# Robinatp/YOLO_Tensorflow

Measured on AMD Instinct MI355X. Metric: images_per_sec, higher is better.
Workload: dtype bf16; 1 GPU; YOLOv3 416x416 batch=32 per GPU, bf16: conv stack + head decode + threshold + TF-NMS; global_batch=32, input=uint8 NHWC resident in HBM, weights=seeded synthetic darknet stream (seed 0), parallelism=dp1

## Files before the change

### include/yolo_hip.h

```cpp
#ifndef YOLO_HIP_H
#define YOLO_HIP_H

#include <stddef.h>
#include <stdint.h>

#ifdef __cplusplus
extern "C" {
#endif

typedef struct yolo_ctx yolo_ctx;

enum yolo_status {
    YOLO_OK = 0,
    YOLO_ERR_INVALID = -1,
    YOLO_ERR_HIP = -2,
    YOLO_ERR_STATE = -3,
    YOLO_ERR_NOMEM = -4,
    YOLO_ERR_IO = -5,
    YOLO_ERR_UNSUPPORTED = -6
};

enum yolo_dtype { YOLO_BF16 = 0, YOLO_FP32 = 1, YOLO_FP8 = 2,
                  YOLO_FP16 = 3,
                  YOLO_FP16X2 = 4 };
// ... 107 lines not shown

int yolo_synchronize(yolo_ctx *ctx);

int yolo_layer_output(yolo_ctx *ctx, int index, int n, float *out, size_t out_floats, int *dims_out);
int yolo_time_forward(yolo_ctx *ctx, int n, int iters, float *total_ms, float *conv_ms);
int yolo_calibrate(int device, void *stream, int f16, double seconds, float *tflops, float *clock_ghz);
int yolo_calibrate_copy(int device, void *stream, double seconds, float *gbs);
int yolo_time_layers(yolo_ctx *ctx, int n, int iters, float *ms_out);
int yolo_autotune(yolo_ctx *ctx, int n, int iters);
int yolo_get_tile_configs(const yolo_ctx *ctx, int32_t *cfgs);
int yolo_set_tile_configs(yolo_ctx *ctx, const int32_t *cfgs);

int yolo_op_conv2d(const float *x, int n, int h, int w, int cin, const float *w_hwio, const float *bias,
                   int k, int stride, int cout, int act, const float *residual, float *out,
                   int dtype, int tile_cfg, int device);
int yolo_op_conv_num_cfgs(void);
int yolo_op_upsample2x(const float *x, int n, int h, int w, int c, int semantics, float *out, int device);
int yolo_op_reorg(const float *x, int n, int h, int w, int c, int stride, int semantics, float *out, int device);
int yolo_op_maxpool(const float *x, int n, int h, int w, int c, int size, int stride, float *out, int device);
int yolo_op_resize_u8(const uint8_t *img, int h, int w, int s, float post_scale, float *out, int device);
int yolo_op_resize_cv2(const uint8_t *img, int h, int w, int oh, int ow, int swap_rb, float divisor, float *out, int device);
int yolo_op_detections_boxes(const float *det, int n, int rows, int attrs, float *out, int device);
int yolo_op_decode(const float *raw, int n, int g, int na, int classes, const float *anchors_wh,
                   int img_size, int decode, int region, float *out, int device);
int yolo_op_letterbox(const float *image_chw, int iw, int ih, int w, int h, int embed, float *out_chw, int device);
int yolo_op_nms_detections(const float *boxes_xywh, float *prob, float *objectness, int n, int classes, float thresh,
                           int by_objectness, int device);
int yolo_op_postprocess(const float *det, int n, int rows, int attrs, float score_thr, float iou_thr,
                        int max_out, int nms_mode, int select_mode, yolo_box *boxes_out,
                        int32_t *counts_out, int device);
int yolo_op_postprocess_rows(const float *det, int n, int rows, int attrs, float score_thr, float iou_thr,
                             int max_out, int nms_mode, int select_mode, yolo_box *boxes_out,
                             int32_t *counts_out, int32_t *rows_out, int device);

int yolo_num_classes(const yolo_ctx *ctx);
int yolo_classify(yolo_ctx *ctx, const void *images, int n, int fmt, int loc, float scale, int top_k,
                  int32_t *classes_out, float *probs_out, int out_loc);
int yolo_classify_images_u8(yolo_ctx *ctx, const uint8_t *pixels, size_t bytes, const yolo_image_desc *descs, int n, int fit, int loc,
                            int top_k, int32_t *classes_out, float *probs_out, int out_loc);
int yolo_op_avgpool(const float *x, int n, int h, int w, int c, int dtype, float *out, int device);
int yolo_op_softmax(const float *x, int n, int len, int groups, float temperature, int top_k, float *probs_out,
                    int32_t *classes_out, float *topk_probs_out, int device);

enum yolo_hierarchy_mode { YOLO_HIER_CONDITIONAL = 0, YOLO_HIER_ABSOLUTE = 1, YOLO_HIER_LEAVES = 2 };
int yolo_set_hier_thresh(yolo_ctx *ctx, float hier_thresh);
int yolo_set_hierarchy_mode(yolo_ctx *ctx, int mode);
int yolo_darknet_boxes_map(yolo_ctx *ctx, int image, int w, int h, float thresh, int relative, const int32_t *map200, float *records, int cap, int *count);
int yolo_tree_geometry(const yolo_ctx *ctx, int32_t *nodes, int32_t *groups, int32_t *parent, int32_t *child, int32_t *group_offset,
                       int32_t *group_size, int32_t *leaf);
int yolo_tree_read(const char *path, int32_t *nodes, int32_t *groups, int32_t *parent, int32_t *child, int32_t *group_offset, int32_t *group_size,
                   int32_t *leaf, char *err, size_t err_len);
int yolo_plan_check(const char *cfg_text, int dtype, char *err, size_t err_len);
int yolo_plan_table(const char *cfg_text, int dtype, int max_batch, int keep_layers, char *out, size_t out_len, char *err, size_t err_len);
int yolo_op_tree_softmax(const float *x, int n, int len, const char *tree_path, float temperature, int mode, float *out, int device);
int yolo_op_tree_top(const float *x_logits, int n, const char *tree_path, float hier_thresh, int32_t *labels_out, int device);

#ifdef __cplusplus
}
#endif
#endif
```

### yolo_tensorflow_amd/csrc/conv_cfgs.h

```cpp
#pragma once
#include "kernels.h"
#include <type_traits>

struct ConvCfg {
    int id, wp, wc, tp, tc, ns, bk, nl;
    bool halo;
    bool free;
    int bh, bw;
    bool head_tail;
};
#define X(id, wp, wc, tp, tc, ns, bk, nl) {id, wp, wc, tp, tc, ns, bk, nl, false, false, 0, 0, false},
#define HX(id, wp, wc, tp, tc, ns, bk, nl, free, bh, bw, head_tail) {id, wp, wc, tp, tc, ns, bk, nl, true, free, bh, bw, head_tail},
constexpr ConvCfg kCfgs[] = {
    X(0, 2, 2, 4, 4, 2, 64, 0)  X(1, 2, 2, 4, 4, 3, 64, 0)  X(2, 2, 2, 2, 4, 2, 64, 0)  X(3, 2, 2, 2, 4, 3, 64, 0)
    X(4, 4, 1, 4, 2, 2, 64, 0)  X(5, 4, 1, 4, 2, 3, 64, 0)  X(6, 2, 2, 4, 2, 2, 64, 0)  X(7, 2, 2, 4, 2, 3, 64, 0)
    X(8, 4, 1, 4, 4, 2, 64, 0)  X(9, 4, 1, 4, 4, 3, 64, 0)  X(10, 4, 2, 4, 4, 2, 64, 0) X(11, 4, 2, 4, 4, 3, 64, 0)
    X(12, 2, 4, 4, 4, 2, 64, 0) X(13, 2, 4, 4, 4, 3, 64, 0) X(14, 2, 2, 2, 2, 2, 64, 0) X(15, 2, 2, 2, 2, 4, 64, 0)
    X(16, 1, 4, 11, 2, 2, 64, 0) X(17, 1, 4, 11, 4, 2, 64, 0) X(18, 1, 4, 11, 1, 2, 64, 0) X(19, 1, 4, 10, 2, 2, 64, 0)
    X(20, 1, 4, 12, 2, 2, 64, 0) X(21, 1, 4, 9, 2, 2, 64, 0) X(22, 1, 4, 13, 2, 2, 64, 0) X(23, 1, 4, 6, 2, 2, 64, 0)
    X(24, 1, 4, 7, 2, 2, 64, 0)
    X(25, 1, 4, 11, 2, 2, 32, 0) X(26, 2, 2, 4, 2, 2, 32, 0)  X(27, 4, 1, 4, 2, 2, 32, 0)  X(28, 4, 1, 4, 4, 2, 32, 0)
    X(29, 2, 2, 2, 2, 2, 32, 0)  X(30, 2, 2, 2, 4, 2, 32, 0)
    X(31, 1, 8, 11, 2, 2, 64, 4) X(32, 1, 8, 11, 2, 2, 64, 0)
    X(33, 1, 4, 11, 2, 3, 64, 0) X(34, 1, 4, 6, 2, 3, 64, 0)
    X(35, 2, 4, 3, 4, 2, 64, 0)
    HX(36, 1, 8, 11, 2, 2, 64, 0, false, 13, 13, false) HX(37, 1, 8, 11, 2, 2, 64, 4, false, 13, 13, false)
    HX(38, 1, 4, 11, 2, 2, 64, 4, false, 13, 13, false) HX(39, 1, 4, 11, 2, 2, 64, 0, false, 13, 13, false)
    HX(40, 1, 8, 11, 2, 2, 64, 0, true, 13, 13, true)   HX(41, 1, 8, 11, 1, 2, 64, 0, true, 13, 13, false)
    HX(42, 1, 4, 11, 2, 2, 64, 0, true, 13, 13, false)  HX(43, 1, 8, 11, 1, 3, 64, 0, true, 13, 13, false)
    X(44, 1, 8, 6, 2, 2, 64, 0) X(45, 1, 8, 6, 2, 3, 64, 0) X(46, 2, 4, 3, 4, 2, 64, 0) X(47, 2, 4, 2, 4, 2, 64, 0)
    X(48, 2, 4, 3, 2, 2, 64, 0) X(49, 2, 4, 4, 2, 3, 64, 0) X(50, 1, 8, 4, 2, 3, 64, 0) X(51, 2, 4, 2, 2, 3, 64, 0)
    X(52, 2, 4, 3, 2, 3, 64, 0) X(53, 2, 4, 3, 2, 4, 64, 0)
    HX(54, 1, 8, 12, 2, 2, 64, 0, true, 10, 19, true) HX(55, 1, 8, 12, 1, 3, 64, 0, true, 10, 19, false) HX(56, 1, 8, 6, 1, 3, 64, 0, true, 5, 19, false)
    HX(57, 1, 4, 11, 4, 2, 64, 0, true, 13, 13, false) HX(58, 1, 4, 11, 2, 2, 64, 0, true, 13, 13, false)
};
#undef X
#undef HX
constexpr int kNumCfgs = (int)(sizeof(kCfgs) / sizeof(kCfgs[0]));
constexpr bool conv_cfgs_indexed() { for (int i = 0; i < kNumCfgs; ++i) if (kCfgs[i].id != i) return false; return true; }
static_assert(conv_cfgs_indexed(), "a tile configuration's id is its index in kCfgs");

template <int... I> struct CfgList { static constexpr bool has(int cfg) { return ((cfg == I) || ...); } };
template <int... I, class F> hipError_t cfg_dispatch(CfgList<I...>, int cfg, F &&f)
{
    hipError_t e = hipErrorInvalidValue;
    (void)((cfg == I && ((e = f(std::integral_constant<int, I>{})), true)) || ...);
    return e;
}
using Cfgs16 = CfgList<0, 1, 2, 3, 4, 5, 6, 7, 8, 9, 10, 11, 12, 13, 14, 15, 16, 17, 18, 19, 20, 21, 22, 23, 24, 25, 26, 27, 28, 29, 30, 31, 32, 33, 34, 35,
                       44, 45, 46, 47, 48, 49, 50, 51, 52, 53>;
using CfgsHalo16 = CfgList<36, 37, 38, 39, 40, 41, 42, 43, 54, 55, 56>;
using CfgsFp8 = CfgList<0, 2, 4, 6, 8, 12, 14, 16, 17, 19, 20, 23, 31, 32, 33, 34, 45, 48, 49, 51>;
using CfgsHaloFp8 = CfgList<36, 37, 38, 39, 40, 41, 42, 43>;
using CfgsSplit = CfgList<0, 2, 3, 4, 6, 7, 8, 14, 15, 16, 23, 25, 26, 27, 28, 33, 34, 45, 49, 52>;
using CfgsHaloSplit = CfgList<40, 41, 43>;
using CfgsPairK = CfgList<0, 2, 3, 4, 6, 7, 8, 14, 15, 16, 23, 33, 34, 45, 49, 52>;
using CfgsHaloPairK = CfgList<40, 41, 43, 57, 58>;
using CfgsPairKPlain = CfgList<0, 2, 4, 6, 8, 14, 16, 33>;

template <int... I> constexpr bool cfgs_are(CfgList<I...>, bool halo) { return ((I >= 0 && I < kNumCfgs && kCfgs[I].halo == halo) && ...); }
static_assert(cfgs_are(Cfgs16{}, false) && cfgs_are(CfgsFp8{}, false) && cfgs_are(CfgsSplit{}, false) && cfgs_are(CfgsPairK{}, false) && cfgs_are(CfgsPairKPlain{}, false), "tiled lists hold tiled ids");
static_assert(cfgs_are(CfgsHalo16{}, true) && cfgs_are(CfgsHaloFp8{}, true) && cfgs_are(CfgsHaloSplit{}, true) && cfgs_are(CfgsHaloPairK{}, true), "halo lists hold halo ids");

inline bool conv_cfg_instantiated(const ConvArgs &a, int cfg)
{
    if (a.in_dt == DT_FP8) return CfgsFp8::has(cfg) || CfgsHaloFp8::has(cfg);
    if (a.pairk) return a.split ? CfgsPairK::has(cfg) || CfgsHaloPairK::has(cfg) : CfgsPairKPlain::has(cfg);
    if (a.split) return CfgsSplit::has(cfg) || CfgsHaloSplit::has(cfg);
    return Cfgs16::has(cfg) || CfgsHalo16::has(cfg);
}

constexpr bool conv_tail_shape(int wp, int wc, int bc, int nl, int eb) { return wp == 1 && wc == 8 && (eb == 2 ? nl == 0 && (bc == 256 || bc == 128) : bc == 256); }
```

### yolo_tensorflow_amd/csrc/conv_igemm.hip

```cpp
#include "kernels.h"
#include <cstdio>
#include <mutex>
#include <set>
#include <utility>

hipError_t conv_opt_in_lds(const void *kernel, size_t lds_bytes)
{
    static std::mutex mu;
    static std::set<std::pair<int, const void *>> done;
    int dev = 0;
    hipError_t e = hipGetDevice(&dev); if (e != hipSuccess) return e;
    std::lock_guard<std::mutex> g(mu);
    if (done.count({dev, kernel})) return hipSuccess;
    e = hipFuncSetAttribute(kernel, hipFuncAttributeMaxDynamicSharedMemorySize, (int)lds_bytes);
    if (e == hipSuccess) done.insert({dev, kernel});
    return e;
}

#include "conv_igemm_kernel.h"


template <int EB>
static hipError_t launch_conv_diag_t(const ConvArgs &a, hipStream_t s)
{
// ... 90 lines not shown

bool conv_c8_direct_ok(const ConvArgs &a)
{
    return (a.in_dt == DT_BF16 || (a.in_dt == DT_F16 && a.out_dt == DT_F16)) && a.ksize == 3 && a.stride == 1 && a.pad == 1 && a.Cin_pad == 8 && a.out_dt != DT_F32 && !a.res && a.Kpad >= 96 &&
           (a.Cout == 16 || a.Cout == 32 || a.Cout == 64);
}

hipError_t launch_conv_c8_direct(const ConvArgs &a, hipStream_t s)
{
    const long M = (long)a.N * a.Ho * a.Wo;
    long waves = (M + 63) / 64;
    long blocks = (waves + 3) / 4; if (blocks > 256 * 8) blocks = 256 * 8;
    dim3 grid((unsigned)blocks), block(256);
    if (a.in_dt == DT_F16) {
        if (a.Cout == 16) hipLaunchKernelGGL((conv_c8_3x3_direct<1, true>), grid, block, 0, s, a);
        else if (a.Cout == 32) hipLaunchKernelGGL((conv_c8_3x3_direct<2, true>), grid, block, 0, s, a);
        else hipLaunchKernelGGL((conv_c8_3x3_direct<4, true>), grid, block, 0, s, a);
    }
    else if (a.Cout == 16) hipLaunchKernelGGL((conv_c8_3x3_direct<1>), grid, block, 0, s, a);
    else if (a.Cout == 32) hipLaunchKernelGGL((conv_c8_3x3_direct<2>), grid, block, 0, s, a);
    else hipLaunchKernelGGL((conv_c8_3x3_direct<4>), grid, block, 0, s, a);
    return hipGetLastError();
}

int conv_num_cfgs() { return kNumCfgs; }
bool conv_cfg_is_halo(int cfg) { return cfg >= 0 && cfg < kNumCfgs && kCfgs[cfg].halo; }
bool conv_cfg_tail_ok(int cfg, int cout, bool fp8, bool head)
{
    if (cfg < 0 || cfg >= kNumCfgs) return false;
    const ConvCfg &c = kCfgs[cfg];
    const int bc = c.wc * c.tc * 16;
    if (head) return !fp8 && c.head_tail && cout == 256;
    return conv_tail_shape(c.wp, c.wc, bc, c.nl, fp8 ? 1 : 2) && bc == cout;
}
const char *conv_cfg_name(int cfg)
{
    struct Names {
        char s[kNumCfgs][32];
        Names()
        {
            for (const ConvCfg &c : kCfgs) {
                const int bp = c.wp * c.tp * 16, bc = c.wc * c.tc * 16;
                if (c.halo && !CfgsHalo16::has(c.id)) snprintf(s[c.id], sizeof s[c.id], "f%dc%d_w%d_pair", bp, bc, c.wp * c.wc);
                else if (c.halo && (c.bh != HALO_B || c.bw != HALO_B)) snprintf(s[c.id], sizeof s[c.id], "f%dx%dc%d_s%d", c.bh, c.bw, bc, c.ns);
                else snprintf(s[c.id], sizeof s[c.id], "%s%dc%d_s%d_k%d%s%d", c.halo ? (c.free ? "f" : "h") : "p", bp, bc, c.ns, c.bk, c.nl ? "_L" : "_w", c.nl ? c.nl : c.wp * c.wc);
            }
        }
    };
    static const Names names;
    if (cfg < 0 || cfg >= kNumCfgs) return cfg == CONV_CFG_DIRECT ? "direct_c8" : "?";
    return names.s[cfg];
}

template <int WP, int WC, int TP, int TC, int NS, int BK, int NL, bool UNI, int EB, bool H16 = false, bool SPLIT = false>
static hipError_t launch_u(const ConvArgs &a, hipStream_t s)
{
    constexpr int BP = WP * TP * 16, BC = WC * TC * 16;
    const long M = (long)a.N * a.Ho * a.Wo;
    const long tiles = ((M + BP - 1) / BP) * ((a.Cout + BC - 1) / BC);
    constexpr size_t lds = conv_lds_bytes<WP, WC, TP, TC, NS, BK, NL>();
    dim3 grid((unsigned)((tiles + 7) / 8 * 8)), block(64 * (WP * WC + NL));
    if (lds > 65536) {
        hipError_t e = conv_opt_in_lds((const void *)conv_igemm<WP, WC, TP, TC, NS, BK, UNI, NL, false, EB, false, false, H16, SPLIT>, lds);
        if (e != hipSuccess) return e;
    }
    hipLaunchKernelGGL((conv_igemm<WP, WC, TP, TC, NS, BK, UNI, NL, false, EB, false, false, H16, SPLIT>), grid, block, lds, s, conv_tile_magic(a, BC, 0));
    return hipGetLastError();
}

template <int WP, int WC, int TP, int TC, int NS, int BK, int NL, int EB, bool H16 = false, bool SPLIT = false>
static hipError_t launch_t(const ConvArgs &a, hipStream_t s)
{
    if (((double)a.N * a.H * a.W * a.in_stride + 2.0 * (a.W + 1) * a.in_stride) * EB >= 2147483648.0) return hipErrorInvalidValue;
    constexpr int BKE = BK * 2 / EB;
    if (a.Kpad % BKE) return hipErrorInvalidValue;
    return (a.Cin_pad % BKE) == 0 ? launch_u<WP, WC, TP, TC, NS, BK, NL, true, EB, H16, SPLIT>(a, s) : launch_u<WP, WC, TP, TC, NS, BK, NL, false, EB, H16, SPLIT>(a, s);
}

template <int ID, int EB, bool H16 = false, bool SPLIT = false>
static hipError_t launch_id(const ConvArgs &a, hipStream_t s)
{
    constexpr ConvCfg c = kCfgs[ID];
    return launch_t<c.wp, c.wc, c.tp, c.tc, c.ns, c.bk, c.nl, EB, H16, SPLIT>(a, s);
}

hipError_t launch_conv_bf16(const ConvArgs &a, int cfg, hipStream_t s)
{
    if (a.in_dt != DT_BF16 && a.in_dt != DT_F16) return hipErrorInvalidValue;
    if (a.in_dt == DT_F16 && a.out_dt != DT_F16 && a.out_dt != DT_F32) return hipErrorInvalidValue;
    if (cfg == CONV_CFG_DIRECT && a.split) return launch_conv_c8_direct_pair(a, s);
    if (a.pairk) return launch_conv_pair(a, cfg, s);
    if (a.split) {
        if (a.in_dt != DT_F16 || (a.out_dt != DT_F16 && a.out_dt != DT_F32) || a.w2 || (a.res && a.out_dt == DT_F32)) return hipErrorInvalidValue;
        if (CfgsHaloSplit::has(cfg)) return launch_conv_halo13(a, cfg, s);
        return cfg_dispatch(CfgsSplit{}, cfg, [&](auto id) { return launch_id<decltype(id)::value, 2, true, true>(a, s); });
    }
    if (cfg == CONV_CFG_DIRECT) return conv_c8_direct_ok(a) ? launch_conv_c8_direct(a, s) : hipErrorInvalidValue;
    if (conv_cfg_is_halo(cfg)) return launch_conv_halo13(a, cfg, s);
    if (a.in_dt == DT_F16) return cfg_dispatch(Cfgs16{}, cfg, [&](auto id) { return launch_id<decltype(id)::value, 2, true>(a, s); });
    return cfg_dispatch(Cfgs16{}, cfg, [&](auto id) { return launch_id<decltype(id)::value, 2>(a, s); });
}

hipError_t launch_conv_fp8(const ConvArgs &a, int cfg, hipStream_t s)
{
    if (a.in_dt != DT_FP8) return hipErrorInvalidValue;
    if (CfgsHaloFp8::has(cfg)) return launch_conv_halo13(a, cfg, s);
    return cfg_dispatch(CfgsFp8{}, cfg, [&](auto id) { return launch_id<decltype(id)::value, 1>(a, s); });
}
```

### yolo_tensorflow_amd/csrc/conv_igemm_kernel.h

```cpp
#pragma once
#include "kernels.h"
#include "conv_cfgs.h"
#include "device_common.h"
#include "halo_perm_tables.h"
#include <type_traits>
#include <utility>

__device__ __forceinline__ uint32_t f32_to_bf16_rn(float f)
{
    __bf16 b = (__bf16)f;
    return (uint32_t)__builtin_bit_cast(uint16_t, b);
}
__device__ __forceinline__ float bf16_bits_to_f32(uint32_t b) { return __builtin_bit_cast(float, b << 16); }
__device__ __forceinline__ void pair_join2(uint32_t H, uint32_t L, float &a, float &b)
{
    asm("v_fma_mix_f32 %0, %1, 1.0, %2 op_sel_hi:[1,0,1]" : "=v"(a) : "v"(H), "v"(L));
    asm("v_fma_mix_f32 %0, %1, 1.0, %2 op_sel:[1,0,1] op_sel_hi:[1,0,1]" : "=v"(b) : "v"(H), "v"(L));
}
__device__ __forceinline__ void pair_split2(float a, float b, uint32_t &H, uint32_t &L)
{
    H = __builtin_bit_cast(uint32_t, __builtin_convertvector(f32x2_t{a, b}, f16x2_t));
    uint32_t l;
    asm("v_fma_mixlo_f16 %0, %1, -1.0, %2 op_sel_hi:[1,0,0]" : "=v"(l) : "v"(H), "v"(a));
    asm("v_fma_mixhi_f16 %0, %1, -1.0, %2 op_sel:[1,0,0] op_sel_hi:[1,0,0]" : "+v"(l) : "v"(H), "v"(b));
    L = l;
}
template <bool HI> __device__ __forceinline__ uint32_t f32x2_to_fp8(float a, float b, uint32_t old)
{
    a = __builtin_amdgcn_fmed3f(a, -FP8_MAX, FP8_MAX); b = __builtin_amdgcn_fmed3f(b, -FP8_MAX, FP8_MAX);
    return (uint32_t)__builtin_amdgcn_cvt_pk_fp8_f32(a, b, (int)old, HI);
}

__device__ __forceinline__ int fast_div(int n, uint32_t mul, uint32_t shift)
{
    return shift == 255 ? n : (int)(__umulhi((uint32_t)n, mul) >> shift);
}

constexpr int PAIR_PD = 4, PAIR_SLEEP = 48;
template <int MAXN> __device__ __forceinline__ void wait_vmcnt_rt(int n)
{
    static_assert(MAXN <= 16, "ladder length");
    switch (n) {
#define W_(k) case k: if (k <= MAXN) { wait_vmcnt<k>(); } break;
        W_(1) W_(2) W_(3) W_(4) W_(5) W_(6) W_(7) W_(8) W_(9) W_(10) W_(11) W_(12) W_(13) W_(14) W_(15) W_(16)
#undef W_
    default: wait_vmcnt<0>(); break;
    }
}

#define OOB_OFFSET 0x80000000u

template <int... I, class F> __device__ __forceinline__ void static_for_impl(std::integer_sequence<int, I...>, F &&f) { (f(std::integral_constant<int, I>{}), ...); }
template <int N, class F> __device__ __forceinline__ void static_for(F &&f) { static_for_impl(std::make_integer_sequence<int, N>{}, f); }

struct HaloPermPk { unsigned w[16][8]; };
template <int N> constexpr HaloPermPk make_halo_perm_pk(const unsigned short (&tab)[N])
{
    HaloPermPk t{};
    for (int l = 0; l < 16; ++l)
        for (int j = 0; j < N / 16; ++j) {
            const unsigned v = tab[j * 16 + l];
            t.w[l][j / 4] |= (v & 0xffu) << (8 * (j % 4));
            t.w[l][4 + j / 4] |= (v >> 8) << (8 * (j % 4));
        }
    return t;
}
__device__ const HaloPermPk kHaloPermPk = make_halo_perm_pk(kHaloPerm13);
__device__ const HaloPermPk kHaloPermPk10x19 = make_halo_perm_pk(kHaloPerm10x19);
__device__ const HaloPermPk kHaloPermPk5x19 = make_halo_perm_pk(kHaloPerm5x19);
constexpr int HALO_B = 13;
constexpr int HALO_APIX = 160;
constexpr int halo_apieces(int bh, int bw) { return ((bh + 2) * (bw + 2) * (HALO_APIX / 16) + 63) / 64; }
constexpr int HALO_APIECES = halo_apieces(HALO_B, HALO_B);
constexpr int HALO_ACT_BYTES = HALO_APIECES * 1024;
constexpr unsigned halo_div_mul(int bw) { return (65536u + bw - 1) / bw; }
constexpr bool halo_div_ok(int bw) { for (unsigned r = 0; r < 256; ++r) if (((r * halo_div_mul(bw)) >> 16) != r / bw) return false; return true; }

template <int WP, int WC, int TP, int TC, int NS, int BK, bool UNI, int NL = 0, bool DIAG = false, int EB = 2, bool HALO = false, bool FREE = false, bool H16 = false, bool SPLIT = false, int BH = HALO_B, int BW = HALO_B, bool HEADT = false, bool PAIRK = false>
__global__ __launch_bounds__(64 * (WP * WC + NL)) void conv_igemm(const ConvArgs a)
{
#if defined(__HIP_DEVICE_COMPILE__)
    constexpr int NC = WP * WC;
    constexpr int NW = NL > 0 ? NL : NC;
    constexpr int NTOT = NC + NL;
    constexpr int BP = WP * TP * 16;
    constexpr int BC = WC * TC * 16;
    static_assert(BK == 64 || BK == 32, "K-step");
    static_assert(BC <= 256, "filters and bias are padded to multiples of 256 output channels (cout_pad): a wider tile would read past them");
    static_assert(EB == 2 || (EB == 1 && BK == 64), "fp8 operands need the 128-B-row form");
    static_assert(!H16 || EB == 2, "fp16 is a 16-bit storage type");
    static_assert(!SPLIT || (H16 && !DIAG), "split pairs are fp16 pairs");
    static_assert(!PAIRK || (H16 && EB == 2 && BK == 64 && UNI && !DIAG && NL == 0), "pair K loop: fp16, 128-byte rows = one 32-channel group hi | lo, uniform taps");
    constexpr int RB = BK * 2;
    constexpr int EPC = 16 / EB;
    constexpr int BKE = RB / EB;
    constexpr int CPRW = RB / 16;
    constexpr int RG = 64 / CPRW;
    constexpr int GP = (BP + RG - 1) / RG, GC = (BC + RG - 1) / RG;
    constexpr int LA = (GP + NW - 1) / NW, LB = (GC + NW - 1) / NW;
    constexpr int L = LA + LB;
    constexpr int BPL = LA * NW * RG, BCL = LB * NW * RG;
    constexpr int STAGE_BYTES = (BPL + BCL) * RB;
    static_assert(!HALO || (WP == 1 && TP == (BH * BW + 15) / 16 && TP <= 16 && BK == 64 && UNI && (NS == 2 || (FREE && NS <= 4))), "halo form: one BH x BW block per workgroup; more than two filter stages in the free-running form only");
    static_assert((BH == 13 && BW == 13) || (BH == 10 && BW == 19) || (BH == 5 && BW == 19), "block shapes with a generated permutation table");
    static_assert(halo_div_ok(BW) && BH * BW <= 256, "row / BW by multiply-high");
    constexpr int HBH = BH, HBW = BW, HPW = BW + 2, HPH = BH + 2, APIX = HALO_APIX, APIECES = halo_apieces(BH, BW), ACT_BYTES = APIECES * 1024;
    constexpr int LAH = HALO ? (APIECES + NW - 1) / NW : 1;
    constexpr int FSTAGE = BCL * RB;
    static_assert(!HALO || LAH <= 9, "a halo tile is fetched during the nine taps of the previous chunk");
    static_assert(!FREE || (HALO && NL == 0 && LB * RG == TC * 16), "free-running form: every wave fetches its own filter rows");

    if constexpr (H16) fp16_saturating_mode();
    extern __shared__ __attribute__((aligned(16))) char smem[];

    unsigned long long t_top = 0;
    if (DIAG) asm volatile("s_memtime %0\n\ts_waitcnt lgkmcnt(0)" : "=s"(t_top)::"memory");
    const int tid = threadIdx.x;
    const int lane = tid & 63;
    u32x4_t perm_rd = {0, 0, 0, 0}, perm_wr = {0, 0, 0, 0};
    if constexpr (HALO) {
        const u32x4_t *pk = (const u32x4_t *)(BH == 10 ? kHaloPermPk10x19.w[lane & 15] : BH == 5 ? kHaloPermPk5x19.w[lane & 15] : kHaloPermPk.w[lane & 15]);
        perm_rd = pk[0]; perm_wr = pk[1];
    }
    asm volatile("" ::"s"(a.in), "s"(a.wt), "s"(a.in_stride), "s"(a.N), "s"(a.H), "s"(a.W), "s"(a.Cout), "s"(a.Kpad), "s"(a.Ho), "s"(a.Wo),
                 "s"(a.tc_mul), "s"(a.tc_shift), "s"(a.bpi_mul), "s"(a.bpi_shift), "s"(a.bpr_mul), "s"(a.bpr_shift));
    const int wave_id = __builtin_amdgcn_readfirstlane(tid >> 6);
    const bool is_loader = NL == 0 || wave_id >= NC;
    const bool is_consumer = wave_id < NC;
    const int wid = NL > 0 ? (wave_id >= NC ? wave_id - NC : 0) : wave_id;
    const int wpi = wave_id % WP, wci = (wave_id / WP) % WC;

    const int M = a.N * a.Ho * a.Wo;
    const int tilesC = (a.Cout + BC - 1) / BC;
    const int hbr = HALO ? (a.H + HBH - 1) / HBH : 0, hbc = HALO ? (a.W + HBW - 1) / HBW : 0;
    const int tilesP = HALO ? a.N * hbr * hbc : (M + BP - 1) / BP;
    const int per_xcd = gridDim.x >> 3;
    const int tile = (blockIdx.x & 7) * per_xcd + (blockIdx.x >> 3);
    if (tile >= tilesP * tilesC) return;
    const int pt = fast_div(tile, a.tc_mul, a.tc_shift);
    const int ct = tile - pt * tilesC;
    int bn = 0, by = 0, bx = 0;
    if constexpr (HALO) {
        const int bpr = hbc, bpi = hbc * hbr;
        bn = fast_div(pt, a.bpi_mul, a.bpi_shift); const int r = pt - bn * bpi; by = fast_div(r, a.bpr_mul, a.bpr_shift); bx = r - by * bpr;
    }
// ... 760 lines not shown
                        *(uint2 *)(st2 + (j * 16 + l15) * RS2 + ((t2g * T2W + t) * 16 + lq * 4) * 2) = uint2{pack16x2<H16>(v[0], v[1]), pack16x2<H16>(v[2], v[3])};
                    };
                    const int j0 = head_tail ? 0 : (TP * t2p) / T2P, j1 = head_tail ? TP : (TP * (t2p + 1)) / T2P;
                    {
                        int j = j0;
#pragma unroll 1
                        for (; j + 1 < j1; j += 2) {
                            f32x4 ca[T2W], cb[T2W];
#pragma unroll
                            for (int t = 0; t < T2W; ++t) ca[t] = cb[t] = f32x4{0.f, 0.f, 0.f, 0.f};
#pragma unroll
                            for (int kk = 0; kk < K2S; ++kk) {
                                const bf16x8 xa = *(const bf16x8 *)(smem + (j * 16 + l15) * RS + (kk * 4 + lq) * 16);
                                const bf16x8 xb = *(const bf16x8 *)(smem + ((j + 1) * 16 + l15) * RS + (kk * 4 + lq) * 16);
#pragma unroll
                                for (int t = 0; t < T2W; ++t) {
                                    ca[t] = mma16<H16>(fw2[t][kk], xa, ca[t]);
                                    cb[t] = mma16<H16>(fw2[t][kk], xb, cb[t]);
                                }
                            }
#pragma unroll
                            for (int t = 0; t < T2W; ++t) { finish(ca[t], j, t); finish(cb[t], j + 1, t); }
                        }
                        if (j < j1) {
                            f32x4 cc_[T2W];
#pragma unroll
                            for (int t = 0; t < T2W; ++t) cc_[t] = f32x4{0.f, 0.f, 0.f, 0.f};
#pragma unroll
                            for (int kk = 0; kk < K2S; ++kk) {
                                const bf16x8 x = *(const bf16x8 *)(smem + (j * 16 + l15) * RS + (kk * 4 + lq) * 16);
#pragma unroll
                                for (int t = 0; t < T2W; ++t) cc_[t] = mma16<H16>(fw2[t][kk], x, cc_[t]);
                            }
#pragma unroll
                            for (int t = 0; t < T2W; ++t) finish(cc_[t], j, t);
                        }
                    }
                }
                if (DIAG) te5 = stamp();
                asm volatile("s_waitcnt lgkmcnt(0)" ::: "memory");
                block_barrier();
                if (DIAG) te6 = stamp();
                constexpr int CPR2 = C2 / 8;
                const __amdgpu_buffer_rsrc_t rs_out2 = tile_rsrc((char *)a.out2 + m0 * a.out2_stride * 2);
                if (!head_tail)
#pragma unroll
                for (int it = 0; it < (BP * CPR2 + NT - 1) / NT; ++it) {
                    int row, cc;
                    const unsigned off = piece_off(tid + it * NT, CPR2, 0, (unsigned)a.out2_stride * 2u, row, cc);
                    __builtin_amdgcn_raw_buffer_store_b128(*(const u32x4_t *)(st2 + row * RS2 + cc * 16), rs_out2, off, 0, OUT_STORE_AUX);
                }
            }
        }
    } else if (is_consumer && !HALO) {
#pragma unroll
        for (int i = 0; i < TC; ++i) {
            const int ch = ct * BC + (wci * TC + i) * 16 + lq * 4;
            if (ch >= a.Cout) continue;
            const float4 bv = *(const float4 *)(a.bias + ch);
            float4 sv = float4{1.f, 1.f, 1.f, 1.f};
            if (EB == 1 && a.oscale) sv = *(const float4 *)(a.oscale + ch);
            int oq = -1, oan = 0;
            if (a.obj_out) {
#pragma unroll
                for (int q = 0; q < 4; ++q) {
                    const int an = fast_div(ch + q, a.obj_mul, a.obj_shift);
                    if (ch + q - an * a.obj_attrs == 4 && ch + q < a.Cout) { oq = q; oan = an; }
                }
            }
#pragma unroll
            for (int j = 0; j < TP; ++j) {
                const int m = pt * BP + (wpi * TP + j) * 16 + l15;
                if (m >= M) continue;
                float v[4];
                if (EB == 1) { v[0] = acc[i][j][0] * sv.x + bv.x; v[1] = acc[i][j][1] * sv.y + bv.y; v[2] = acc[i][j][2] * sv.z + bv.z; v[3] = acc[i][j][3] * sv.w + bv.w; }
                else { v[0] = acc[i][j][0] + bv.x; v[1] = acc[i][j][1] + bv.y; v[2] = acc[i][j][2] + bv.z; v[3] = acc[i][j][3] + bv.w; }
                if (a.act == ACT_LEAKY) {
#pragma unroll
                    for (int q = 0; q < 4; ++q) v[q] = fmaxf(v[q], 0.1f * v[q]);
                }
                float *o = (float *)a.out + (size_t)m * a.out_stride + ch;
                if (oq >= 0) a.obj_out[(size_t)m * a.obj_na + oan] = oq == 0 ? v[0] : oq == 1 ? v[1] : oq == 2 ? v[2] : v[3];
                if (ch + 3 < a.Cout) *(float4 *)o = float4{v[0], v[1], v[2], v[3]};
                else
                    for (int q = 0; q < 4; ++q) if (ch + q < a.Cout) o[q] = v[q];
            }
        }
    }
    if (DIAG && a.dbg && lane == 0) {
        asm volatile("s_waitcnt vmcnt(0)" ::: "memory");
        const unsigned long long t_end = stamp_loop();
        unsigned long long *d = a.dbg + ((size_t)tile * NTOT + wave_id) * 16;
        const unsigned long long rt1 = __builtin_amdgcn_s_memrealtime();
        d[0] = t_wait; d[1] = t_issue; d[2] = t_mma; d[3] = t_loop_end - t_all0; d[4] = t_end - t_loop_end;
        d[6] = t_all0 - t_top; d[7] = t_first - t_all0; d[8] = te1 - t_loop_end; d[9] = te2 - te1; d[10] = te3 - te2; d[11] = t_end - (te6 ? te6 : te3);
        d[12] = te4 ? te4 - te3 : 0; d[13] = te4 ? te5 - te4 : 0; d[14] = te4 ? te6 - te5 : 0;
        d[15] = (t_loop_end - t_all0) * 100ull / (rt_loop - rt0 ? rt_loop - rt0 : 1);
        d[5] = ((unsigned long long)KT << 40) | ((t_end - t_all0) * 100ull / (rt1 - rt0 ? rt1 - rt0 : 1));
    }
#endif
}

template <int WP, int WC, int TP, int TC, int NS, int BK, int NL = 0, bool HALO = false, int BH = HALO_B, int BW = HALO_B>
constexpr size_t conv_lds_bytes()
{
    constexpr int NW = NL > 0 ? NL : WP * WC, BP = WP * TP * 16, BC = WC * TC * 16;
// ... 8 lines not shown
```

### yolo_tensorflow_amd/csrc/kernels.h

```cpp
#pragma once
#ifndef OUT_STORE_AUX
#define OUT_STORE_AUX 16
#endif
#ifndef HALO_LOAD_AUX
#define HALO_LOAD_AUX 0
#endif
#ifndef RES_LOAD_AUX
#define RES_LOAD_AUX 0
#endif
#include <hip/hip_runtime.h>
#include <stdint.h>
typedef unsigned out_u32x4 __attribute__((ext_vector_type(4)));
__device__ __forceinline__ void out_store16_at(const void *base, unsigned byte_off, unsigned x, unsigned y, unsigned z, unsigned w)
{
#if defined(__HIP_DEVICE_COMPILE__)
    __amdgpu_buffer_rsrc_t r = __builtin_amdgcn_make_buffer_rsrc((void *)base, 0, 0x80000000u, 0x00020000);
    __builtin_amdgcn_raw_buffer_store_b128(out_u32x4{x, y, z, w}, r, byte_off, 0, OUT_STORE_AUX);
#endif
}

typedef uint16_t bf16_t;
struct fp8_t { uint8_t b; };
struct f16_t { uint16_t b; };
enum { DT_BF16 = 0, DT_F32 = 1, DT_FP8 = 2, DT_F16 = 3 };
inline size_t dt_size(int dt) { return dt == DT_F32 ? 4 : dt == DT_FP8 ? 1 : 2; }
#define FP8_MAX 448.0f

struct TView {
    void *ptr = nullptr;
    int n = 0, h = 0, w = 0, c = 0;
    int stride = 0;
    int dt = DT_BF16;
};

enum { ACT_LINEAR = 0, ACT_LEAKY = 1 };

struct ConvArgs {
    const void *in; int in_stride;
    const void *wt;
    const float *bias;
    void *out; int out_stride; int out_dt;
    const void *res; int res_stride;
    int in_dt;
    int split;
    int pairk;
    const float *oscale;
    float out_inv_scale, res_scale;
    float mid_scale, mid_inv_scale;
    const void *w2; const float *b2; void *out2; int out2_stride, K2pad, act2;
    const void *w2f;
    const float *oscale2; float out2_inv_scale;
    int N, H, W, Cin_pad;
    int Ho, Wo, Cout;
    int ksize, stride, pad;
    int Kpad;
    int kchunk;
    int act;
    const void *zeros;
    uint32_t howo_mul, howo_shift, wo_mul, wo_shift;
    float *obj_out; int obj_attrs, obj_na; uint32_t obj_mul, obj_shift;
    unsigned long long *dbg;
    int dbg_light;
    int C2out;
    int tail_f32;
    uint32_t tc_mul, tc_shift, bpi_mul, bpi_shift, bpr_mul, bpr_shift;
};
inline int conv_kchunk(int cin_pad, int wdt) { const int row = wdt == DT_FP8 ? 128 : 64; return (wdt != DT_F32 && cin_pad % row == 0) ? row : cin_pad; }
inline void conv_magic(uint32_t d, uint32_t &mul, uint32_t &shift)
{
    if (d <= 1) { mul = 0; shift = 255; return; }
    uint32_t l = 0; while ((1u << l) < d) ++l;
    const unsigned k = 31 + l;
    mul = (uint32_t)(((unsigned long long)1 << k) / d + 1);
    shift = k - 32;
}
inline void conv_finalize(ConvArgs &a)
{
    conv_magic((uint32_t)(a.Ho * a.Wo), a.howo_mul, a.howo_shift);
    conv_magic((uint32_t)a.Wo, a.wo_mul, a.wo_shift);
}
inline ConvArgs conv_tile_magic(const ConvArgs &a0, int BC, int bh, int bw = 0)
{
    ConvArgs a = a0;
    if (bw == 0) bw = bh;
    conv_magic((uint32_t)((a.Cout + BC - 1) / BC), a.tc_mul, a.tc_shift);
    if (bh > 0) { const int br = (a.H + bh - 1) / bh, bc = (a.W + bw - 1) / bw; conv_magic((uint32_t)(br * bc), a.bpi_mul, a.bpi_shift); conv_magic((uint32_t)bc, a.bpr_mul, a.bpr_shift); }
    return a;
}

hipError_t conv_opt_in_lds(const void *kernel, size_t lds_bytes);
#define CONV_CFG_DIRECT 1000
bool conv_c8_direct_ok(const ConvArgs &a);
int conv_num_cfgs();
const char *conv_cfg_name(int cfg);
int conv_default_cfg(const ConvArgs &a);
bool conv_cfg_runs(const ConvArgs &a, int cfg);
int conv_resolve_cfg(const ConvArgs &a, int planned);
hipError_t launch_conv_bf16(const ConvArgs &a, int cfg, hipStream_t s);
bool conv_halo13_ok(const ConvArgs &a);
bool conv_halo_cfg_ok(const ConvArgs &a, int cfg);
bool conv_cfg_is_halo(int cfg);
hipError_t launch_conv_halo13(const ConvArgs &a, int cfg, hipStream_t s);
hipError_t launch_conv_halo13_diag(const ConvArgs &a, hipStream_t s, int variant = 0);
bool conv_cfg_tail_ok(int cfg, int cout, bool fp8, bool head = false);
hipError_t launch_conv_pair(const ConvArgs &a, int cfg, hipStream_t s);
struct StemPairArgs {
    const void *in;
    const uint8_t *in_u8; float in_scale, in_mul, in_add;
    const void *w0; const float *b0; int Kpad0, C0, act0;
    const void *w1; const float *b1; int Kpad1, act1;
    void *out; int out_stride;
    int N, H, W, Ho, Wo;
};
bool conv_stem_pair_ok(const StemPairArgs &a);
hipError_t launch_conv_stem_pair(const StemPairArgs &a, hipStream_t s);
bool conv_c8_direct_pair_ok(const ConvArgs &a);
hipError_t launch_conv_c8_direct_pair(const ConvArgs &a, hipStream_t s);
hipError_t launch_conv_fp8(const ConvArgs &a, int cfg, hipStream_t s);
hipError_t launch_conv_diag(const ConvArgs &a, hipStream_t s);
struct StemArgs {
    const void *in; int in_stride;
    const uint8_t *in_u8; float in_scale, in_mul, in_add;
    const void *w0; const float *b0; int Kpad0, C0, act0;
    const void *w1; const float *b1; int Kpad1, C1, act1;
    void *out; int out_stride;
    int dt;
    const void *w2; const float *b2; int Kpad2, C2, act2;
    void *out2; int out2_stride;
    int N, H, W, Ho, Wo;
    const void *zeros;
};
bool conv_stem_ok(const StemArgs &a);
hipError_t launch_conv_stem(const StemArgs &a, hipStream_t s);
// ... 54 lines not shown
hipError_t launch_upsample2x(const TView &in, const TView &out, int bilinear, hipStream_t s);
hipError_t launch_maxpool(const TView &in, const TView &out, int size, int stride, int pad, hipStream_t s);
hipError_t launch_reorg(const TView &in, const TView &out, int stride, int darknet, hipStream_t s);
hipError_t launch_add(const TView &a, const TView &b, const TView &out, hipStream_t s, float sa = 1.f, float sb = 1.f, float so = 1.f);
hipError_t launch_copy(const TView &in, const TView &out, hipStream_t s);
hipError_t launch_local(const TView &in, const TView &out, const void *w, const float *bias, int k, int stride, int pad, int act, hipStream_t s);
hipError_t launch_to_f32(const TView &in, float *out, hipStream_t s, float scale = 1.f);
hipError_t launch_from_f32(const float *in, const TView &out, hipStream_t s, float scale = 1.f);
enum { PAIR_ILV = 0, PAIR_B3 = 1 };
hipError_t launch_split_from_f32(const float *in, int in_stride, void *out, int out_stride, int Cp, size_t npix, hipStream_t s, int layout = PAIR_ILV);
hipError_t launch_split_to_f32(const void *in, int in_stride, int Cp, float *out, int out_stride, size_t npix, hipStream_t s, int layout = PAIR_ILV);
hipError_t launch_upsample2x_pair(const TView &in, const TView &out, int bilinear, hipStream_t s);
hipError_t launch_add_split(const void *a, int a_stride, const void *b, int b_stride, void *out, int out_stride, int Cp, size_t npix, hipStream_t s);

hipError_t launch_avgpool(const TView &in, bool in_pair, const TView &out, hipStream_t s);
#define CLS_SOFTMAX_MAX 8192
#define CLS_TOPK_MAX 32
struct SoftmaxArgs {
    const float *x; int x_stride;
    int n, groups, len; float temperature;
    float *probs; int p_stride;
    int top_k; int *cls; float *topk_probs;
};
hipError_t launch_softmax_topk(const SoftmaxArgs &a, hipStream_t s);
bool avgpool_softmax_ok(const TView &in, const SoftmaxArgs &a);
hipError_t launch_avgpool_softmax(const TView &in, float *pooled, int pooled_stride, const SoftmaxArgs &a, hipStream_t s);

struct TreeDev { int n, groups, levels; const int *parent, *child, *goff, *gsize, *leaf, *order, *lvl; };
struct TreeRows { const float *x; size_t rows; int na, cell_stride, an_stride, off; };
enum { TREE_CONDITIONAL = 0, TREE_ABSOLUTE = 1, TREE_LEAVES = 2 };
hipError_t launch_tree_softmax(const TreeDev &t, const TreeRows &x, float temperature, int mode, float *out, int out_stride,
                               int top_k, int *cls, float *topk_probs, hipStream_t s);
hipError_t launch_tree_top(const TreeDev &t, const TreeRows &x, float hier_thresh, int *labels, hipStream_t s);
struct DecodeArgs;
hipError_t launch_decode_region_tree(const DecodeArgs &a, const TreeDev &t, hipStream_t s);
hipError_t launch_tree_score_rows(const float *det, size_t nrows, int attrs, const TreeDev &t, float hier_thresh, float *scores, int *labels, hipStream_t s);
hipError_t launch_decode_region_tree_lean(const DecodeArgs &a, const TreeDev &t, float hier_thresh, float *scores, int *labels, hipStream_t s);
hipError_t launch_darknet_tree_probs(const float *det, int attrs, const TreeDev &t, float thresh, float hier_thresh, const int *map200,
                                     float *rec, const int *src, const int *count, int cap, hipStream_t s);
hipError_t launch_head_darknet_layout_tree(const float *raw, int raw_stride, int cells, int na, int classes, const TreeDev &t, float *out, hipStream_t s);

struct DecodeArgs {
    const float *raw; int raw_stride;
    int n, g, na, classes;
    float anchors[2 * 16];
    int img_size;
    int mode;
    int region;
    float *det; int rows_total; int row_off;
    float *box4;
    float reject_below;
};
#ifdef __HIPCC__
__device__ __forceinline__ float region_sigmoid(float x) { return 1.0f / (1.0f + expf(-x)); }
__device__ __forceinline__ float region_box_attr(int k, const float *p, int cell, int g, const float *anchor_wh)
{
    const float G = (float)g;
    if (k == 0) return ((float)(cell % g) + region_sigmoid(p[0])) / G;
    if (k == 1) return ((float)(cell / g) + region_sigmoid(p[1])) / G;
    if (k == 2) return (anchor_wh[0] * expf(p[2])) / G;
    if (k == 3) return (anchor_wh[1] * expf(p[3])) / G;
    return region_sigmoid(p[4]);
}
__device__ __forceinline__ float darknet_layout_box_attr(int k, const float *p)
{
    return (k == 2 || k == 3) ? p[k] : (float)(1. / (1. + exp(-(double)p[k])));
}
#endif
struct LeanHead { const float *raw; const float *obj; int raw_stride, g, na, row_off; long box_begin; float anchors[2 * 16]; };
struct LeanArgs {
    int nheads; LeanHead h[4];
    long total;
    int n, classes, img_size, mode, rows_total;
    float *box4; float reject_below;
    uint4 *list; unsigned *list_count; unsigned list_cap;
};
hipError_t launch_decode_lean(const LeanArgs &a, float *scores, int *labels, hipStream_t s);
hipError_t launch_decode(const DecodeArgs &a, float *scores, int *labels, hipStream_t s);
hipError_t launch_decode_v1(const float *raw, int raw_stride, int n, int side, int num, int classes, int sqr, float *det, int rows_total,
                            int row_off, float *scores, int *labels, hipStream_t s);

struct PostArgs {
    const float *det; int n, rows, attrs;
    float score_thr, iou_thr; int max_out, nms_mode, select_mode;
    const float *box4;
    int scores_ready;
    int corners_in;
    int img_h, img_w;
    float *scores; int *labels; int *cand; unsigned long long *keys; int rows_pow2;
    float4 *sbox; int *slabel; float *sscore;
    void *boxes_out; int *counts_out;
    int *rows_out; int *srow;
    unsigned *zero_word;
    const ImgDesc *geom; int geom_fit, geom_pixels, geom_relative, net_size;
    int geom_net_pixels;
};
hipError_t launch_postprocess(const PostArgs &a, hipStream_t s);
void launch_score_rows(const float *det, size_t nrows, int attrs, float *scores, int *labels, hipStream_t s, int objectness_mode = 0);
hipError_t launch_letterbox_chw(const float *img, int iw, int ih, int S, void *out, int out_dt, int out_stride, hipStream_t s);
hipError_t launch_nms_dets(const float4 *boxes, float *prob, float *objectness, int n, int classes, float thresh, int by_obj, hipStream_t s);
struct DnBoxesArgs {
    const float *det; int attrs;
    int nheads, kind[8], grid[8], na[8], off[8];
    float thresh; int w, h, netw, neth, relative;
    const float *raw; int side, classes, sqr;
    float *rec;
// ... 8 lines not shown
```

### yolo_tensorflow_amd/csrc/post_ops.hip

```cpp
#include "kernels.h"
#include "wave_ops.h"
#include <math.h>

struct BoxOut { float x0, y0, x1, y1, score; int cls; };

__device__ __forceinline__ float sigmoidf_(float x) { return 1.0f / (1.0f + expf(-x)); }
__device__ __forceinline__ float sigmoid_fast(float x)
{
    const float e = __builtin_amdgcn_exp2f(-x * 1.44269504088896340736f);
    return __builtin_amdgcn_rcpf(1.0f + e);
}

__device__ __forceinline__ float yolo_box_attr(int k, float x, int cx, int cy, const float *anchor, float G, float S, int mode)
{
    const float t = k < 2 ? sigmoidf_(x) + (float)(k == 0 ? cx : cy) : expf(x) * anchor[k - 2];
    return mode == 0 ? t / G : t * S;
}

__global__ __launch_bounds__(256) void k_decode_yolo(const DecodeArgs a, float *scores, int *labels)
{
    const int attrs = 5 + a.classes;
    const int lane = threadIdx.x & 63;
    const long wave = ((long)blockIdx.x * blockDim.x + threadIdx.x) >> 6;
    const long nwaves = ((long)gridDim.x * blockDim.x) >> 6;
    const long total = (long)a.n * a.g * a.g * a.na;
    const int stride = a.img_size / a.g;
    const float G = (float)a.g, S = (float)stride;
    const int gg = a.g * a.g;
    constexpr int U = 4;
    const bool two = attrs > 64;
    for (long b0 = wave * U; b0 < total; b0 += nwaves * U) {
        float v0[U], v1[U];
        const float *src[U]; float *dst[U]; size_t rowi[U]; int an_[U], cell_[U];
        const unsigned ub = (unsigned)__builtin_amdgcn_readfirstlane((int)b0);
        unsigned t0 = ub / (unsigned)a.na; int an = (int)(ub - t0 * a.na);
        int b = (int)(t0 / (unsigned)gg); int cell = (int)(t0 - (unsigned)b * gg);
#pragma unroll
        for (int u = 0; u < U; ++u) {
            if (u > 0 && b0 + u < total) { if (++an == a.na) { an = 0; if (++cell == gg) { cell = 0; ++b; } } }
            an_[u] = an; cell_[u] = cell;
            src[u] = a.raw + ((size_t)b * gg + cell) * a.raw_stride + an * attrs;
            rowi[u] = (size_t)b * a.rows_total + a.row_off + (size_t)cell * a.na + an;
            dst[u] = a.det + rowi[u] * attrs;
            v0[u] = lane < attrs ? src[u][lane] : 0.f;
            v1[u] = (two && lane + 64 < attrs) ? src[u][lane + 64] : 0.f;
        }
#pragma unroll
        for (int u = 0; u < U; ++u) {
            if (b0 + u >= total) break;
            const int an = an_[u], cell = cell_[u];
            const float r0 = lane < 4 ? yolo_box_attr(lane, v0[u], cell % a.g, cell / a.g, a.anchors + 2 * an, G, S, a.mode) : sigmoid_fast(v0[u]);
            const float r1 = sigmoid_fast(v1[u]);
            if (lane < attrs) dst[u][lane] = r0;
            if (two && lane + 64 < attrs) dst[u][lane + 64] = r1;
            const float obj = __shfl(r0, 4);
            float best = -INFINITY; int bi = 0x7fffffff;
            if (lane >= 5 && lane < attrs) { best = obj * r0; bi = lane - 5; }
            if (two && lane + 64 < attrs) first_max(best, bi, obj * r1, lane + 59);
            wave_argmax(best, bi);
            if (lane == 0 && scores) { scores[rowi[u]] = best; labels[rowi[u]] = bi; }
        }
    }
}

// ... 907 lines not shown
```

### yolo_tensorflow_amd/csrc/yolo_api.cpp

```cpp
#include "yolo_ctx.h"

extern "C" {

yolo_ctx *yolo_create(const yolo_config *cfg, char *err, size_t err_len)
{
    auto bail = [&](yolo_ctx *c, const std::string &m) -> yolo_ctx * { if (err && err_len) snprintf(err, err_len, "%s", m.c_str()); if (c) yolo_destroy(c); return nullptr; };
    if (!cfg || cfg->struct_size != sizeof(yolo_config)) return bail(nullptr, "yolo_create: bad yolo_config (struct_size)");
    if (cfg->max_batch < 1) return bail(nullptr, "yolo_create: max_batch < 1");
    if (cfg->dtype != YOLO_BF16 && cfg->dtype != YOLO_FP32 && cfg->dtype != YOLO_FP8 && cfg->dtype != YOLO_FP16 && cfg->dtype != YOLO_FP16X2) return bail(nullptr, "yolo_create: dtype");
    yolo_ctx *c = new yolo_ctx();
    c->device = cfg->device; c->max_batch = cfg->max_batch; c->dtype = cfg->dtype; c->semantics = cfg->semantics;
    c->decode = cfg->decode; c->keep_layers = cfg->keep_layers;
    int ndev = 0;
    if (hipGetDeviceCount(&ndev) != hipSuccess || ndev < 1) return bail(c, "yolo_create: no HIP device (this library has no CPU fallback)");
    if (hipSetDevice(c->device) != hipSuccess) return bail(c, "yolo_create: hipSetDevice failed");
    if (cfg->stream) c->stream = (hipStream_t)cfg->stream;
    else { if (hipStreamCreate(&c->stream) != hipSuccess) return bail(c, "yolo_create: hipStreamCreate failed"); c->own_stream = true; }
    std::vector<Section> secs; std::string perr;
    c->cfg_text = cfg->cfg_text ? cfg->cfg_text : "";
    if (!parse_cfg(cfg->cfg_text, secs, perr)) return bail(c, perr);
    if (build_plan(c, secs) != YOLO_OK) return bail(c, c->err);
    if (allocate(c) != YOLO_OK) return bail(c, c->err);
    resolve_scales(c);
    return c;
}

void yolo_destroy(yolo_ctx *c)
{
    if (!c) return;
    hipSetDevice(c->device);
    if (c->stream) hipStreamSynchronize(c->stream);
    for (void *p : c->phys) if (p) hipFree(p);
    for (auto &L : c->layers) { if (L.d_w) hipFree(L.d_w); if (L.d_b) hipFree(L.d_b); if (L.d_sc) hipFree(L.d_sc); if (L.d_wf) hipFree(L.d_wf); if (L.d_obj) hipFree(L.d_obj); }
    void *ptrs[] = {c->input.ptr, c->d_zeros, c->d_stage, c->d_det, c->d_scores, c->d_labels, c->d_cand, c->d_keys, c->d_sbox, c->d_slabel, c->d_sscore, c->d_boxes, c->d_counts,
                    c->d_dn_rec, c->d_dn_src, c->d_dn_count, c->d_dn_last, c->d_box4, c->s2d.ptr, c->d_srow, c->d_rows, c->d_lean_list, c->d_lean_cnt, c->d_f32a, c->d_f32b, c->d_descs, c->d_pix, c->d_cls_idx, c->d_cls_prob};
    for (void *p : ptrs) if (p) hipFree(p);
    for (auto &t : c->trees) free_tree(t);
    if (c->d_map200) hipFree(c->d_map200);
    if (c->gexec) hipGraphExecDestroy(c->gexec);
    if (c->gexec_img) hipGraphExecDestroy(c->gexec_img);
    if (c->own_stream && c->stream) hipStreamDestroy(c->stream);
    delete c;
}

const char *yolo_last_error(const yolo_ctx *c) { return c ? c->err.c_str() : g_op_err.c_str(); }

size_t yolo_weights_count(const yolo_ctx *c) { return c ? c->weights_count : 0; }

int yolo_input_size(const yolo_ctx *c, int *h, int *w, int *ch) { if (!c) return YOLO_ERR_INVALID; if (h) *h = c->in_h; if (w) *w = c->in_w; if (ch) *ch = c->in_c; return YOLO_OK; }
int yolo_num_rows(const yolo_ctx *c) { return c ? c->rows : YOLO_ERR_INVALID; }
int yolo_num_attrs(const yolo_ctx *c) { return c ? c->attrs : YOLO_ERR_INVALID; }
int yolo_num_classes(const yolo_ctx *c) { return !c ? YOLO_ERR_INVALID : c->cls_layer >= 0 ? c->layers[c->cls_layer].C : c->attrs - 5; }
int yolo_num_layers(const yolo_ctx *c) { return c ? (int)c->layers.size() : YOLO_ERR_INVALID; }
// ... 63 lines not shown
        if (a.nheads == 8) return fail(c, YOLO_ERR_UNSUPPORTED, "more than 8 heads");
        if (L.type == L_DETECT) {
            if (a.nheads) return fail(c, YOLO_ERR_UNSUPPORTED, "a [detection] head next to other heads");
            a.raw = (const float *)c->layers[li - 1].out.ptr + (size_t)image * c->layers[li - 1].out.stride; a.side = L.side; a.classes = L.classes; a.sqr = L.sqr;
            a.kind[0] = 2; a.grid[0] = L.side; a.na[0] = L.na; a.off[0] = L.row_off; a.nheads = 1;
            continue;
        }
        if (a.raw) return fail(c, YOLO_ERR_UNSUPPORTED, "a [detection] head next to other heads");
        a.kind[a.nheads] = L.type == L_REGION; a.grid[a.nheads] = L.H; a.na[a.nheads] = L.na; a.off[a.nheads] = L.row_off; ++a.nheads;
    }
    a.thresh = thresh; a.w = w; a.h = h; a.netw = c->in_w; a.neth = c->in_h; a.relative = relative;
    a.cap = cap < c->rows ? cap : c->rows;
    a.rec = a.cap > 0 ? c->d_dn_rec : nullptr; a.src = c->d_dn_src; a.count = c->d_dn_count;
    HIPCK(c, launch_darknet_boxes(a, c->stream));
    if (c->tree_head >= 0 && a.rec) {
        if (map200) {
            if (!c->d_map200) HIPCK(c, hipMalloc((void **)&c->d_map200, 200 * 4));
            HIPCK(c, hipMemcpyAsync(c->d_map200, map200, 200 * 4, hipMemcpyHostToDevice, c->stream));
        }
        HIPCK(c, launch_darknet_tree_probs(a.det, c->attrs, c->trees[c->layers[c->tree_head].tree].dev, thresh, c->hier_thresh, map200 ? c->d_map200 : nullptr,
                                           a.rec, a.src, a.count, a.cap, c->stream));
    }
    int n = 0;
    HIPCK(c, hipMemcpyAsync(&n, c->d_dn_count, 4, hipMemcpyDeviceToHost, c->stream)); HIPCK(c, hipStreamSynchronize(c->stream));
    *count = n;
    const int got = n < a.cap ? n : a.cap;
    if (got > 0) { HIPCK(c, hipMemcpyAsync(records, c->d_dn_rec, (size_t)got * c->attrs * 4, hipMemcpyDeviceToHost, c->stream)); HIPCK(c, hipStreamSynchronize(c->stream)); }
    return YOLO_OK;
}

size_t yolo_last_layer_size(const yolo_ctx *c)
{
    if (!c) return 0;
    if (c->cls_layer >= 0) return (size_t)c->layers[c->cls_layer].C;
    for (int i = (int)c->layers.size() - 1; i >= 0; --i) {
        const Layer &L = c->layers[i];
        if (L.type == L_DETECT) return (size_t)L.side * L.side * (L.classes + 5 * L.na);
        if (L.type == L_YOLO || L.type == L_REGION) return (size_t)L.H * L.W * L.na * (5 + L.classes);
    }
    return 0;
}

int yolo_last_layer_output_batch(yolo_ctx *c, int n, float *out, size_t out_floats)
{
    if (!c || !out) return YOLO_ERR_INVALID;
    if (c->last_n < 1) return fail(c, YOLO_ERR_STATE, "yolo_last_layer_output before a forward pass");
    if (n < 1 || n > c->last_n) return fail(c, YOLO_ERR_INVALID, "yolo_last_layer_output of %d images but the last forward ran %d", n, c->last_n);
    if (c->cls_layer >= 0) {
        const Layer &S = c->layers[c->cls_layer];
        if (out_floats < (size_t)n * S.C) return fail(c, YOLO_ERR_INVALID, "output buffer too small (%zu < %zu floats)", out_floats, (size_t)n * S.C);
        HIPCK(c, hipSetDevice(c->device));
        return copy_out(c, out, S.out.ptr, (size_t)n * S.C * 4, YOLO_HOST);
    }
    const int li = output_layer(c);
    if (li < 1 || (c->layers[li].type != L_YOLO && c->layers[li].type != L_REGION && c->layers[li].type != L_DETECT))
        return fail(c, YOLO_ERR_UNSUPPORTED, "the last layer is not a detection head");
    const Layer &L = c->layers[li]; const Layer &P = c->layers[li - 1];
    const size_t per = yolo_last_layer_size(c), need = per * (size_t)n;
    if (out_floats < need) return fail(c, YOLO_ERR_INVALID, "output buffer too small (%zu < %zu floats)", out_floats, need);
    HIPCK(c, hipSetDevice(c->device));
    if (L.type == L_DETECT) {
        HIPCK(c, hipMemcpy2DAsync(out, per * 4, P.out.ptr, (size_t)P.out.stride * 4, per * 4, (size_t)n, hipMemcpyDeviceToHost, c->stream)); HIPCK(c, hipStreamSynchronize(c->stream));
        return YOLO_OK;
    }
    if (!c->d_dn_last || c->dn_last_cap < need) {
        if (c->d_dn_last) { HIPCK(c, hipStreamSynchronize(c->stream)); HIPCK(c, hipFree(c->d_dn_last)); c->d_dn_last = nullptr; c->dn_last_cap = 0; }
        HIPCK(c, hipMalloc((void **)&c->d_dn_last, need * 4)); c->dn_last_cap = need;
    }
    const size_t cells = (size_t)L.H * L.W;
    for (int b = 0; b < n; ++b)
        if (L.tree >= 0) HIPCK(c, launch_head_darknet_layout_tree((const float *)P.out.ptr + (size_t)b * cells * P.out.stride, P.out.stride, (int)cells, L.na, L.classes, c->trees[L.tree].dev, c->d_dn_last + (size_t)b * per, c->stream));
        else HIPCK(c, launch_head_darknet_layout((const float *)P.out.ptr + (size_t)b * cells * P.out.stride, P.out.stride, (int)cells, L.na, L.classes, L.type == L_REGION, c->d_dn_last + (size_t)b * per, c->stream));
    HIPCK(c, hipMemcpyAsync(out, c->d_dn_last, need * 4, hipMemcpyDeviceToHost, c->stream)); HIPCK(c, hipStreamSynchronize(c->stream));
    return YOLO_OK;
}

int yolo_last_layer_output(yolo_ctx *c, float *out, size_t out_floats) { return yolo_last_layer_output_batch(c, 1, out, out_floats); }

int yolo_head_raw(yolo_ctx *c, int head, int n, float *out, size_t out_floats)
{
    if (!c || !out || head < 0) return YOLO_ERR_INVALID;
    if (int r = need_detector(c, "yolo_head_raw")) return r;
    if (c->last_n < 1 || n < 1 || n > c->last_n) return fail(c, YOLO_ERR_STATE, "yolo_head_raw of %d images but the last forward ran %d", n, c->last_n);
    int k = 0;
    for (size_t li = 1; li < c->layers.size(); ++li) {
        const Layer &L = c->layers[li];
        if (L.type != L_YOLO && L.type != L_REGION && L.type != L_DETECT) continue;
        if (k++ != head) continue;
        const Layer &P = c->layers[li - 1];
        const size_t px = (size_t)n * P.H * P.W, need = px * P.C;
        if (out_floats < need) return fail(c, YOLO_ERR_INVALID, "output buffer too small (%zu < %zu floats)", out_floats, need);
        if (P.out.dt != DT_F32 || !P.out.ptr) return fail(c, YOLO_ERR_STATE, "internal: head conv output is not fp32");
        HIPCK(c, hipSetDevice(c->device));
        HIPCK(c, hipMemcpy2DAsync(out, (size_t)P.C * 4, P.out.ptr, (size_t)P.out.stride * 4, (size_t)P.C * 4, px, hipMemcpyDeviceToHost, c->stream));
        HIPCK(c, hipStreamSynchronize(c->stream));
        return YOLO_OK;
    }
    return fail(c, YOLO_ERR_INVALID, "no detection head %d", head);
}

int yolo_synchronize(yolo_ctx *c) { if (!c) return YOLO_ERR_INVALID; HIPCK(c, hipStreamSynchronize(c->stream)); return YOLO_OK; }

int yolo_layer_output(yolo_ctx *c, int index, int n, float *out, size_t out_floats, int *dims_out)
{
    if (!c) return YOLO_ERR_INVALID;
    if (index < 0 || index >= (int)c->layers.size() || n < 1 || n > c->last_n) return fail(c, YOLO_ERR_INVALID, "bad layer index / n");
    const Layer &L = c->layers[index];
    if (!c->keep_layers) {
        bool kept = L.type == L_CONV && L.storage >= 0 && L.residual_from < -1 && !never_stored(L, index);
        if (kept) for (const Storage &o : c->storages) if (&o != &c->storages[L.storage] && o.phys == c->storages[L.storage].phys && o.def > c->storages[L.storage].def) kept = false;
        if (!kept) return fail(c, YOLO_ERR_STATE, "yolo_layer_output needs keep_layers=1 (without it: only a conv layer's own tensor whose buffer no later layer reuses)");
    }
    if (dims_out) { dims_out[0] = L.H; dims_out[1] = L.W; dims_out[2] = L.C; }
    size_t need = (size_t)n * L.H * L.W * L.C;
    if (!out) return YOLO_OK;
    if (out_floats < need) return fail(c, YOLO_ERR_INVALID, "output buffer too small");
    HIPCK(c, hipSetDevice(c->device));
    float *tmp = nullptr; HIPCK(c, hipMalloc((void **)&tmp, need * 4));
    TView v = L.out; v.n = n;
    float vs = 1.f;
    if (v.dt == DT_FP8) {
        vs = c->eff_scale[index];
        if (vs != vs) { hipFree(tmp); return fail(c, YOLO_ERR_UNSUPPORTED, "layer %d concatenates tensors with different fp8 scales; read its sources", index); }
    }
    hipError_t e = hipSuccess;
    float *wide = nullptr;
    if (L.pair && v.dt == DT_F16) {
        const int cp = roundup(L.C, 32);
        e = hipMalloc((void **)&wide, (size_t)n * L.H * L.W * cp * 4);
        if (e == hipSuccess) e = launch_split_to_f32(v.ptr, v.stride, cp, wide, cp, (size_t)n * L.H * L.W, c->stream);
        v.ptr = wide; v.stride = cp; v.dt = DT_F32;
    }
    if (e == hipSuccess) e = launch_to_f32(v, tmp, c->stream, vs);
    if (e == hipSuccess) e = hipMemcpyAsync(out, tmp, need * 4, hipMemcpyDeviceToHost, c->stream);
    if (e == hipSuccess) e = hipStreamSynchronize(c->stream);
    hipFree(tmp); if (wide) hipFree(wide);
    if (e != hipSuccess) return fail(c, YOLO_ERR_HIP, "layer_output: %s", hipGetErrorString(e));
    return YOLO_OK;
}

}
```

### yolo_tensorflow_amd/csrc/yolo_ctx.h

```cpp
#pragma once
#include "../../include/yolo_hip.h"
#include "kernels.h"

#include <algorithm>
#include <cmath>
#include <cstdarg>
#include <cstdio>
#include <cstdlib>
#include <cstring>
#include <map>
#include <string>
#include <vector>

namespace yolo_impl {

enum LType { L_CONV, L_SHORTCUT, L_ROUTE, L_UPSAMPLE, L_MAXPOOL, L_REORG, L_YOLO, L_REGION, L_DETECT, L_LOCAL, L_AVGPOOL, L_SOFTMAX };
enum ConvKernel { K_TILED, K_HALO, K_S2 };
enum FuseKind { F_NONE, F_STEM, F_PSTEM, F_RESBLOCK, F_C3S2 };

struct Section { std::string type; std::map<std::string, std::string> kv; };

struct Layer {
    LType type;
    int H = 0, W = 0, C = 0;
    std::vector<int> in;
    int filters = 0, size = 0, stride = 1, pad = 0, bn = 0, act = ACT_LINEAR;
    int cin = 0, cin_pad = 0, kpad = 0, cout_pad = 0;
    void *d_w = nullptr; float *d_b = nullptr; float *d_sc = nullptr;
    void *d_wf = nullptr;
    int in_dt = DT_BF16;
    int store_dt = DT_BF16;
    bool pair = false;
    int tile_cfg = -1;
    int residual_from = -2;
    bool head = false;
    float *d_obj = nullptr;
    int kernel = K_TILED;
    int fused = F_NONE, launcher = -1;
    int fuse_n = 0; bool fuse_ok = false;
    bool fc = false; int fc_h = 0, fc_w = 0, fc_c = 0;
    bool s2d7 = false;
    int side = 0, sqr = 0;
    int tail_layer = -1, fused_into = -1; bool tail_on = false;
    bool noop = false;
    std::vector<int> copy_inputs;
    std::vector<int> copy_offsets;
    int psize = 0, pstride = 0, ppad = 0;
    int na = 0, classes = 0, row_off = 0;
    std::vector<float> anchors;
    int groups = 1; float temperature = 1.f; bool pool_fused = false; bool cost = false;
    int tree = -1;
    int storage = -1; int ch_off = 0;
    TView out;
};

struct Tree {
    std::string path, text;
    int n = 0, groups = 0, levels = 0;
    std::vector<int> parent, child, goff, gsize, leaf, order, lvl;
    int *d_all = nullptr; TreeDev dev{};
};

struct Storage { int def = 1 << 30, last = -1; size_t bytes = 0; int phys = -1; int stride = 0; int dt = DT_BF16; bool persistent = false; };


}
using namespace yolo_impl;

struct yolo_ctx {
    std::string err, cfg_text;
    int device = 0;
    hipStream_t stream = nullptr; bool own_stream = false;
    int max_batch = 1, dtype = YOLO_BF16, semantics = YOLO_SEM_TF, decode = YOLO_DECODE_RATIO, keep_layers = 0;
    int in_h = 0, in_w = 0, in_c = 0;
    std::vector<Layer> layers;
    std::vector<Storage> storages;
    std::vector<void *> phys; std::vector<size_t> phys_bytes;
    TView input;
    void *d_zeros = nullptr;
    void *d_stage = nullptr; size_t stage_bytes = 0;
    TView s2d;
    const uint8_t *stem_u8 = nullptr; float stem_scale = 1.f; int stem_u8_n = 0;
    float in_mul = 1.f, in_add = 0.f;
    float *d_det = nullptr; int rows = 0, attrs = 0;
    int cls_layer = -1, cls_topk = 0, cls_mode = 0; int *d_cls_idx = nullptr; float *d_cls_prob = nullptr;
    bool lean_cnt_dirty = false;
    void *d_lean_list = nullptr; unsigned *d_lean_cnt = nullptr;
    float *d_box4 = nullptr; bool lean = false, det_valid = false, lean_ok = false; float lean_thr = 0.f; int lean_heads = 0;
    float *d_scores = nullptr; int *d_labels = nullptr; int *d_cand = nullptr; unsigned long long *d_keys = nullptr;
    float4 *d_sbox = nullptr; int *d_slabel = nullptr; float *d_sscore = nullptr; int rows_pow2 = 0;
    void *d_boxes = nullptr; int *d_counts = nullptr; int boxes_cap = 0;
    int *d_srow = nullptr, *d_rows = nullptr;
    float *d_dn_rec = nullptr; int *d_dn_src = nullptr; int *d_dn_count = nullptr; float *d_dn_last = nullptr; size_t dn_last_cap = 0;
    struct GKey { const void *img; int n, fmt; float scale, st, it; int mo, nm, sm; void *bo, *co; } gkey{};
    hipGraphExec_t gexec = nullptr; int gstate = 0;
    ImgDesc *d_descs = nullptr; void *d_pix = nullptr; size_t pix_cap = 0;
    int geom_fit = -1, geom_n = 0;
    struct GKeyImages { const void *pix; size_t bytes; int n, fit, units; float st, it; int mo, nm, sm; void *bo, *co; } gkey_img;
    hipGraphExec_t gexec_img = nullptr; int gstate_img = 0;
    std::vector<Tree> trees; int tree_head = -1; float hier_thresh = 0.5f, lean_hier = 0.f; int hierarchy_mode = 0; bool tree_full = false;
    int *d_map200 = nullptr;
    bool weights_loaded = false;
    int scores_mode = -1;
    size_t weights_count = 0;
    double conv_flops = 0;
    int last_n = 0;
    std::vector<float> user_scale, eff_scale;
    bool split() const { return dtype == YOLO_FP16X2; }
    bool in_pair = false;
    bool pair_of(int idx) const { return idx < 0 ? in_pair : layers[idx].pair; }
    float *d_f32a = nullptr, *d_f32b = nullptr; size_t f32_cap = 0;
    int act_dt() const { return dtype == YOLO_FP32 ? DT_F32 : dtype == YOLO_FP8 ? DT_FP8 : (dtype == YOLO_FP16 || dtype == YOLO_FP16X2) ? DT_F16 : DT_BF16; }
    bool half_like() const { return dtype == YOLO_BF16 || dtype == YOLO_FP16; }
    int gran() const { return dtype == YOLO_FP8 ? 16 : 8; }
    size_t esize() const { return dt_size(act_dt()); }
};

namespace yolo_impl {

int fail(yolo_ctx *c, int code, const char *fmt, ...);
#define HIPCK(c, expr)                                                                       \
    do { hipError_t e_ = (expr);                                                             \
        if (e_ != hipSuccess) return fail(c, YOLO_ERR_HIP, "%s: %s", #expr, hipGetErrorString(e_)); } while (0)

inline int roundup(int x, int m) { return (x + m - 1) / m * m; }
inline int pair_width(int C) { return 2 * roundup(C, 32); }
inline int gran_of(int dt) { return dt == DT_FP8 ? 16 : 8; }
inline void drop_graph(yolo_ctx *c)
{
    if (c->gexec) { hipGraphExecDestroy(c->gexec); c->gexec = nullptr; } if (c->gstate > 0) c->gstate = 0;
    if (c->gexec_img) { hipGraphExecDestroy(c->gexec_img); c->gexec_img = nullptr; } if (c->gstate_img > 0) c->gstate_img = 0;
}

inline bool fused_may_fall_back(const Layer &L) { return L.fused == F_RESBLOCK || L.fused == F_C3S2; }
inline bool never_stored(const Layer &L, int i) { return L.fused != F_NONE && i < L.launcher; }
inline bool input_never_loaded(const Layer &L, int i) { return L.fused != F_NONE && L.fused != F_PSTEM && i >= L.launcher; }
inline bool fixed_kernel(const Layer &L) { return L.kernel != K_TILED || L.fused != F_NONE; }
inline bool window_check_skipped(const Layer &L, int i) { return L.fused != F_NONE && (!fused_may_fall_back(L) || (L.fused == F_RESBLOCK && i < L.launcher)); }
inline bool rides_as_tail(const yolo_ctx *c, const Layer &L) { return L.fused_into >= 0 && c->layers[L.fused_into].tail_on; }
inline bool issues_launch(const yolo_ctx *c, int i) { const Layer &L = c->layers[i]; return (L.fused == F_NONE || L.launcher == i) && !rides_as_tail(c, L); }

uint16_t f2bf(float f);
uint16_t f2h(float f);
uint8_t f2e4m3(float f);
void pack_conv(const Layer &L, const float *bn_or_bias, const float *w_oihw, int wdt, const float *in_scale,
               std::vector<uint8_t> &wbuf, std::vector<float> &bias, std::vector<float> &osc, int semantics = YOLO_SEM_TF, int split = 0);
float h2f(uint16_t h);
void resolve_scales(yolo_ctx *c);
void channel_scales(const yolo_ctx *c, int idx, std::vector<float> &out);
int tail_fragments(yolo_ctx *c);
int parse_tree(const std::string &text, Tree &t, std::string &err);
int load_tree(const std::string &path, Tree &t, std::string &err);
std::vector<int> pack_tree(const Tree &t, size_t at[7]);
TreeDev tree_dev(const Tree &t, const int *base, const size_t at[7]);
int upload_tree(yolo_ctx *c, Tree &t);
void free_tree(Tree &t);
int score_tree_rows(yolo_ctx *c, int n);
extern thread_local const std::vector<std::pair<std::string, std::string>> *g_tree_texts;
bool parse_cfg(const char *text, std::vector<Section> &out, std::string &err);
int build_plan(yolo_ctx *c, const std::vector<Section> &secs);
int allocate(yolo_ctx *c);
TView view_of(const yolo_ctx *c, int idx);
ConvArgs conv_args(const yolo_ctx *c, const Layer &L, int n);
int run_layer(yolo_ctx *c, int i, int n);
int stage_in(yolo_ctx *c, const void *images, int n, int fmt, int loc, float scale);
int run_network(yolo_ctx *c, int n, bool lean = false);
int copy_out(yolo_ctx *c, void *dst, const void *src, size_t bytes, int loc);
int output_layer(const yolo_ctx *c);
int need_detector(yolo_ctx *c, const char *what);
int post_args_ok(yolo_ctx *c, int max_out, int nms_mode, int select_mode);
struct PostGeom { int fit, pixels; };
int post(yolo_ctx *c, const float *det, int n, int rows, int attrs, float score_thr, float iou_thr, int max_out,
         int nms_mode, int select_mode, int img_h, int img_w, int scores_ready, yolo_box *boxes_out, int32_t *counts_out, int out_loc, int32_t *rows_out = nullptr,
         const PostGeom *geom = nullptr);
extern thread_local std::string g_op_err;
TView make_view(void *p, int n, int h, int w, int c, int stride, int dt);

}
```

### yolo_tensorflow_amd/csrc/yolo_pack.cpp

```cpp
#include "yolo_ctx.h"

namespace yolo_impl {

uint16_t f2bf(float f)
{
    uint32_t u; memcpy(&u, &f, 4);
    if ((u & 0x7fffffffu) > 0x7f800000u) return (uint16_t)((u >> 16) | 0x40);
    u += 0x7fffu + ((u >> 16) & 1u);
    return (uint16_t)(u >> 16);
}

uint16_t f2h(float f)
{
    uint32_t u; memcpy(&u, &f, 4);
    const uint16_t sign = (uint16_t)((u >> 16) & 0x8000u);
    if (f != f) return (uint16_t)(sign | 0x7e00u);
    float a = fabsf(f);
    if (a >= 65504.f) return (uint16_t)(sign | 0x7bffu);
    if (a < ldexpf(1.f, -24) * 0.5f) return sign;
    int e; frexpf(a, &e); e -= 1;
    if (e < -14) e = -14;
    const float quantum = ldexpf(1.f, e - 10);
    const float q = nearbyintf(a / quantum);
    const float v = q * quantum;
// ... 83 lines not shown
    }
}

void resolve_scales(yolo_ctx *c)
{
    const int NL = (int)c->layers.size();
    if ((int)c->user_scale.size() != NL) c->user_scale.assign(NL, 1.f);
    c->eff_scale.assign(NL, 1.f);
    for (int i = 0; i < NL; ++i) {
        const Layer &L = c->layers[i];
        switch (L.type) {
        case L_CONV: c->eff_scale[i] = L.store_dt != DT_FP8 ? 1.f : (L.residual_from >= -1 && i + 1 < NL) ? c->user_scale[i + 1] : c->user_scale[i]; break;
        case L_SHORTCUT: c->eff_scale[i] = L.store_dt != DT_FP8 ? 1.f : c->user_scale[i]; break;
        case L_ROUTE: c->eff_scale[i] = L.in.size() == 1 ? c->eff_scale[L.in[0]] : NAN; break;
        case L_UPSAMPLE: case L_MAXPOOL: case L_REORG: c->eff_scale[i] = c->eff_scale[L.in[0]]; break;
        default: break;
        }
    }
}
void channel_scales(const yolo_ctx *c, int idx, std::vector<float> &out)
{
    const Layer &L = c->layers[idx];
    if (L.type == L_ROUTE && L.in.size() > 1) { for (int j : L.in) channel_scales(c, j, out); return; }
    if (L.type == L_REORG) {
        std::vector<float> src; channel_scales(c, L.in[0], src);
        for (int k = 0; k < L.C; ++k) out.push_back(src[0]);
        return;
    }
    if (L.type == L_ROUTE || L.type == L_UPSAMPLE || L.type == L_MAXPOOL) { channel_scales(c, L.in[0], out); return; }
    for (int k = 0; k < L.C; ++k) out.push_back(c->eff_scale[idx]);
}

int tail_fragments(yolo_ctx *c)
{
    std::vector<uint16_t> src, dst;
    for (auto &T : c->layers) {
        if (T.type != L_CONV || T.fused_into < 0) continue;
        if (T.in_dt != DT_BF16 && T.in_dt != DT_F16) continue;
        const int C2 = T.head ? T.cout_pad : roundup(T.filters, 16), K = T.kpad;
        if (C2 > T.cout_pad || K % 32 || (T.head && T.cout_pad < 256)) continue;
        src.resize((size_t)T.cout_pad * K); dst.assign((size_t)C2 * K, 0);
        HIPCK(c, hipMemcpy(src.data(), T.d_w, src.size() * 2, hipMemcpyDeviceToHost));
        const int K2S = K / 32;
        for (int ct2 = 0; ct2 < C2 / 16; ++ct2)
            for (int kk = 0; kk < K2S; ++kk)
                for (int lane = 0; lane < 64; ++lane)
                    memcpy(&dst[(((size_t)ct2 * K2S + kk) * 64 + lane) * 8], &src[(size_t)(ct2 * 16 + (lane & 15)) * K + (kk * 4 + (lane >> 4)) * 8], 16);
        if (!T.d_wf) HIPCK(c, hipMalloc(&T.d_wf, dst.size() * 2));
        HIPCK(c, hipMemcpy(T.d_wf, dst.data(), dst.size() * 2, hipMemcpyHostToDevice));
    }
    return YOLO_OK;
}

}

extern "C" {

int yolo_set_act_scales(yolo_ctx *c, const float *scales, int n)
{
    if (!c) return YOLO_ERR_INVALID;
    if (c->dtype != YOLO_FP8) return fail(c, YOLO_ERR_STATE, "activation scales only exist in the fp8 configuration");
    if (!scales || n != (int)c->layers.size()) return fail(c, YOLO_ERR_INVALID, "need one scale per layer (%zu)", c->layers.size());
    for (int i = 0; i < n; ++i) if (!(scales[i] > 0.f) || !std::isfinite(scales[i])) return fail(c, YOLO_ERR_INVALID, "layer %d: scale must be finite and > 0", i);
    c->user_scale.assign(scales, scales + n);
    resolve_scales(c);
    c->weights_loaded = false;
    drop_graph(c);
    return YOLO_OK;
}

int yolo_set_weights(yolo_ctx *c, const float *flat, size_t n)
{
    if (!c) return YOLO_ERR_INVALID;
    if (!flat) return fail(c, YOLO_ERR_INVALID, "weights == NULL");
    if (n != c->weights_count) return fail(c, YOLO_ERR_IO, "weights stream has %zu floats, topology needs %zu", n, c->weights_count);
    HIPCK(c, hipSetDevice(c->device));
    const float *p = flat;
    std::vector<uint8_t> wbuf; std::vector<float> bias, osc;
    resolve_scales(c);
    for (auto &L : c->layers) {
        if (L.type == L_LOCAL) {
            const int loc = L.H * L.W, F = L.filters, k = L.size, C = L.cin;
            const float *bfile = p; p += (size_t)F * loc;
            const float *wfile = p; p += (size_t)loc * F * C * k * k;
            std::vector<float> b((size_t)loc * F);
            for (int f = 0; f < F; ++f) for (int l = 0; l < loc; ++l) b[(size_t)l * F + f] = bfile[(size_t)f * loc + l];
            const size_t es = dt_size(L.in_dt);
            std::vector<uint8_t> wb((size_t)loc * F * k * k * C * es);
            for (size_t lf = 0; lf < (size_t)loc * F; ++lf)
                for (int ch = 0; ch < C; ++ch)
                    for (int t = 0; t < k * k; ++t) {
                        const float v = wfile[(lf * C + ch) * k * k + t];
                        const size_t idx = (lf * k * k + t) * C + ch;
                        if (L.in_dt == DT_F32) memcpy(&wb[idx * 4], &v, 4);
                        else { uint16_t h = L.in_dt == DT_F16 ? f2h(v) : f2bf(v); memcpy(&wb[idx * 2], &h, 2); }
                    }
            HIPCK(c, hipMemcpy(L.d_w, wb.data(), wb.size(), hipMemcpyHostToDevice));
            HIPCK(c, hipMemcpy(L.d_b, b.data(), b.size() * 4, hipMemcpyHostToDevice));
            continue;
        }
        if (L.type != L_CONV) continue;
        const float *params = p; p += (size_t)L.filters * (L.bn ? 4 : 1);
        const float *w = p; p += (size_t)L.filters * L.cin * L.size * L.size;
        std::vector<float> in_sc;
        if (L.in_dt == DT_FP8) {
            channel_scales(c, L.in[0], in_sc);
            if ((int)in_sc.size() != L.cin) return fail(c, YOLO_ERR_STATE, "internal: scale vector of %zu for %d channels", in_sc.size(), L.cin);
        }
        std::vector<float> wperm;
        const Layer *PL = &L; Layer tmp;
        if (L.fc && L.fc_h * L.fc_w > 1) {
            const int hw = L.fc_h * L.fc_w, C = L.fc_c;
            wperm.resize((size_t)L.filters * L.cin);
            for (int o = 0; o < L.filters; ++o)
                for (int ch = 0; ch < C; ++ch)
                    for (int q = 0; q < hw; ++q) wperm[(size_t)o * L.cin + (size_t)q * C + ch] = w[(size_t)o * L.cin + (size_t)ch * hw + q];
            w = wperm.data();
        } else if (L.s2d7) {
            tmp = L; tmp.size = 4; tmp.cin = 32; PL = &tmp;
            wperm.assign((size_t)L.filters * 32 * 16, 0.f);
            for (int o = 0; o < L.filters; ++o)
                for (int ch = 0; ch < 3; ++ch)
                    for (int a4 = 0; a4 < 4; ++a4) for (int dy = 0; dy < 2; ++dy) { const int kh = 2 * a4 + dy - 1; if (kh < 0 || kh > 6) continue;
                        for (int b4 = 0; b4 < 4; ++b4) for (int dx = 0; dx < 2; ++dx) { const int kw = 2 * b4 + dx - 1; if (kw < 0 || kw > 6) continue;
                            wperm[(((size_t)o * 32 + (dy * 2 + dx) * 8 + ch) * 4 + a4) * 4 + b4] = w[(((size_t)o * 3 + ch) * 7 + kh) * 7 + kw]; } }
            w = wperm.data();
        }
        pack_conv(*PL, params, w, L.in_dt, in_sc.empty() ? nullptr : in_sc.data(), wbuf, bias, osc, c->semantics, !c->pair_of(L.in[0]) ? 0 : L.in[0] < 0 ? 1 : 2);
        HIPCK(c, hipMemcpy(L.d_w, wbuf.data(), wbuf.size(), hipMemcpyHostToDevice));
        HIPCK(c, hipMemcpy(L.d_b, bias.data(), bias.size() * 4, hipMemcpyHostToDevice));
        if (L.d_sc) HIPCK(c, hipMemcpy(L.d_sc, osc.data(), osc.size() * 4, hipMemcpyHostToDevice));
    }
    if (int rc = tail_fragments(c)) return rc;
    c->weights_loaded = true;
    return YOLO_OK;
}

int yolo_load_darknet_weights(yolo_ctx *c, const char *path, int header_ints)
{
    if (!c) return YOLO_ERR_INVALID;
    FILE *f = path ? fopen(path, "rb") : nullptr;
    if (!f) return fail(c, YOLO_ERR_IO, "cannot open weights file '%s'", path ? path : "(null)");
    int32_t ver[3];
    if (fread(ver, 4, 3, f) != 3) { fclose(f); return fail(c, YOLO_ERR_IO, "truncated header in '%s'", path); }
    if (header_ints == 0) header_ints = (ver[0] * 10 + ver[1]) >= 2 ? 5 : 4;
    if (header_ints != 4 && header_ints != 5) { fclose(f); return fail(c, YOLO_ERR_INVALID, "header_ints must be 0, 4 or 5"); }
    fseek(f, 0, SEEK_END); long end = ftell(f); fseek(f, header_ints * 4, SEEK_SET);
    size_t n = (size_t)(end - header_ints * 4) / 4;
    if (n != c->weights_count) { fclose(f); return fail(c, YOLO_ERR_IO, "'%s' holds %zu floats after a %d-int header, topology needs %zu", path, n, header_ints, c->weights_count); }
    std::vector<float> flat(n);
    size_t got = fread(flat.data(), 4, n, f); fclose(f);
    if (got != n) return fail(c, YOLO_ERR_IO, "short read on '%s'", path);
    return yolo_set_weights(c, flat.data(), n);
}

namespace {
struct ArtHeader { char magic[8]; uint32_t version, dtype, semantics, decode, n_layers, num_cfgs, cfg_len, reserved; };
const char kArtMagic[8] = {'Y', 'O', 'L', 'O', 'H', 'I', 'P', '1'};
const uint32_t kArtHasTrees = 1;
const uint32_t kArtVersion = 3;
uint64_t fnv1a(uint64_t h, const void *p, size_t n) { const uint8_t *b = (const uint8_t *)p; for (size_t i = 0; i < n; ++i) { h ^= b[i]; h *= 1099511628211ull; } return h; }
struct ArtWriter {
    FILE *f; uint64_t h = 1469598103934665603ull; bool ok = true;
    void put(const void *p, size_t n) { if (ok && n && fwrite(p, 1, n, f) != n) ok = false; h = fnv1a(h, p, n); }
};
struct ArtReader {
    FILE *f; uint64_t h = 1469598103934665603ull; bool ok = true;
    void get(void *p, size_t n) { if (ok && n && fread(p, 1, n, f) != n) ok = false; if (ok) h = fnv1a(h, p, n); }
};
}

int yolo_export(yolo_ctx *c, const char *path)
{
    if (!c) return YOLO_ERR_INVALID;
    if (!c->weights_loaded) return fail(c, YOLO_ERR_STATE, "yolo_export before weights were loaded");
    HIPCK(c, hipSetDevice(c->device)); HIPCK(c, hipStreamSynchronize(c->stream));
    FILE *f = path ? fopen(path, "wb") : nullptr;
    if (!f) return fail(c, YOLO_ERR_IO, "cannot create '%s'", path ? path : "(null)");
    ArtWriter w{f};
    const uint32_t NL = (uint32_t)c->layers.size();
    ArtHeader hd; memset(&hd, 0, sizeof hd); memcpy(hd.magic, kArtMagic, 8);
    hd.version = kArtVersion; hd.dtype = c->dtype; hd.semantics = c->semantics; hd.decode = c->decode; hd.n_layers = NL;
    hd.num_cfgs = (uint32_t)conv_num_cfgs(); hd.cfg_len = (uint32_t)c->cfg_text.size();
    hd.reserved = c->trees.empty() ? 0 : kArtHasTrees;
    w.put(&hd, sizeof hd); w.put(c->cfg_text.data(), c->cfg_text.size());
    std::vector<float> sc(c->user_scale); sc.resize(NL, 1.f); w.put(sc.data(), NL * 4);
    std::vector<int32_t> plan(NL); yolo_get_tile_configs(c, plan.data()); w.put(plan.data(), NL * 4);
    for (auto &t : c->trees) { const uint32_t len[2] = {(uint32_t)t.path.size(), (uint32_t)t.text.size()}; w.put(len, sizeof len); w.put(t.path.data(), t.path.size()); w.put(t.text.data(), t.text.size()); }
// ... 21 lines not shown
{
    auto bail = [&](yolo_ctx *c, const std::string &m) -> yolo_ctx * { if (err && err_len) snprintf(err, err_len, "%s", m.c_str()); if (c) yolo_destroy(c); return nullptr; };
    FILE *f = path ? fopen(path, "rb") : nullptr;
    if (!f) return bail(nullptr, std::string("cannot open '") + (path ? path : "(null)") + "'");
    ArtReader r{f};
    ArtHeader hd; r.get(&hd, sizeof hd);
    if (!r.ok || memcmp(hd.magic, kArtMagic, 8) != 0 || hd.version != kArtVersion || hd.cfg_len > (1u << 24) || hd.n_layers > 4096) { fclose(f); return bail(nullptr, "not a YOLOHIP1 artifact (or an unsupported version)"); }
    std::string cfg_text(hd.cfg_len, '\0'); r.get(&cfg_text[0], hd.cfg_len);
    std::vector<float> sc(hd.n_layers); r.get(sc.data(), (size_t)hd.n_layers * 4);
    std::vector<int32_t> plan(hd.n_layers); r.get(plan.data(), (size_t)hd.n_layers * 4);
    std::vector<std::pair<std::string, std::string>> trees;
    {
        std::vector<Section> secs; std::string perr;
        if (parse_cfg(cfg_text.c_str(), secs, perr))
            for (size_t i = 1; i < secs.size() && r.ok; ++i) {
                if ((secs[i].type != "region" && secs[i].type != "softmax") || !secs[i].kv.count("tree")) continue;
                if (!(hd.reserved & kArtHasTrees)) { fclose(f); return bail(nullptr, "the artifact's cfg names a softmax tree but the artifact carries none (exported before trees were served): export it again"); }
                uint32_t len[2] = {0, 0}; r.get(len, sizeof len);
                if (!r.ok || len[0] > (1u << 16) || len[1] > (1u << 26)) { r.ok = false; break; }
                std::string path(len[0], '\0'), text(len[1], '\0'); r.get(&path[0], len[0]); r.get(&text[0], len[1]);
                trees.emplace_back(path, text);
            }
    }
    if (!r.ok) { fclose(f); return bail(nullptr, "truncated artifact"); }
    yolo_config cfg; memset(&cfg, 0, sizeof cfg);
    cfg.struct_size = sizeof cfg; cfg.cfg_text = cfg_text.c_str(); cfg.max_batch = max_batch; cfg.dtype = (int)hd.dtype; cfg.semantics = (int)hd.semantics;
    cfg.decode = (int)hd.decode; cfg.device = device; cfg.keep_layers = keep_layers; cfg.stream = stream;
    g_tree_texts = &trees;
    yolo_ctx *c = yolo_create(&cfg, err, err_len);
    g_tree_texts = nullptr;
    if (!c) { fclose(f); return nullptr; }
    if (c->layers.size() != hd.n_layers) { fclose(f); return bail(c, "artifact layer count does not match its own cfg"); }
    if (c->dtype == YOLO_FP8 && yolo_set_act_scales(c, sc.data(), (int)hd.n_layers) != YOLO_OK) { fclose(f); return bail(c, c->err); }
    std::vector<uint8_t> buf;
    for (auto &L : c->layers) {
        if (L.type != L_CONV && L.type != L_LOCAL) continue;
        uint64_t sz[3]; r.get(sz, sizeof sz);
        uint64_t want[3] = {(uint64_t)L.cout_pad * L.kpad * dt_size(L.in_dt), (uint64_t)L.cout_pad, L.d_sc ? (uint64_t)L.cout_pad : 0};
        if (L.type == L_LOCAL) { want[0] = (uint64_t)L.H * L.W * L.filters * L.size * L.size * L.cin * dt_size(L.in_dt); want[1] = (uint64_t)L.H * L.W * L.filters; want[2] = 0; }
        if (!r.ok || sz[0] != want[0] || sz[1] != want[1] || sz[2] != want[2]) { fclose(f); return bail(c, "artifact parameters do not fit the topology (truncated file or different packing)"); }
        void *dst[3] = {L.d_w, L.d_b, L.d_sc}; const size_t bytes[3] = {(size_t)sz[0], (size_t)sz[1] * 4, (size_t)sz[2] * 4};
        for (int k = 0; k < 3; ++k) {
            if (!bytes[k]) continue;
            buf.resize(bytes[k]); r.get(buf.data(), bytes[k]);
            if (!r.ok) { fclose(f); return bail(c, "truncated artifact"); }
            if (hipMemcpy(dst[k], buf.data(), bytes[k], hipMemcpyHostToDevice) != hipSuccess) { fclose(f); return bail(c, "artifact upload failed"); }
        }
    }
    uint64_t sum = 0; const bool got = fread(&sum, 1, 8, f) == 8; fclose(f);
    if (!got || sum != r.h) return bail(c, "artifact checksum mismatch");
    if (tail_fragments(c) != YOLO_OK) return bail(c, c->err);
    c->weights_loaded = true;
    if (hd.num_cfgs == (uint32_t)conv_num_cfgs() && !keep_layers) { if (yolo_set_tile_configs(c, plan.data()) != YOLO_OK) { std::vector<int32_t> none(hd.n_layers, -1); yolo_set_tile_configs(c, none.data()); } }
    return c;
}

}
```

### yolo_tensorflow_amd/csrc/yolo_plan.cpp

```cpp
#include "yolo_ctx.h"

namespace yolo_impl {

bool parse_cfg(const char *text, std::vector<Section> &out, std::string &err)
{
    std::string s(text ? text : "");
    size_t pos = 0;
    while (pos <= s.size()) {
        size_t e = s.find('\n', pos); if (e == std::string::npos) e = s.size();
        std::string line = s.substr(pos, e - pos); pos = e + 1;
        size_t a = line.find_first_not_of(" \t\r"); if (a == std::string::npos) continue;
        size_t b = line.find_last_not_of(" \t\r"); line = line.substr(a, b - a + 1);
        if (line[0] == '#' || line[0] == ';') continue;
        if (line[0] == '[') {
            size_t r = line.find(']'); if (r == std::string::npos) { err = "cfg: unterminated section " + line; return false; }
            Section sec; sec.type = line.substr(1, r - 1); out.push_back(sec);
        } else {
            size_t eq = line.find('='); if (eq == std::string::npos || out.empty()) { err = "cfg: bad line '" + line + "'"; return false; }
            std::string k = line.substr(0, eq), v = line.substr(eq + 1);
            auto trim = [](std::string &t) { size_t x = t.find_first_not_of(" \t"); size_t y = t.find_last_not_of(" \t"); t = x == std::string::npos ? "" : t.substr(x, y - x + 1); };
            trim(k); trim(v); out.back().kv[k] = v;
        }
    }
    if (out.empty() || (out[0].type != "net" && out[0].type != "network")) { err = "cfg: first section must be [net]"; return false; }
    return true;
}
int opt_i(const Section &s, const char *k, int d) { auto it = s.kv.find(k); return it == s.kv.end() ? d : atoi(it->second.c_str()); }
std::string opt_s(const Section &s, const char *k, const char *d) { auto it = s.kv.find(k); return it == s.kv.end() ? std::string(d) : it->second; }
std::vector<float> opt_list(const Section &s, const char *k)
{
    std::vector<float> v; auto it = s.kv.find(k); if (it == s.kv.end()) return v;
    const char *p = it->second.c_str();
    while (*p) { char *e; double d = strtod(p, &e); if (e == p) break; v.push_back((float)d); p = e; while (*p == ',' || *p == ' ') ++p; }
    return v;
}

#define TREE_DESCENT_DEFAULT 0

static int plan_tree(yolo_ctx *c, int i, const char *section, const std::string &path, int want, const char *of)
{
    Tree t; std::string err;
    if (int r = load_tree(path, t, err)) return fail(c, r, "layer %d: [%s] %s", i, section, err.c_str());
    if (t.n != want) return fail(c, YOLO_ERR_INVALID, "layer %d: [%s] tree '%s' has %d nodes but the layer has %d %s", i, section, path.c_str(), t.n, want, of);
    c->trees.push_back(std::move(t)); c->layers[i].tree = (int)c->trees.size() - 1;
    return YOLO_OK;
}

TView view_of(const yolo_ctx *c, int idx) { return idx < 0 ? c->input : c->layers[idx].out; }

int build_plan(yolo_ctx *c, const std::vector<Section> &secs)
{
    const Section &net = secs[0];
    c->in_h = opt_i(net, "height", 0); c->in_w = opt_i(net, "width", 0); c->in_c = opt_i(net, "channels", 3);
// ... 358 lines not shown
    c->input.dt = c->dtype == YOLO_FP32 ? DT_F32 : (c->dtype == YOLO_FP16 || c->split()) ? DT_F16 : DT_BF16;
    const int in_stride = c->in_pair ? 24 : 8;
    size_t in_bytes = (size_t)c->max_batch * c->in_h * c->in_w * in_stride * dt_size(c->input.dt);
    HIPCK(c, hipMalloc(&c->input.ptr, in_bytes)); HIPCK(c, hipMemsetAsync(c->input.ptr, 0, in_bytes, c->stream));
    c->input.n = c->max_batch; c->input.h = c->in_h; c->input.w = c->in_w; c->input.c = 8; c->input.stride = in_stride;
    if (c->split()) {
        size_t cap = (size_t)c->max_batch * c->in_h * c->in_w * 8;
        for (auto &L : c->layers) if (L.type == L_UPSAMPLE || L.type == L_MAXPOOL || L.type == L_REORG) {
            const TView in = view_of(c, L.in[0]);
            cap = std::max(cap, (size_t)c->max_batch * in.h * in.w * roundup(in.c, 32));
            cap = std::max(cap, (size_t)c->max_batch * L.H * L.W * roundup(L.C, 32));
        }
        c->f32_cap = cap;
        HIPCK(c, hipMalloc((void **)&c->d_f32a, cap * 4)); HIPCK(c, hipMalloc((void **)&c->d_f32b, cap * 4));
    }
    HIPCK(c, hipMalloc(&c->d_zeros, 4096)); HIPCK(c, hipMemsetAsync(c->d_zeros, 0, 4096, c->stream));
    for (size_t i = 0; i < c->layers.size(); ++i) {
        const Layer &L = c->layers[i];
        if (L.s2d7 && c->split()) return fail(c, YOLO_ERR_UNSUPPORTED, "layer %zu: a 7x7 / stride 2 first conv is not served in the split-fp16 configuration", i);
        if (L.s2d7) {
            c->s2d = c->input; c->s2d.h = c->in_h / 2; c->s2d.w = c->in_w / 2; c->s2d.c = 32; c->s2d.stride = 32;
            HIPCK(c, hipMalloc(&c->s2d.ptr, (size_t)c->max_batch * c->s2d.h * c->s2d.w * 32 * dt_size(c->s2d.dt)));
        }
        if (L.fc) {
            const TView in = view_of(c, L.in[0]);
            if (in.stride != in.c || in.c != L.fc_c) return fail(c, YOLO_ERR_UNSUPPORTED, "layer %zu: [connected] needs a dense producer (channels a multiple of 8, not part of a concat)", i);
        }
    }
    c->stage_bytes = (size_t)c->max_batch * c->in_h * c->in_w * 3 * 4;
    HIPCK(c, hipMalloc(&c->d_stage, c->stage_bytes));
    HIPCK(c, hipMalloc((void **)&c->d_descs, (size_t)c->max_batch * sizeof(ImgDesc)));
    size_t nr = (size_t)c->max_batch * c->rows;
    if (c->cls_layer >= 0) {
        nr = 1;
        HIPCK(c, hipMalloc((void **)&c->d_cls_idx, (size_t)c->max_batch * CLS_TOPK_MAX * 4)); HIPCK(c, hipMalloc((void **)&c->d_cls_prob, (size_t)c->max_batch * CLS_TOPK_MAX * 4));
    }
    HIPCK(c, hipMalloc((void **)&c->d_det, nr * (c->attrs ? c->attrs : 1) * 4));
    HIPCK(c, hipMalloc((void **)&c->d_box4, nr * 16));
    HIPCK(c, hipMalloc(&c->d_lean_list, nr * 16)); HIPCK(c, hipMalloc((void **)&c->d_lean_cnt, 4)); HIPCK(c, hipMemsetAsync(c->d_lean_cnt, 0, 4, c->stream));
    for (auto &t : c->trees) if (int r = upload_tree(c, t)) return r;
    c->lean_ok = true;
    for (auto &L : c->layers) {
        if (L.type == L_REGION || L.type == L_DETECT) c->lean_ok = false;
        if (L.type == L_YOLO && L.na * (5 + L.classes) > 256) c->lean_ok = false;
    }
    c->tree_full = getenv("YOLO_TREE_FULL") ? true : getenv("YOLO_TREE_DESCENT") ? false : !TREE_DESCENT_DEFAULT;
    if (c->tree_head >= 0) c->lean_ok = !c->tree_full;
    c->lean_heads = 0;
    if (c->lean_ok) {
        int classes = -1; bool same = true;
        for (auto &L : c->layers) if (L.type == L_YOLO) { ++c->lean_heads; same = same && (classes < 0 || classes == L.classes) && L.na <= 16 && 5 + L.classes <= 128; classes = L.classes; }
        if (!same || (size_t)c->max_batch * c->rows * 340 >= 0xffffffffull) c->lean_heads = 0;
    }
    c->rows_pow2 = 1; while (c->rows_pow2 < c->rows) c->rows_pow2 <<= 1;
    HIPCK(c, hipMalloc((void **)&c->d_scores, nr * 4)); HIPCK(c, hipMalloc((void **)&c->d_labels, nr * 4));
    HIPCK(c, hipMalloc((void **)&c->d_cand, nr * 4)); HIPCK(c, hipMalloc((void **)&c->d_keys, (size_t)c->max_batch * c->rows_pow2 * 8));
    HIPCK(c, hipMalloc((void **)&c->d_sbox, nr * 16)); HIPCK(c, hipMalloc((void **)&c->d_slabel, nr * 4)); HIPCK(c, hipMalloc((void **)&c->d_sscore, nr * 4));
    HIPCK(c, hipMalloc((void **)&c->d_counts, (size_t)c->max_batch * 4));
    for (auto &L : c->layers) if (L.type == L_CONV) {
        size_t wb = (size_t)L.cout_pad * L.kpad * dt_size(L.in_dt);
        HIPCK(c, hipMalloc(&L.d_w, wb)); HIPCK(c, hipMemsetAsync(L.d_w, 0, wb, c->stream));
        HIPCK(c, hipMalloc((void **)&L.d_b, (size_t)L.cout_pad * 4)); HIPCK(c, hipMemsetAsync(L.d_b, 0, (size_t)L.cout_pad * 4, c->stream));
        if (L.in_dt == DT_FP8) { HIPCK(c, hipMalloc((void **)&L.d_sc, (size_t)L.cout_pad * 4)); HIPCK(c, hipMemsetAsync(L.d_sc, 0, (size_t)L.cout_pad * 4, c->stream)); }
    }
    for (auto &L : c->layers) if (L.type == L_LOCAL) {
        const size_t wn = (size_t)L.H * L.W * L.filters * L.size * L.size * L.cin;
        HIPCK(c, hipMalloc(&L.d_w, wn * dt_size(L.in_dt))); HIPCK(c, hipMalloc((void **)&L.d_b, (size_t)L.H * L.W * L.filters * 4));
    }
    if (c->dtype != YOLO_FP32)
        for (size_t i = 1; i < c->layers.size(); ++i) {
            const Layer &Y = c->layers[i]; Layer &P = c->layers[i - 1];
            if (Y.type == L_YOLO && P.type == L_CONV && P.head && !P.fc) HIPCK(c, hipMalloc((void **)&P.d_obj, (size_t)c->max_batch * P.H * P.W * Y.na * 4));
        }
    HIPCK(c, hipStreamSynchronize(c->stream));
    if (c->dtype != YOLO_FP32)
        for (size_t i = 0; i < c->layers.size(); ++i) {
            const Layer &L = c->layers[i];
            if (L.type != L_CONV || L.fc || L.s2d7 || window_check_skipped(L, (int)i)) continue;
            const TView in = view_of(c, L.in[0]);
            const double per_image = (double)in.h * in.w * in.stride * dt_size(L.in_dt), slack = 2.0 * (in.w + 1) * in.stride * dt_size(L.in_dt);
            if (per_image * c->max_batch + slack >= 2147483648.0)
                return fail(c, YOLO_ERR_UNSUPPORTED, "max_batch %d: layer %zu reads %.0f bytes per image%s, and a conv's whole-batch input must stay below 2 GiB (32-bit buffer offsets): at most %d images per context",
                            c->max_batch, i, per_image, c->split() ? " (split fp16 pairs: 2 x the channels)" : "", (int)((2147483648.0 - slack - 1) / per_image));
        }
    return YOLO_OK;
}

}
```

### yolo_tensorflow_amd/csrc/yolo_run.cpp

```cpp
#include "yolo_ctx.h"

namespace yolo_impl {

int fail(yolo_ctx *c, int code, const char *fmt, ...)
{
    char buf[512];
    va_list ap; va_start(ap, fmt); vsnprintf(buf, sizeof buf, fmt, ap); va_end(ap);
    if (c) c->err = buf;
    return code;
}

ConvArgs conv_args(const yolo_ctx *c, const Layer &L, int n)
{
    ConvArgs a; memset(&a, 0, sizeof a);
    TView in = view_of(c, L.in[0]);
    a.in = in.ptr; a.in_stride = in.stride; a.wt = L.d_w; a.bias = L.d_b;
    a.out = L.out.ptr; a.out_stride = L.out.stride; a.out_dt = L.out.dt; a.in_dt = L.in_dt; a.oscale = L.d_sc;
    if (L.pair || (c->split() && L.out.dt == DT_F32)) a.split = 1;
    a.pairk = L.in[0] >= 0 && c->pair_of(L.in[0]) ? 1 : 0;
    a.out_inv_scale = 1.f; a.res_scale = 1.f; a.mid_scale = 1.f; a.mid_inv_scale = 1.f;
    const int li = (int)(&L - c->layers.data());
    if (L.residual_from >= -1) { TView r = view_of(c, L.residual_from); a.res = r.ptr; a.res_stride = r.stride; }
    if (L.tail_on && L.tail_layer >= 0 && c->layers[L.tail_layer].in_dt == L.in_dt && (L.in_dt == DT_FP8 || c->layers[L.tail_layer].d_wf)) {
        const Layer &T = c->layers[L.tail_layer];
// ... 70 lines not shown
    b.N = n; b.H = B.H; b.W = B.W; b.C = B.filters; b.Cmid = A.filters; b.dt = B.in_dt;
    return b;
}
static C3S2Args c3s2_args(const yolo_ctx *c, int l, int n)
{
    const Layer &A = c->layers[l - 2], &B = c->layers[l]; const TView x = view_of(c, A.in[0]), r = view_of(c, A.residual_from); C3S2Args t; memset(&t, 0, sizeof t);
    t.in = x.ptr; t.in_stride = x.stride; t.w3 = A.d_w; t.b3 = A.d_b; t.Kpad3 = A.kpad; t.act3 = A.act; t.res = r.ptr; t.res_stride = r.stride;
    t.w5 = B.d_w; t.b5 = B.d_b; t.Kpad5 = B.kpad; t.act5 = B.act; t.out = B.out.ptr; t.out_stride = B.out.stride;
    t.N = n; t.H = A.H; t.W = A.W; t.dt = B.in_dt;
    return t;
}
static HaloArgs halo_args(const ConvArgs &a, const Layer &L, int n)
{
    HaloArgs h; memset(&h, 0, sizeof h);
    h.in = a.in; h.in_stride = a.in_stride; h.w = a.wt; h.b = a.bias; h.Kpad = a.Kpad; h.Cin = L.cin; h.Cout = L.filters; h.act = L.act;
    h.res = a.res; h.res_stride = a.res_stride; h.out = a.out; h.out_stride = a.out_stride; h.N = n; h.H = a.H; h.W = a.W; h.dt = L.in_dt;
    return h;
}

static bool fused_launch_applies(yolo_ctx *c, const Layer &L, int n)
{
    if (!fused_may_fall_back(L)) return L.fused != F_NONE;
    Layer &G = c->layers[L.launcher]; const int l = L.launcher;
    if (G.fuse_n != n) { G.fuse_ok = L.fused == F_RESBLOCK ? conv_resblock_ok(block_args(c, l, n)) : conv_c3s2_ok(c3s2_args(c, l, n)); G.fuse_n = n; }
    return G.fuse_ok;
}

static int run_conv(yolo_ctx *c, int i, int n)
{
    Layer &L = c->layers[i];
    hipStream_t s = c->stream;
    auto nview = [&](TView v) { v.n = n; return v; };
    if (fused_launch_applies(c, L, n)) {
        if (i == L.launcher) switch (L.fused) {
        case F_STEM: { StemArgs t = stem_args(c, i, n); HIPCK(c, launch_conv_stem(t, s)); break; }
        case F_PSTEM: { StemPairArgs t = stem_pair_args(c, i, n); if (c->input.stride != 24 || !conv_stem_pair_ok(t)) return fail(c, YOLO_ERR_STATE, "layer %d: the fused split-fp16 stem does not apply to this plan", i);
            HIPCK(c, launch_conv_stem_pair(t, s)); break; }
        case F_RESBLOCK: { BlockArgs b = block_args(c, i, n); HIPCK(c, launch_conv_resblock(b, s)); break; }
        case F_C3S2: { C3S2Args t = c3s2_args(c, i, n); HIPCK(c, launch_conv_c3s2(t, s)); break; }
        }
        return YOLO_OK;
    }
    if (rides_as_tail(c, L)) return YOLO_OK;
    ConvArgs a = conv_args(c, L, n);
    if (L.tail_on && !a.w2) return fail(c, YOLO_ERR_STATE, "layer %d: the plan folds the 1x1 conv %d into this layer, but its filters are not available in the producer's operand type", i, L.tail_layer);
    if (L.s2d7) HIPCK(c, launch_reorg(nview(c->input), nview(c->s2d), 2, 0, s));
    if (L.kernel != K_TILED) {
        HaloArgs h = halo_args(a, L, n);
        if (L.kernel == K_HALO && conv_halo_ok(h)) { HIPCK(c, launch_conv_halo(h, s)); return YOLO_OK; }
        if (L.kernel == K_S2 && conv_s2_ok(h)) { HIPCK(c, launch_conv_s2(h, s)); return YOLO_OK; }
    }
    if (c->dtype == YOLO_FP32) { HIPCK(c, launch_conv_f32(a, s)); return YOLO_OK; }
    const int cfg = conv_resolve_cfg(a, L.tile_cfg);
    if (a.w2 && !a.split && !a.pairk && !conv_cfg_tail_ok(cfg, a.Cout, a.in_dt == DT_FP8, a.tail_f32 != 0)) return fail(c, YOLO_ERR_STATE, "layer %d: tile config %d cannot run the fused 1x1 tail", i, cfg);
    HIPCK(c, a.in_dt == DT_FP8 ? launch_conv_fp8(a, cfg, s) : launch_conv_bf16(a, cfg, s));
    return YOLO_OK;
}

static int run_decode(yolo_ctx *c, int i, int n)
{
    const Layer &L = c->layers[i];
    hipStream_t s = c->stream;
    if (L.tree < 0 && c->lean && c->lean_thr > 0.f && c->lean_heads >= 1 && c->lean_heads <= 4) {
        bool later_head = false;
        for (size_t k = i + 1; k < c->layers.size(); ++k) later_head |= c->layers[k].type == L_YOLO;
        if (later_head) return YOLO_OK;
        LeanArgs la; memset(&la, 0, sizeof la);
        long begin = 0;
        for (size_t k = 0; k < c->layers.size(); ++k) {
            const Layer &Y = c->layers[k];
            if (Y.type != L_YOLO) continue;
            const Layer &P = c->layers[k - 1];
            LeanHead &h = la.h[la.nheads++];
            h.raw = (const float *)P.out.ptr; h.obj = P.d_obj; h.raw_stride = P.out.stride; h.g = Y.H; h.na = Y.na; h.row_off = Y.row_off; h.box_begin = begin;
            const int stride = c->in_h / Y.H;
            for (int q = 0; q < 2 * Y.na; ++q) h.anchors[q] = (float)(1.0 * (double)Y.anchors[q] / (double)stride);
            begin += (long)n * Y.H * Y.W * Y.na;
        }
        la.total = begin; la.n = n; la.classes = L.classes; la.img_size = c->in_h; la.mode = c->decode; la.rows_total = c->rows;
        la.box4 = c->d_box4; la.reject_below = c->lean_thr; la.list = (uint4 *)c->d_lean_list; la.list_count = c->d_lean_cnt; la.list_cap = (unsigned)((size_t)c->max_batch * c->rows);
        if (c->lean_cnt_dirty) HIPCK(c, hipMemsetAsync(c->d_lean_cnt, 0, 4, s));
        c->lean_cnt_dirty = true;
        HIPCK(c, launch_decode_lean(la, c->d_scores, c->d_labels, s));
        return YOLO_OK;
    }
    const Layer &P = c->layers[i - 1];
    DecodeArgs d; memset(&d, 0, sizeof d);
    d.raw = (const float *)P.out.ptr; d.raw_stride = P.out.stride; d.n = n; d.g = L.H; d.na = L.na; d.classes = L.classes;
    d.img_size = c->in_h; d.mode = c->decode; d.region = L.type == L_REGION;
    const int stride = c->in_h / L.H;
    for (int k = 0; k < 2 * L.na; ++k) d.anchors[k] = L.type == L_YOLO ? (float)(1.0 * (double)L.anchors[k] / (double)stride) : L.anchors[k];
    d.det = c->lean ? nullptr : c->d_det; d.box4 = c->lean ? c->d_box4 : nullptr; d.rows_total = c->rows; d.row_off = L.row_off;
    d.reject_below = c->lean ? c->lean_thr : -INFINITY;
    if (L.tree < 0) HIPCK(c, launch_decode(d, c->d_scores, c->d_labels, s));
    else if (c->lean) { HIPCK(c, launch_decode_region_tree_lean(d, c->trees[L.tree].dev, c->hier_thresh, c->d_scores, c->d_labels, s)); c->lean_hier = c->hier_thresh; }
    else HIPCK(c, launch_decode_region_tree(d, c->trees[L.tree].dev, s));
    return YOLO_OK;
}

int run_layer(yolo_ctx *c, int i, int n)
{
    Layer &L = c->layers[i];
    hipStream_t s = c->stream;
    auto nview = [&](TView v) { v.n = n; return v; };
    switch (L.type) {
    case L_CONV: return run_conv(c, i, n);
    case L_SHORTCUT:
        if (!L.noop && L.pair) {
            HIPCK(c, launch_add_split(view_of(c, L.in[0]).ptr, view_of(c, L.in[0]).stride, view_of(c, L.in[1]).ptr, view_of(c, L.in[1]).stride, L.out.ptr, L.out.stride, roundup(L.C, 32), (size_t)n * L.H * L.W, s));
        } else if (!L.noop) {
            float sa = 1.f, sb = 1.f, so = 1.f;
            if (c->dtype == YOLO_FP8) { sa = c->eff_scale[L.in[0]]; sb = c->eff_scale[L.in[1]]; so = 1.f / c->eff_scale[i]; }
            HIPCK(c, launch_add(nview(view_of(c, L.in[0])), nview(view_of(c, L.in[1])), nview(L.out), s, sa, sb, so));
        }
        break;
    case L_ROUTE:
// ... 31 lines not shown
            const TreeRows rows{(const float *)in.ptr, (size_t)n, 1, in.stride, 0, 0};
            HIPCK(c, launch_tree_softmax(c->trees[L.tree].dev, rows, L.temperature, i == c->cls_layer ? c->cls_mode : TREE_CONDITIONAL, a.probs, a.p_stride,
                                         a.top_k, a.cls, a.topk_probs, s));
            break;
        }
        if (P.type == L_AVGPOOL && P.pool_fused) {
            const TView in = nview(view_of(c, P.in[0]));
            if (!avgpool_softmax_ok(in, a)) return fail(c, YOLO_ERR_STATE, "layer %d: the fused [avgpool] + [softmax] launch does not apply to this plan", i);
            HIPCK(c, launch_avgpool_softmax(in, (float *)P.out.ptr, P.out.stride, a, s));
        } else {
            const TView in = view_of(c, L.in[0]);
            if (in.dt != DT_F32) return fail(c, YOLO_ERR_STATE, "layer %d: [softmax] input is not fp32", i);
            a.x = (const float *)in.ptr; a.x_stride = in.stride;
            HIPCK(c, launch_softmax_topk(a, s));
        }
        break; }
    case L_DETECT: {
        const Layer &P = c->layers[i - 1];
        HIPCK(c, launch_decode_v1((const float *)P.out.ptr, P.out.stride, n, L.side, L.na, L.classes, L.sqr, c->d_det, c->rows, L.row_off,
                                  c->d_scores, c->d_labels, s));
        break; }
    case L_YOLO: case L_REGION: return run_decode(c, i, n);
    }
    return YOLO_OK;
}

int stage_in(yolo_ctx *c, const void *images, int n, int fmt, int loc, float scale)
{
    if (n < 1 || n > c->max_batch) return fail(c, YOLO_ERR_INVALID, "batch %d outside 1..%d", n, c->max_batch);
    if (!images) return fail(c, YOLO_ERR_INVALID, "images == NULL");
    size_t npix = (size_t)n * c->in_h * c->in_w;
    const void *src = images;
    if (loc == YOLO_HOST) {
        HIPCK(c, hipMemcpyAsync(c->d_stage, images, npix * 3 * (fmt == YOLO_IMG_U8 ? 1 : 4), hipMemcpyHostToDevice, c->stream));
        src = c->d_stage;
    }
    c->stem_u8 = nullptr;
    if (fmt == YOLO_IMG_U8 && c->layers.size() > 1 && never_stored(c->layers[0], 0) && (double)npix * 3 < 2147483648.0 && ((size_t)src & 3) == 0) {
        c->stem_u8 = (const uint8_t *)src; c->stem_scale = scale; c->stem_u8_n = n;
        return YOLO_OK;
    }
    if (c->in_pair) {
        HIPCK(c, launch_preprocess(src, fmt, n, c->in_h * c->in_w, scale, c->d_f32a, DT_F32, 8, c->stream, c->in_mul, c->in_add));
        HIPCK(c, launch_split_from_f32(c->d_f32a, 8, c->input.ptr, 24, 8, npix, c->stream, PAIR_B3));
        return YOLO_OK;
    }
    HIPCK(c, launch_preprocess(src, fmt, n, c->in_h * c->in_w, scale, c->input.ptr, c->input.dt, 8, c->stream, c->in_mul, c->in_add));
    return YOLO_OK;
}

static int run_layers(yolo_ctx *c, int n, bool skip_conv = false, std::vector<hipEvent_t> *ev = nullptr)
{
    const int NL = (int)c->layers.size();
    for (int i = 0; i < NL; ++i) {
        if (!(skip_conv && c->layers[i].type == L_CONV)) { int r = run_layer(c, i, n); if (r) return r; }
        if (ev) HIPCK(c, hipEventRecord((*ev)[i + 1], c->stream));
    }
    return YOLO_OK;
}

int run_network(yolo_ctx *c, int n, bool lean)
{
    c->lean = lean && c->lean_ok;
    { int r = run_layers(c, n); if (r) { c->lean = false; return r; } }
    c->last_n = n; c->scores_mode = 0; c->det_valid = !c->lean;
    return YOLO_OK;
}

int output_layer(const yolo_ctx *c)
{
    int o = (int)c->layers.size() - 1;
    while (o >= 0 && c->layers[o].cost) --o;
    return o;
}

int need_detector(yolo_ctx *c, const char *what)
{
    if (c->cls_layer >= 0) return fail(c, YOLO_ERR_INVALID, "%s: the network is a classifier (its output layer is a [softmax], it has no detection head); use yolo_classify*", what);
    return YOLO_OK;
}

int post_args_ok(yolo_ctx *c, int max_out, int nms_mode, int select_mode)
{
    if (int r = need_detector(c, "threshold + NMS")) return r;
    if (max_out < 1) return fail(c, YOLO_ERR_INVALID, "max_out < 1");
    if (nms_mode < 0 || nms_mode > 4 || select_mode < 0 || select_mode > 1) return fail(c, YOLO_ERR_INVALID, "bad nms/select mode");
    return YOLO_OK;
}

int copy_out(yolo_ctx *c, void *dst, const void *src, size_t bytes, int loc)
{
    if (loc == YOLO_HOST) { HIPCK(c, hipMemcpyAsync(dst, src, bytes, hipMemcpyDeviceToHost, c->stream)); HIPCK(c, hipStreamSynchronize(c->stream)); }
    else HIPCK(c, hipMemcpyAsync(dst, src, bytes, hipMemcpyDeviceToDevice, c->stream));
    return YOLO_OK;
}

int post(yolo_ctx *c, const float *det, int n, int rows, int attrs, float score_thr, float iou_thr, int max_out,
         int nms_mode, int select_mode, int img_h, int img_w, int scores_ready, yolo_box *boxes_out, int32_t *counts_out, int out_loc, int32_t *rows_out,
         const PostGeom *geom)
{
    if (int r = post_args_ok(c, max_out, nms_mode, select_mode)) return r;
    size_t need = (size_t)n * max_out;
    if ((int)need > c->boxes_cap) {
        drop_graph(c);
        HIPCK(c, hipStreamSynchronize(c->stream));
        if (c->d_boxes) HIPCK(c, hipFree(c->d_boxes));
// ... 115 lines not shown
    c->scores_mode = want;
    return post(c, c->d_det, n, c->rows, c->attrs, score_thr, iou_thr, max_out, nms_mode, select_mode,
                nms_mode == YOLO_NMS_PER_CLASS ? c->in_h : 0, nms_mode == YOLO_NMS_PER_CLASS ? c->in_w : 0, ready, boxes_out, counts_out, out_loc, rows_out, geom);
}

int yolo_postprocess_rows(yolo_ctx *c, int n, float score_thr, float iou_thr, int max_out, int nms_mode, int select_mode,
                          yolo_box *boxes_out, int32_t *counts_out, int32_t *rows_out, int out_loc)
{
    if (!c) return YOLO_ERR_INVALID;
    return postprocess_impl(c, n, score_thr, iou_thr, max_out, nms_mode, select_mode, boxes_out, counts_out, rows_out, out_loc, nullptr);
}

int yolo_postprocess(yolo_ctx *c, int n, float score_thr, float iou_thr, int max_out, int nms_mode, int select_mode,
                     yolo_box *boxes_out, int32_t *counts_out, int out_loc)
{
    return yolo_postprocess_rows(c, n, score_thr, iou_thr, max_out, nms_mode, select_mode, boxes_out, counts_out, nullptr, out_loc);
}

int yolo_detect(yolo_ctx *c, const void *images, int n, int fmt, int loc, float scale, float score_thr, float iou_thr,
                int max_out, int nms_mode, int select_mode, yolo_box *boxes_out, int32_t *counts_out, int out_loc)
{
    if (!c) return YOLO_ERR_INVALID;
    if (int r = post_args_ok(c, max_out, nms_mode, select_mode)) return r;
    int r = forward_impl(c, images, n, fmt, loc, scale, nullptr, YOLO_DEVICE, nms_mode != YOLO_NMS_NUMPY_V3, score_thr); if (r) return r;
    return yolo_postprocess(c, n, score_thr, iou_thr, max_out, nms_mode, select_mode, boxes_out, counts_out, out_loc);
}

int yolo_detect_graph(yolo_ctx *c, const void *images, int n, int fmt, float scale, float score_thr, float iou_thr, int max_out,
                      int nms_mode, int select_mode, yolo_box *boxes_out, int32_t *counts_out)
{
    if (!c) return YOLO_ERR_INVALID;
    if (!images || !boxes_out || !counts_out) return fail(c, YOLO_ERR_INVALID, "yolo_detect_graph needs device pointers for images, boxes_out and counts_out");
    yolo_ctx::GKey k{images, n, fmt, scale, score_thr, iou_thr, max_out, nms_mode, select_mode, (void *)boxes_out, (void *)counts_out};
    if (memcmp(&k, &c->gkey, sizeof k) != 0) {
        if (c->gexec) { hipGraphExecDestroy(c->gexec); c->gexec = nullptr; }
        c->gkey = k; if (c->gstate >= 0) c->gstate = 0;
    }
    if (int r = post_args_ok(c, max_out, nms_mode, select_mode)) return r;
    auto eager = [&]() -> int {
        int r = forward_impl(c, images, n, fmt, YOLO_DEVICE, scale, nullptr, YOLO_DEVICE, nms_mode != YOLO_NMS_NUMPY_V3, score_thr); if (r) return r;
        return yolo_postprocess(c, n, score_thr, iou_thr, max_out, nms_mode, select_mode, boxes_out, counts_out, YOLO_DEVICE);
    };
    if (c->gstate <= 0) { int r = eager(); if (r == YOLO_OK && c->gstate == 0) c->gstate = 1; return r; }
    HIPCK(c, hipSetDevice(c->device));
    if (c->gstate == 1) {
        hipGraph_t g = nullptr;
        if (hipStreamBeginCapture(c->stream, hipStreamCaptureModeThreadLocal) != hipSuccess) { (void)hipGetLastError(); c->gstate = -1; return eager(); }
        int r = eager();
        hipError_t e = hipStreamEndCapture(c->stream, &g);
        if (r != YOLO_OK || e != hipSuccess || !g) { (void)hipGetLastError(); if (g) hipGraphDestroy(g); c->gstate = -1; return r ? r : eager(); }
        e = hipGraphInstantiate(&c->gexec, g, nullptr, nullptr, 0);
        hipGraphDestroy(g);
        if (e != hipSuccess) { (void)hipGetLastError(); c->gexec = nullptr; c->gstate = -1; return eager(); }
        c->gstate = 2;
    }
    if (c->lean_cnt_dirty) { HIPCK(c, hipMemsetAsync(c->d_lean_cnt, 0, 4, c->stream)); c->lean_cnt_dirty = false; }
    HIPCK(c, hipGraphLaunch(c->gexec, c->stream));
    c->lean = nms_mode != YOLO_NMS_NUMPY_V3 && c->lean_ok; c->det_valid = !c->lean; c->lean_thr = score_thr;
    c->last_n = n; c->scores_mode = nms_mode == YOLO_NMS_NUMPY_V3 ? 1 : 0;
    return YOLO_OK;
}

static_assert(sizeof(ImgDesc) == sizeof(yolo_image_desc) && sizeof(yolo_image_desc) == 16, "yolo_image_desc is the device table's row");

static int images_check(yolo_ctx *c, const void *pixels, size_t bytes, const yolo_image_desc *descs, int n, int fit)
{
    if (!c->weights_loaded) return fail(c, YOLO_ERR_STATE, "forward of images before weights were loaded");
    if (n < 1 || n > c->max_batch) return fail(c, YOLO_ERR_INVALID, "batch %d outside 1..%d", n, c->max_batch);
    if (!pixels || !descs) return fail(c, YOLO_ERR_INVALID, "pixels / descs == NULL");
    if (fit < YOLO_FIT_STRETCH || fit > YOLO_FIT_CV2_BGR) return fail(c, YOLO_ERR_INVALID, "bad fit %d", fit);
    if (bytes < 3 || bytes > 0xffffffffull) return fail(c, YOLO_ERR_INVALID, "packed buffer of %zu bytes (3 .. 2^32 - 1)", bytes);
    for (int i = 0; i < n; ++i) {
        const yolo_image_desc &d = descs[i];
        if (d.h < 1 || d.w < 1) return fail(c, YOLO_ERR_INVALID, "image %d: %d x %d", i, (int)d.h, (int)d.w);
        const uint64_t need = (uint64_t)d.h * (uint64_t)d.w * 3u;
        if (d.offset > bytes || need > bytes - d.offset)
            return fail(c, YOLO_ERR_INVALID, "image %d: %d x %d x 3 bytes at offset %llu end past the %zu-byte buffer", i, (int)d.h, (int)d.w, (unsigned long long)d.offset, bytes);
        if (fit == YOLO_FIT_LETTERBOX) {
            int nw, nh; letterbox_dims(c->in_w, c->in_h, d.w, d.h, &nw, &nh);
            if (nw < 1 || nh < 1) return fail(c, YOLO_ERR_INVALID, "image %d: %d x %d letterboxes to less than one pixel", i, (int)d.h, (int)d.w);
        }
    }
    return YOLO_OK;
}

static int detect_images_check(yolo_ctx *c, int fit, int max_out, int nms_mode, int select_mode, int units)
{
    if (int r = post_args_ok(c, max_out, nms_mode, select_mode)) return r;
    if (units != YOLO_UNITS_NETWORK && units != YOLO_UNITS_SOURCE_PIXELS) return fail(c, YOLO_ERR_INVALID, "bad units %d", units);
    if (fit == YOLO_FIT_LETTERBOX)
        for (auto &L : c->layers) if (L.type == L_DETECT) return fail(c, YOLO_ERR_UNSUPPORTED, "letterbox box mapping of a [detection] head (darknet v1 does not letterbox)");
    return YOLO_OK;
}

static int images_step(yolo_ctx *c, const uint8_t *pixels, size_t bytes, const yolo_image_desc *descs, int n, int fit, bool upload, bool lean, float score_thr)
{
    c->lean_thr = score_thr;
    if (upload) HIPCK(c, hipMemcpyAsync(c->d_descs, descs, (size_t)n * sizeof(ImgDesc), hipMemcpyHostToDevice, c->stream));
    c->stem_u8 = nullptr;
    if (c->in_pair) {
        HIPCK(c, launch_fit_images(pixels, bytes, c->d_descs, n, fit, c->in_h, c->d_f32a, DT_F32, 8, c->in_mul, c->in_add, c->stream));
        HIPCK(c, launch_split_from_f32(c->d_f32a, 8, c->input.ptr, 24, 8, (size_t)n * c->in_h * c->in_w, c->stream, PAIR_B3));
    } else HIPCK(c, launch_fit_images(pixels, bytes, c->d_descs, n, fit, c->in_h, c->input.ptr, c->input.dt, 8, c->in_mul, c->in_add, c->stream));
    if (int r = run_network(c, n, lean)) return r;
    c->geom_fit = fit; c->geom_n = n;
    return YOLO_OK;
}

static int forward_images_impl(yolo_ctx *c, const uint8_t *pixels, size_t bytes, const yolo_image_desc *descs, int n, int fit, int loc,
                               float *det_out, int out_loc, bool lean, float score_thr)
{
// ... 16 lines not shown
}

int yolo_forward_images_u8(yolo_ctx *c, const uint8_t *pixels, size_t bytes, const yolo_image_desc *descs, int n, int fit, int loc,
                           float *det_out, int out_loc)
{
    if (!c) return YOLO_ERR_INVALID;
    return forward_images_impl(c, pixels, bytes, descs, n, fit, loc, det_out, out_loc, false, 0.f);
}

int yolo_detect_images_u8(yolo_ctx *c, const uint8_t *pixels, size_t bytes, const yolo_image_desc *descs, int n, int fit, int loc,
                          float score_thr, float iou_thr, int max_out, int nms_mode, int select_mode, int units,
                          yolo_box *boxes_out, int32_t *counts_out, int out_loc)
{
    if (!c) return YOLO_ERR_INVALID;
    if (int r = detect_images_check(c, fit, max_out, nms_mode, select_mode, units)) return r;
    if (int r = forward_images_impl(c, pixels, bytes, descs, n, fit, loc, nullptr, YOLO_DEVICE, nms_mode != YOLO_NMS_NUMPY_V3, score_thr)) return r;
    const PostGeom g{fit, units == YOLO_UNITS_SOURCE_PIXELS};
    return postprocess_impl(c, n, score_thr, iou_thr, max_out, nms_mode, select_mode, boxes_out, counts_out, nullptr, out_loc, &g);
}

int yolo_detect_images_graph(yolo_ctx *c, const uint8_t *pixels, size_t bytes, const yolo_image_desc *descs, int n, int fit,
                             float score_thr, float iou_thr, int max_out, int nms_mode, int select_mode, int units,
                             yolo_box *boxes_out, int32_t *counts_out)
{
    if (!c) return YOLO_ERR_INVALID;
    if (!pixels || !boxes_out || !counts_out) return fail(c, YOLO_ERR_INVALID, "yolo_detect_images_graph needs device pointers for pixels, boxes_out and counts_out");
    if (int r = detect_images_check(c, fit, max_out, nms_mode, select_mode, units)) return r;
    if (int r = images_check(c, pixels, bytes, descs, n, fit)) return r;
    yolo_ctx::GKeyImages k; memset(&k, 0, sizeof k);
    k.pix = pixels; k.bytes = bytes; k.n = n; k.fit = fit; k.units = units; k.st = score_thr; k.it = iou_thr; k.mo = max_out; k.nm = nms_mode; k.sm = select_mode;
    k.bo = (void *)boxes_out; k.co = (void *)counts_out;
    if (memcmp(&k, &c->gkey_img, sizeof k) != 0) {
        if (c->gexec_img) { hipGraphExecDestroy(c->gexec_img); c->gexec_img = nullptr; }
        c->gkey_img = k; if (c->gstate_img >= 0) c->gstate_img = 0;
    }
    HIPCK(c, hipSetDevice(c->device));
    HIPCK(c, hipMemcpyAsync(c->d_descs, descs, (size_t)n * sizeof(ImgDesc), hipMemcpyHostToDevice, c->stream));
    const PostGeom g{fit, units == YOLO_UNITS_SOURCE_PIXELS};
    const bool lean = nms_mode != YOLO_NMS_NUMPY_V3;
    auto eager = [&]() -> int {
        if (int r = images_step(c, pixels, bytes, descs, n, fit, false, lean, score_thr)) return r;
        return postprocess_impl(c, n, score_thr, iou_thr, max_out, nms_mode, select_mode, boxes_out, counts_out, nullptr, YOLO_DEVICE, &g);
    };
    if (c->gstate_img <= 0) { int r = eager(); if (r == YOLO_OK && c->gstate_img == 0) c->gstate_img = 1; return r; }
    if (c->gstate_img == 1) {
        hipGraph_t gr = nullptr;
        if (hipStreamBeginCapture(c->stream, hipStreamCaptureModeThreadLocal) != hipSuccess) { (void)hipGetLastError(); c->gstate_img = -1; return eager(); }
        int r = eager();
        hipError_t e = hipStreamEndCapture(c->stream, &gr);
        if (r != YOLO_OK || e != hipSuccess || !gr) { (void)hipGetLastError(); if (gr) hipGraphDestroy(gr); c->gstate_img = -1; return r ? r : eager(); }
        e = hipGraphInstantiate(&c->gexec_img, gr, nullptr, nullptr, 0);
        hipGraphDestroy(gr);
        if (e != hipSuccess) { (void)hipGetLastError(); c->gexec_img = nullptr; c->gstate_img = -1; return eager(); }
        c->gstate_img = 2;
    }
    if (c->lean_cnt_dirty) { HIPCK(c, hipMemsetAsync(c->d_lean_cnt, 0, 4, c->stream)); c->lean_cnt_dirty = false; }
    HIPCK(c, hipGraphLaunch(c->gexec_img, c->stream));
    c->lean = lean && c->lean_ok; c->det_valid = !c->lean; c->lean_thr = score_thr;
    c->last_n = n; c->scores_mode = nms_mode == YOLO_NMS_NUMPY_V3 ? 1 : 0; c->stem_u8 = nullptr; c->geom_fit = fit; c->geom_n = n;
    return YOLO_OK;
}

static int classify_check(yolo_ctx *c, int top_k, const int32_t *classes_out, const float *probs_out)
{
    if (c->cls_layer < 0) return fail(c, YOLO_ERR_INVALID, "yolo_classify: the network is a detector (its output layer is not a [softmax])");
    const Layer &L = c->layers[c->cls_layer];
    if (top_k < 0 || top_k > CLS_TOPK_MAX || top_k > L.C) return fail(c, YOLO_ERR_INVALID, "top_k %d outside 0..%d", top_k, L.C < CLS_TOPK_MAX ? L.C : CLS_TOPK_MAX);
    if (top_k > 0 && L.groups != 1) return fail(c, YOLO_ERR_INVALID, "top_k needs a [softmax] with groups=1 (this one has groups=%d)", L.groups);
    if (!probs_out || (top_k > 0 && !classes_out)) return fail(c, YOLO_ERR_INVALID, "classes_out / probs_out == NULL");
    return YOLO_OK;
}

static int classify_out(yolo_ctx *c, int n, int top_k, int32_t *classes_out, float *probs_out, int out_loc)
{
    const Layer &L = c->layers[c->cls_layer];
    if (top_k == 0) return copy_out(c, probs_out, L.out.ptr, (size_t)n * L.C * 4, out_loc);
    if (int r = copy_out(c, classes_out, c->d_cls_idx, (size_t)n * top_k * 4, out_loc)) return r;
    return copy_out(c, probs_out, c->d_cls_prob, (size_t)n * top_k * 4, out_loc);
}

int yolo_classify(yolo_ctx *c, const void *images, int n, int fmt, int loc, float scale, int top_k, int32_t *classes_out, float *probs_out, int out_loc)
{
    if (!c) return YOLO_ERR_INVALID;
    if (int r = classify_check(c, top_k, classes_out, probs_out)) return r;
    c->cls_topk = top_k; c->cls_mode = c->hierarchy_mode;
    const int r = forward_impl(c, images, n, fmt, loc, scale, nullptr, YOLO_DEVICE, false);
    c->cls_topk = 0; c->cls_mode = 0;
    if (r) return r;
    return classify_out(c, n, top_k, classes_out, probs_out, out_loc);
}

int yolo_classify_images_u8(yolo_ctx *c, const uint8_t *pixels, size_t bytes, const yolo_image_desc *descs, int n, int fit, int loc, int top_k,
                            int32_t *classes_out, float *probs_out, int out_loc)
{
    if (!c) return YOLO_ERR_INVALID;
    if (int r = classify_check(c, top_k, classes_out, probs_out)) return r;
    c->cls_topk = top_k; c->cls_mode = c->hierarchy_mode;
    const int r = forward_images_impl(c, pixels, bytes, descs, n, fit, loc, nullptr, YOLO_DEVICE, false, 0.f);
    c->cls_topk = 0; c->cls_mode = 0;
    if (r) return r;
    return classify_out(c, n, top_k, classes_out, probs_out, out_loc);
}

float yolo_fit_unit_value(int fit, int value)
{
    if (fit < YOLO_FIT_STRETCH || fit > YOLO_FIT_CV2_BGR || value < 0 || value > 255) return NAN;
    return fit_unit_value(fit, (unsigned)value);
}

namespace { struct EventSet {
    std::vector<hipEvent_t> e; bool ok = true;
    explicit EventSet(int n) { e.reserve(n); for (int i = 0; i < n; ++i) { hipEvent_t x; if (hipEventCreate(&x) != hipSuccess) { ok = false; break; } e.push_back(x); } }
    ~EventSet() { for (auto x : e) hipEventDestroy(x); }
    EventSet(const EventSet &) = delete; EventSet &operator=(const EventSet &) = delete;
}; }

int yolo_time_forward(yolo_ctx *c, int n, int iters, float *total_ms, float *conv_ms)
{
    if (!c) return YOLO_ERR_INVALID;
    if (!c->weights_loaded) return fail(c, YOLO_ERR_STATE, "weights not loaded");
    if (n < 1 || n > c->max_batch || iters < 1) return fail(c, YOLO_ERR_INVALID, "bad n/iters");
    HIPCK(c, hipSetDevice(c->device));
    EventSet evs(2); if (!evs.ok) return fail(c, YOLO_ERR_HIP, "hipEventCreate failed");
    hipEvent_t e0 = evs.e[0], e1 = evs.e[1];
    c->lean = false;
    if (c->stem_u8 && n > c->stem_u8_n) c->stem_u8 = nullptr;
    if (total_ms) {
        HIPCK(c, hipEventRecord(e0, c->stream));
        for (int it = 0; it < iters; ++it) { int r = run_network(c, n); if (r) return r; }
        HIPCK(c, hipEventRecord(e1, c->stream)); HIPCK(c, hipEventSynchronize(e1));
        float ms = 0; HIPCK(c, hipEventElapsedTime(&ms, e0, e1)); *total_ms = ms / iters;
    }
    if (conv_ms) {
        float all_ms = 0, rest_ms = 0;
        for (int pass = 0; pass < 2; ++pass) {
            HIPCK(c, hipEventRecord(e0, c->stream));
            for (int it = 0; it < iters; ++it) { int r = run_layers(c, n, pass == 1); if (r) return r; }
            HIPCK(c, hipEventRecord(e1, c->stream)); HIPCK(c, hipEventSynchronize(e1));
            float ms = 0; HIPCK(c, hipEventElapsedTime(&ms, e0, e1)); (pass == 0 ? all_ms : rest_ms) = ms / iters;
        }
        *conv_ms = all_ms - rest_ms;
        c->last_n = n; c->scores_mode = 0; c->det_valid = true;
    }
    return YOLO_OK;
}

int yolo_time_layers(yolo_ctx *c, int n, int iters, float *ms_out)
{
    if (!c || !ms_out) return YOLO_ERR_INVALID;
    if (!c->weights_loaded) return fail(c, YOLO_ERR_STATE, "weights not loaded");
    if (n < 1 || n > c->max_batch || iters < 1) return fail(c, YOLO_ERR_INVALID, "bad n/iters");
    HIPCK(c, hipSetDevice(c->device));
    const int NL = (int)c->layers.size();
    c->lean = false; c->det_valid = true;
    if (c->stem_u8 && n > c->stem_u8_n) c->stem_u8 = nullptr;
    EventSet evs(NL + 1); if (!evs.ok) return fail(c, YOLO_ERR_HIP, "hipEventCreate failed");
    std::vector<hipEvent_t> &ev = evs.e;
    std::vector<double> acc(NL, 0.0);
    for (int it = 0; it < iters; ++it) {
        HIPCK(c, hipEventRecord(ev[0], c->stream));
        for (int i = 0; i < NL; ++i) { int r = run_layer(c, i, n); if (r) return r; HIPCK(c, hipEventRecord(ev[i + 1], c->stream)); }
        HIPCK(c, hipStreamSynchronize(c->stream));
        for (int i = 0; i < NL; ++i) { float ms = 0; HIPCK(c, hipEventElapsedTime(&ms, ev[i], ev[i + 1])); acc[i] += ms; }
    }
    for (int i = 0; i < NL; ++i) ms_out[i] = (float)(acc[i] / iters);
    c->last_n = n;
    return YOLO_OK;
}

}
```

### yolo_tensorflow_amd/csrc/yolo_tune.cpp

```cpp
#include "yolo_ctx.h"
#include "conv_cfgs.h"

template <int... I> static constexpr bool in_every_family(CfgList<I...>) { return ((Cfgs16::has(I) && CfgsFp8::has(I) && CfgsSplit::has(I) && CfgsPairK::has(I) && CfgsPairKPlain::has(I)) && ...); }
static_assert(in_every_family(CfgList<0, 2, 4, 6, 8, 14>{}), "every id conv_default_cfg returns is instantiated for every storage family");

int conv_default_cfg(const ConvArgs &a)
{
    if (a.split || a.pairk ? conv_c8_direct_pair_ok(a) : conv_c8_direct_ok(a)) return CONV_CFG_DIRECT;
    const long M = (long)a.N * a.Ho * a.Wo;
    if (a.Cout <= 32) return 4;
    if (a.Cout <= 64) return M >= 65536 ? 8 : 6;
    const long tiles128 = ((M + 127) / 128) * ((a.Cout + 127) / 128);
    if (tiles128 < 512) return M < 8192 && tiles128 < 128 ? 14 : 2;
    return 0;
}

bool conv_cfg_runs(const ConvArgs &a, int cfg)
{
    if (a.split || a.pairk) {
        if (conv_c8_direct_pair_ok(a) || cfg == CONV_CFG_DIRECT) return cfg == CONV_CFG_DIRECT && conv_c8_direct_pair_ok(a);
        if (conv_cfg_is_halo(cfg) && a.out_dt == DT_F32) return false;
    } else if (cfg == CONV_CFG_DIRECT) return conv_c8_direct_ok(a);
    return conv_cfg_is_halo(cfg) ? conv_halo_cfg_ok(a, cfg) : conv_cfg_instantiated(a, cfg);
}
// ... 53 lines not shown
        }
    }
    for (int i = 0; i < NL; ++i) {
        Layer &L = c->layers[i];
        if (L.type != L_CONV || fixed_kernel(L)) continue;
        auto it = score.find(shape_key(L));
        int best = fallback[i]; double bt = 1e30;
        if (it != score.end()) for (auto &kv : it->second) if (kv.second < bt) { bt = kv.second; best = kv.first; }
        L.tile_cfg = best;
    }
    {
        int r = yolo_time_layers(c, n, iters, ms.data()); if (r) return r;
        std::vector<float> base(ms);
        std::vector<int> base_cfg(NL, -1);
        for (int i = 0; i < NL; ++i) base_cfg[i] = c->layers[i].tile_cfg;
        std::map<std::string, std::pair<double, int>> best;
        auto tail_key = [&](const Layer &L) { return shape_key(L) + (c->layers[L.tail_layer].head ? "_head" : ""); };
        for (int i = 0; i < NL; ++i) {
            const Layer &L = c->layers[i];
            if (L.type != L_CONV || L.tail_layer < 0) continue;
            auto &b = best[tail_key(L)];
            if (b.second == 0 && b.first == 0) b = {0.0, -1};
            b.first += base[i] + base[L.tail_layer];
        }
        for (int cfg = 0; cfg < conv_num_cfgs(); ++cfg) {
            bool any = false;
            for (int i = 0; i < NL; ++i) {
                Layer &L = c->layers[i];
                if (L.type != L_CONV || L.tail_layer < 0) continue;
                const bool ok = conv_cfg_tail_ok(cfg, L.filters, L.in_dt == DT_FP8, c->layers[L.tail_layer].head) && c->layers[L.tail_layer].in_dt == L.in_dt && valid(L, cfg);
                L.tile_cfg = ok ? cfg : base_cfg[i]; L.tail_on = ok; any |= ok;
            }
            if (!any) continue;
            r = yolo_time_layers(c, n, iters, ms.data()); if (r) return r;
            std::map<std::string, double> t;
            for (int i = 0; i < NL; ++i) {
                const Layer &L = c->layers[i];
                if (L.type == L_CONV && L.tail_layer >= 0 && L.tail_on) t[tail_key(L)] += ms[i] + ms[L.tail_layer];
            }
            for (auto &kv : t) {
                auto &b = best[kv.first];
                if (getenv("YOLO_TUNE_VERBOSE")) fprintf(stderr, "tune-tail %s cfg %d %-16s fused pair %.4f ms (unfused best so far %.4f)\n", kv.first.c_str(), cfg, conv_cfg_name(cfg), kv.second, b.first);
                if (kv.second < b.first) b = {kv.second, cfg};
            }
        }
        for (int i = 0; i < NL; ++i) {
            Layer &L = c->layers[i];
            if (L.type != L_CONV || L.tail_layer < 0) continue;
            const auto &b = best[tail_key(L)];
            L.tail_on = b.second >= 0; L.tile_cfg = b.second >= 0 ? b.second : base_cfg[i];
        }
    }
    drop_graph(c);
    return YOLO_OK;
}

int yolo_get_tile_configs(const yolo_ctx *c, int32_t *cfgs)
{
    if (!c || !cfgs) return YOLO_ERR_INVALID;
    for (size_t i = 0; i < c->layers.size(); ++i) {
        const Layer &L = c->layers[i];
        cfgs[i] = L.type == L_CONV ? (L.tail_on && L.tile_cfg >= 0 ? L.tile_cfg + 10000 : L.tile_cfg) : -1;
    }
    return YOLO_OK;
}

int yolo_set_tile_configs(yolo_ctx *c, const int32_t *cfgs)
{
    if (!c || !cfgs) return YOLO_ERR_INVALID;
    for (size_t i = 0; i < c->layers.size(); ++i) {
        if (c->layers[i].type != L_CONV) continue;
        int v = cfgs[i]; bool tail = false;
        if (v >= 10000) { v -= 10000; tail = true; }
        if (v != -1 && v != CONV_CFG_DIRECT && (v < 0 || v >= conv_num_cfgs())) return fail(c, YOLO_ERR_INVALID, "layer %zu: tile config %d out of range", i, v);
        if (tail && (c->layers[i].tail_layer < 0 || !conv_cfg_tail_ok(v, c->layers[i].filters, c->layers[i].in_dt == DT_FP8, c->layers[c->layers[i].tail_layer].head) || c->layers[c->layers[i].tail_layer].in_dt != c->layers[i].in_dt))
            return fail(c, YOLO_ERR_INVALID, "layer %zu: plan asks for a fused 1x1 tail this layer / tile config cannot run", i);
        if (tail && fixed_kernel(c->layers[i])) return fail(c, YOLO_ERR_INVALID, "layer %zu runs a fixed kernel (stem / conv3 / block / stride-2): it hosts no fused 1x1 tail", i);
        if (tail && conv_cfg_is_halo(v) && !conv_cfg_runs(conv_args(c, c->layers[i], c->max_batch), v))
            return fail(c, YOLO_ERR_INVALID, "layer %zu: the halo-staged tile config %d does not apply to this layer, so it cannot carry the fused 1x1 tail", i, v);
        c->layers[i].tile_cfg = v; c->layers[i].tail_on = tail;
    }
    drop_graph(c);
    return YOLO_OK;
}

}
```

### yolo_tensorflow_amd/hip.py

```python
import ctypes as C
import os
import numpy as np

_HERE = os.path.dirname(os.path.abspath(__file__))
LIB_OVERRIDE = os.environ.get("YOLO_HIP_LIB") or None
LIB_PATH = LIB_OVERRIDE or os.path.join(_HERE, "libyolo_hip.so")

BF16, FP32, FP8, FP16, FP16X2 = 0, 1, 2, 3, 4
SEM_TF, SEM_DARKNET = 0, 1
DECODE_RATIO, DECODE_PIXEL = 0, 1
HOST, DEVICE = 0, 1
IMG_U8, IMG_F32, IMG_F32_CHW = 0, 1, 2
NMS_TF, NMS_PER_CLASS, NMS_DARKNET, NMS_NUMPY_V3, NMS_TF_V1 = 0, 1, 2, 3, 4
SELECT_GT, SELECT_GE = 0, 1
FIT_STRETCH, FIT_LETTERBOX, FIT_CV2, FIT_CV2_BGR = 0, 1, 2, 3
UNITS_NETWORK, UNITS_SOURCE_PIXELS = 0, 1

BOX_DTYPE = np.dtype([("x0", "<f4"), ("y0", "<f4"), ("x1", "<f4"), ("y1", "<f4"), ("score", "<f4"), ("cls", "<i4")])
DESC_DTYPE = np.dtype([("offset", "<u8"), ("h", "<i4"), ("w", "<i4")])


class ImageDesc(C.Structure):
    _fields_ = [("offset", C.c_uint64), ("h", C.c_int32), ("w", C.c_int32)]

EXPORTS = [
    "yolo_create", "yolo_destroy", "yolo_last_error", "yolo_load_darknet_weights", "yolo_set_weights",
    "yolo_weights_count", "yolo_set_act_scales", "yolo_export", "yolo_create_from_file", "yolo_input_size", "yolo_num_rows", "yolo_num_attrs", "yolo_num_layers", "yolo_head_geometry",
    "yolo_conv_flops", "yolo_conv_bytes", "yolo_forward", "yolo_forward_image_u8", "yolo_postprocess",
    "yolo_detect", "yolo_detect_graph", "yolo_synchronize", "yolo_layer_output", "yolo_time_forward", "yolo_time_layers",
    "yolo_autotune", "yolo_get_tile_configs", "yolo_set_tile_configs", "yolo_op_conv2d", "yolo_op_conv_num_cfgs", "yolo_op_upsample2x", "yolo_op_reorg",
    "yolo_darknet_boxes", "yolo_last_layer_size", "yolo_last_layer_output", "yolo_op_letterbox",
    "yolo_op_maxpool", "yolo_op_resize_u8", "yolo_op_detections_boxes", "yolo_op_nms_detections", "yolo_forward_letterbox_chw", "yolo_op_decode", "yolo_op_postprocess",
    "yolo_postprocess_rows", "yolo_op_postprocess_rows", "yolo_last_layer_output_batch", "yolo_head_raw", "yolo_calibrate", "yolo_calibrate_copy", "yolo_op_resize_cv2",
    "yolo_forward_images_u8", "yolo_detect_images_u8", "yolo_detect_images_graph", "yolo_fit_unit_value", "yolo_darknet_boxes_at",
    "yolo_num_classes", "yolo_classify", "yolo_classify_images_u8", "yolo_op_avgpool", "yolo_op_softmax",
    "yolo_set_hier_thresh", "yolo_set_hierarchy_mode", "yolo_darknet_boxes_map", "yolo_tree_geometry", "yolo_tree_read", "yolo_plan_check", "yolo_plan_table",
    "yolo_op_tree_softmax", "yolo_op_tree_top",
]
HIER_CONDITIONAL, HIER_ABSOLUTE, HIER_LEAVES = 0, 1, 2
_HIER_MODES = {None: HIER_CONDITIONAL, "conditional": HIER_CONDITIONAL, "absolute": HIER_ABSOLUTE, "leaves": HIER_LEAVES}
DIST_EXPORTS = ["yolo_shard_bounds", "yolo_dist_flat_words", "yolo_dist_split_records", "yolo_dist_unique_id", "yolo_dist_create",
                "yolo_dist_detect", "yolo_dist_detect_async", "yolo_dist_destroy"]


class YoloError(RuntimeError):
    pass


class _Config(C.Structure):
    _fields_ = [("struct_size", C.c_uint32), ("cfg_text", C.c_char_p), ("max_batch", C.c_int32),
                ("dtype", C.c_int32), ("semantics", C.c_int32), ("decode", C.c_int32), ("device", C.c_int32),
                ("keep_layers", C.c_int32), ("stream", C.c_void_p)]


_lib = None


def load_library():
    global _lib
    if _lib is not None:
        return _lib
    if not os.path.exists(LIB_PATH):
        raise YoloError("%s is missing -- build it with `python -c 'import __graft_entry__ as g; g.build()'` "
                        "(or `make -C yolo_tensorflow_amd/csrc`); there is no CPU fallback" % LIB_PATH)
    l = C.CDLL(LIB_PATH)
    P, I, F, D = C.c_void_p, C.c_int, C.c_float, C.c_double
    FP = C.POINTER(C.c_float)
    l.yolo_create.argtypes = [C.POINTER(_Config), C.c_char_p, C.c_size_t]; l.yolo_create.restype = P
    l.yolo_destroy.argtypes = [P]; l.yolo_destroy.restype = None
    l.yolo_last_error.argtypes = [P]; l.yolo_last_error.restype = C.c_char_p
    l.yolo_load_darknet_weights.argtypes = [P, C.c_char_p, I]
    l.yolo_set_weights.argtypes = [P, FP, C.c_size_t]
    l.yolo_weights_count.argtypes = [P]; l.yolo_weights_count.restype = C.c_size_t
    l.yolo_set_act_scales.argtypes = [P, P, I]
    l.yolo_head_geometry.argtypes = [P, I, P, P, P, P]
    l.yolo_export.argtypes = [P, C.c_char_p]
    l.yolo_create_from_file.argtypes = [C.c_char_p, I, I, P, I, C.c_char_p, C.c_size_t]; l.yolo_create_from_file.restype = P
    l.yolo_input_size.argtypes = [P, C.POINTER(I), C.POINTER(I), C.POINTER(I)]
    for n in ("yolo_num_rows", "yolo_num_attrs", "yolo_num_layers", "yolo_synchronize", "yolo_num_classes"):
        getattr(l, n).argtypes = [P]
    l.yolo_conv_flops.argtypes = [P]; l.yolo_conv_flops.restype = D
    l.yolo_conv_bytes.argtypes = [P, I]; l.yolo_conv_bytes.restype = D
    l.yolo_forward.argtypes = [P, P, I, I, I, F, P, I]
    l.yolo_forward_image_u8.argtypes = [P, P, I, I, I, P, I]
    l.yolo_postprocess.argtypes = [P, I, F, F, I, I, I, P, P, I]
    l.yolo_detect.argtypes = [P, P, I, I, I, F, F, F, I, I, I, P, P, I]
    l.yolo_detect_graph.argtypes = [P, P, I, I, F, F, F, I, I, I, P, P]
    l.yolo_layer_output.argtypes = [P, I, I, P, C.c_size_t, C.POINTER(I)]
    l.yolo_time_forward.argtypes = [P, I, I, FP, FP]
    l.yolo_time_layers.argtypes = [P, I, I, FP]
    l.yolo_autotune.argtypes = [P, I, I]
    l.yolo_get_tile_configs.argtypes = [P, P]
    l.yolo_set_tile_configs.argtypes = [P, P]
    l.yolo_op_conv2d.argtypes = [P, I, I, I, I, P, P, I, I, I, I, P, P, I, I, I]
    l.yolo_op_conv_num_cfgs.argtypes = []
    l.yolo_op_upsample2x.argtypes = [P, I, I, I, I, I, P, I]
    l.yolo_op_reorg.argtypes = [P, I, I, I, I, I, I, P, I]
    l.yolo_op_maxpool.argtypes = [P, I, I, I, I, I, I, P, I]
    l.yolo_op_resize_u8.argtypes = [P, I, I, I, F, P, I]
    l.yolo_op_detections_boxes.argtypes = [P, I, I, I, P, I]
    l.yolo_op_nms_detections.argtypes = [P, P, P, I, I, F, I, I]
    l.yolo_forward_letterbox_chw.argtypes = [P, P, I, I, I, P, I]
    l.yolo_op_decode.argtypes = [P, I, I, I, I, P, I, I, I, P, I]
    l.yolo_darknet_boxes.argtypes = [P, I, I, F, I, P, I, P]
    l.yolo_last_layer_size.argtypes = [P]; l.yolo_last_layer_size.restype = C.c_size_t
    l.yolo_last_layer_output.argtypes = [P, P, C.c_size_t]
    l.yolo_op_letterbox.argtypes = [P, I, I, I, I, I, P, I]
    l.yolo_op_postprocess.argtypes = [P, I, I, I, F, F, I, I, I, P, P, I]
    l.yolo_op_postprocess_rows.argtypes = [P, I, I, I, F, F, I, I, I, P, P, P, I]
    l.yolo_postprocess_rows.argtypes = [P, I, F, F, I, I, I, P, P, P, I]
    l.yolo_last_layer_output_batch.argtypes = [P, I, P, C.c_size_t]
    l.yolo_head_raw.argtypes = [P, I, I, P, C.c_size_t]
    l.yolo_calibrate.argtypes = [I, P, I, C.c_double, FP, FP]
    l.yolo_calibrate_copy.argtypes = [I, P, C.c_double, FP]
    l.yolo_op_resize_cv2.argtypes = [P, I, I, I, I, I, F, P, I]
    SZ = C.c_size_t
    l.yolo_forward_images_u8.argtypes = [P, P, SZ, P, I, I, I, P, I]
    l.yolo_detect_images_u8.argtypes = [P, P, SZ, P, I, I, I, F, F, I, I, I, I, P, P, I]
    l.yolo_detect_images_graph.argtypes = [P, P, SZ, P, I, I, F, F, I, I, I, I, P, P]
    l.yolo_fit_unit_value.argtypes = [I, I]; l.yolo_fit_unit_value.restype = F
    l.yolo_darknet_boxes_at.argtypes = [P, I, I, I, F, I, P, I, P]
    l.yolo_classify.argtypes = [P, P, I, I, I, F, I, P, P, I]
    l.yolo_classify_images_u8.argtypes = [P, P, SZ, P, I, I, I, I, P, P, I]
    l.yolo_op_avgpool.argtypes = [P, I, I, I, I, I, P, I]
    l.yolo_op_softmax.argtypes = [P, I, I, I, F, I, P, P, P, I]
    l.yolo_set_hier_thresh.argtypes = [P, F]
    l.yolo_set_hierarchy_mode.argtypes = [P, I]
    l.yolo_darknet_boxes_map.argtypes = [P, I, I, I, F, I, P, P, I, P]
    l.yolo_tree_geometry.argtypes = [P, P, P, P, P, P, P, P]
    l.yolo_tree_read.argtypes = [C.c_char_p, P, P, P, P, P, P, P, C.c_char_p, SZ]
    l.yolo_plan_check.argtypes = [C.c_char_p, I, C.c_char_p, SZ]
    l.yolo_plan_table.argtypes = [C.c_char_p, I, I, I, C.c_char_p, SZ, C.c_char_p, SZ]
    l.yolo_op_tree_softmax.argtypes = [P, I, I, C.c_char_p, F, I, P, I]
    l.yolo_op_tree_top.argtypes = [P, I, C.c_char_p, F, P, I]
    l.yolo_shard_bounds.argtypes = [I, I, I, C.POINTER(I), C.POINTER(I)]
    l.yolo_dist_flat_words.argtypes = [I, I]; l.yolo_dist_flat_words.restype = C.c_size_t
    l.yolo_dist_split_records.argtypes = [P, I, I, I, P, P]
    l.yolo_dist_unique_id.argtypes = [P]
    l.yolo_dist_create.argtypes = [P, I, I, P, P, I, I, C.c_char_p, C.c_size_t]; l.yolo_dist_create.restype = P
    l.yolo_dist_detect.argtypes = [P, P, I, F, F, F, I, I, P, P]
    l.yolo_dist_detect_async.argtypes = [P, P, I, F, F, F, I, I, C.POINTER(P)]
    l.yolo_dist_destroy.argtypes = [P]; l.yolo_dist_destroy.restype = None
    _lib = l
    return l


def _ptr(a):
    if a is None:
        return None, HOST
    if isinstance(a, int):
        return C.c_void_p(a), DEVICE
    if isinstance(a, np.ndarray):
        if not a.flags["C_CONTIGUOUS"]:
            raise YoloError("array must be C-contiguous")
        return C.c_void_p(a.ctypes.data), HOST
    if hasattr(a, "data_ptr"):
        if not a.is_contiguous():
            raise YoloError("tensor must be contiguous")
        return C.c_void_p(a.data_ptr()), (DEVICE if a.is_cuda else HOST)
    raise YoloError("unsupported buffer type %r" % type(a))


def _op_check(rc, what):
    if rc != 0:
        msg = load_library().yolo_last_error(None)
        raise YoloError("%s failed (%d): %s" % (what, rc, msg.decode() if msg else ""))


_warned_legacy = False
HIP_STREAM_LEGACY = 1


def pack_images(images):
    arrs = []
    for i, im in enumerate(images):
        a = np.ascontiguousarray(im)
        if a.dtype != np.uint8 or a.ndim != 3 or a.shape[2] != 3 or a.shape[0] < 1 or a.shape[1] < 1:
            raise YoloError("image %d: need a uint8 [h, w, 3] array, got %s %s" % (i, a.dtype, a.shape))
        arrs.append(a)
    if not arrs:
        raise YoloError("pack_images: no images")
    descs = np.zeros(len(arrs), dtype=DESC_DTYPE)
    off = 0
    for i, a in enumerate(arrs):
        descs[i] = (off, a.shape[0], a.shape[1])
        off += a.size
    buf = np.empty(off, dtype=np.uint8)
# ... 583 lines not shown
```

Baseline: 12630 img/s.

## Skip storing head conv outputs for cells below the objectness score threshold

Adds a pruning epilogue to the tiled head conv. It computes objectness per anchor, stages pass/fail flags in idle LDS, and writes the full attribute rows only for cells whose objectness sigmoid clears the detect threshold. Spare padded output channels are packed with duplicate objectness filters so every channel tile can see its anchor's objectness. The aim is to cut head output write traffic. In exchange it adds a barrier and a second epilogue pass, and head tensors become invalid for later raw-output queries, which now return an error.

```diff
diff --git a/include/yolo_hip.h b/include/yolo_hip.h
--- a/include/yolo_hip.h
+++ b/include/yolo_hip.h
@@ -183,6 +183,8 @@
                    int32_t *leaf, char *err, size_t err_len);
 int yolo_plan_check(const char *cfg_text, int dtype, char *err, size_t err_len);
 int yolo_plan_table(const char *cfg_text, int dtype, int max_batch, int keep_layers, char *out, size_t out_len, char *err, size_t err_len);
+int yolo_head_prune_plan(int cout, int attrs, int anchors, int bc, int cout_pad, int32_t *spare_src);
+int yolo_head_pack_spares(void *filters, size_t row_bytes, float *bias, int cout, int attrs, int anchors, int bc, int cout_pad);
 int yolo_op_tree_softmax(const float *x, int n, int len, const char *tree_path, float temperature, int mode, float *out, int device);
 int yolo_op_tree_top(const float *x_logits, int n, const char *tree_path, float hier_thresh, int32_t *labels_out, int device);
 
diff --git a/yolo_tensorflow_amd/csrc/conv_cfgs.h b/yolo_tensorflow_amd/csrc/conv_cfgs.h
--- a/yolo_tensorflow_amd/csrc/conv_cfgs.h
+++ b/yolo_tensorflow_amd/csrc/conv_cfgs.h
@@ -57,9 +57,12 @@
 using CfgsPairK = CfgList<0, 2, 3, 4, 6, 7, 8, 14, 15, 16, 23, 33, 34, 45, 49, 52>;
 using CfgsHaloPairK = CfgList<40, 41, 43, 57, 58>;
 using CfgsPairKPlain = CfgList<0, 2, 4, 6, 8, 14, 16, 33>;
+using CfgsHeadPrune = CfgList<16, 17, 44>;
 
 template <int... I> constexpr bool cfgs_are(CfgList<I...>, bool halo) { return ((I >= 0 && I < kNumCfgs && kCfgs[I].halo == halo) && ...); }
 static_assert(cfgs_are(Cfgs16{}, false) && cfgs_are(CfgsFp8{}, false) && cfgs_are(CfgsSplit{}, false) && cfgs_are(CfgsPairK{}, false) && cfgs_are(CfgsPairKPlain{}, false), "tiled lists hold tiled ids");
+template <int... I> constexpr bool cfgs_prune_shaped(CfgList<I...>) { return ((Cfgs16::has(I) && kCfgs[I].nl == 0 && kCfgs[I].wc * kCfgs[I].tc * 16 >= 128) && ...); }
+static_assert(cfgs_are(CfgsHeadPrune{}, false) && cfgs_prune_shaped(CfgsHeadPrune{}), "pruning heads: symmetric tiled 16-bit shapes of >= 128 channels");
 static_assert(cfgs_are(CfgsHalo16{}, true) && cfgs_are(CfgsHaloFp8{}, true) && cfgs_are(CfgsHaloSplit{}, true) && cfgs_are(CfgsHaloPairK{}, true), "halo lists hold halo ids");
 
 inline bool conv_cfg_instantiated(const ConvArgs &a, int cfg)
diff --git a/yolo_tensorflow_amd/csrc/conv_igemm.hip b/yolo_tensorflow_amd/csrc/conv_igemm.hip
--- a/yolo_tensorflow_amd/csrc/conv_igemm.hip
+++ b/yolo_tensorflow_amd/csrc/conv_igemm.hip
@@ -166,7 +166,7 @@
     return names.s[cfg];
 }
 
-template <int WP, int WC, int TP, int TC, int NS, int BK, int NL, bool UNI, int EB, bool H16 = false, bool SPLIT = false>
+template <int WP, int WC, int TP, int TC, int NS, int BK, int NL, bool UNI, int EB, bool H16 = false, bool SPLIT = false, bool HEADP = false>
 static hipError_t launch_u(const ConvArgs &a, hipStream_t s)
 {
     constexpr int BP = WP * TP * 16, BC = WC * TC * 16;
@@ -175,27 +175,35 @@
     constexpr size_t lds = conv_lds_bytes<WP, WC, TP, TC, NS, BK, NL>();
     dim3 grid((unsigned)((tiles + 7) / 8 * 8)), block(64 * (WP * WC + NL));
     if (lds > 65536) {
-        hipError_t e = conv_opt_in_lds((const void *)conv_igemm<WP, WC, TP, TC, NS, BK, UNI, NL, false, EB, false, false, H16, SPLIT>, lds);
+        hipError_t e = conv_opt_in_lds((const void *)conv_igemm<WP, WC, TP, TC, NS, BK, UNI, NL, false, EB, false, false, H16, SPLIT, HALO_B, HALO_B, false, false, HEADP>, lds);
         if (e != hipSuccess) return e;
     }
-    hipLaunchKernelGGL((conv_igemm<WP, WC, TP, TC, NS, BK, UNI, NL, false, EB, false, false, H16, SPLIT>), grid, block, lds, s, conv_tile_magic(a, BC, 0));
+    hipLaunchKernelGGL((conv_igemm<WP, WC, TP, TC, NS, BK, UNI, NL, false, EB, false, false, H16, SPLIT, HALO_B, HALO_B, false, false, HEADP>), grid, block, lds, s, conv_tile_magic(a, BC, 0));
     return hipGetLastError();
 }
 
-template <int WP, int WC, int TP, int TC, int NS, int BK, int NL, int EB, bool H16 = false, bool SPLIT = false>
+template <int WP, int WC, int TP, int TC, int NS, int BK, int NL, int EB, bool H16 = false, bool SPLIT = false, bool HEADP = false>
 static hipError_t launch_t(const ConvArgs &a, hipStream_t s)
 {
     if (((double)a.N * a.H * a.W * a.in_stride + 2.0 * (a.W + 1) * a.in_stride) * EB >= 2147483648.0) return hipErrorInvalidValue;
     constexpr int BKE = BK * 2 / EB;
     if (a.Kpad % BKE) return hipErrorInvalidValue;
-    return (a.Cin_pad % BKE) == 0 ? launch_u<WP, WC, TP, TC, NS, BK, NL, true, EB, H16, SPLIT>(a, s) : launch_u<WP, WC, TP, TC, NS, BK, NL, false, EB, H16, SPLIT>(a, s);
-}
-
-template <int ID, int EB, bool H16 = false, bool SPLIT = false>
+    return (a.Cin_pad % BKE) == 0 ? launch_u<WP, WC, TP, TC, NS, BK, NL, true, EB, H16, SPLIT, HEADP>(a, s) : launch_u<WP, WC, TP, TC, NS, BK, NL, false, EB, H16, SPLIT, HEADP>(a, s);
+}
+
+template <int ID, int EB, bool H16 = false, bool SPLIT = false, bool HEADP = false>
 static hipError_t launch_id(const ConvArgs &a, hipStream_t s)
 {
     constexpr ConvCfg c = kCfgs[ID];
-    return launch_t<c.wp, c.wc, c.tp, c.tc, c.ns, c.bk, c.nl, EB, H16, SPLIT>(a, s);
+    return launch_t<c.wp, c.wc, c.tp, c.tc, c.ns, c.bk, c.nl, EB, H16, SPLIT, HEADP>(a, s);
+}
+
+int conv_head_prune_bc(int cfg) { return CfgsHeadPrune::has(cfg) ? kCfgs[cfg].wc * kCfgs[cfg].tc * 16 : 0; }
+bool conv_head_prune_ok(const ConvArgs &a, int cfg)
+{
+    const int bc = conv_head_prune_bc(cfg);
+    return bc > 0 && (a.in_dt == DT_BF16 || a.in_dt == DT_F16) && !a.split && !a.pairk && a.out_dt == DT_F32 && !a.res && !a.w2 && a.obj_out && a.obj_na >= 1 && a.obj_na <= 16 &&
+           head_prunable(a.Cout, a.obj_attrs, a.obj_na, bc, (a.Cout + 255) / 256 * 256, nullptr);
 }
 
 hipError_t launch_conv_bf16(const ConvArgs &a, int cfg, hipStream_t s)
@@ -211,6 +219,11 @@
     }
     if (cfg == CONV_CFG_DIRECT) return conv_c8_direct_ok(a) ? launch_conv_c8_direct(a, s) : hipErrorInvalidValue;
     if (conv_cfg_is_halo(cfg)) return launch_conv_halo13(a, cfg, s);
+    if (a.prune_below > 0.f) {
+        if (!conv_head_prune_ok(a, cfg)) return hipErrorInvalidValue;
+        if (a.in_dt == DT_F16) return cfg_dispatch(CfgsHeadPrune{}, cfg, [&](auto id) { return launch_id<decltype(id)::value, 2, true, false, true>(a, s); });
+        return cfg_dispatch(CfgsHeadPrune{}, cfg, [&](auto id) { return launch_id<decltype(id)::value, 2, false, false, true>(a, s); });
+    }
     if (a.in_dt == DT_F16) return cfg_dispatch(Cfgs16{}, cfg, [&](auto id) { return launch_id<decltype(id)::value, 2, true>(a, s); });
     return cfg_dispatch(Cfgs16{}, cfg, [&](auto id) { return launch_id<decltype(id)::value, 2>(a, s); });
 }
diff --git a/yolo_tensorflow_amd/csrc/conv_igemm_kernel.h b/yolo_tensorflow_amd/csrc/conv_igemm_kernel.h
--- a/yolo_tensorflow_amd/csrc/conv_igemm_kernel.h
+++ b/yolo_tensorflow_amd/csrc/conv_igemm_kernel.h
@@ -76,7 +76,7 @@
 constexpr unsigned halo_div_mul(int bw) { return (65536u + bw - 1) / bw; }
 constexpr bool halo_div_ok(int bw) { for (unsigned r = 0; r < 256; ++r) if (((r * halo_div_mul(bw)) >> 16) != r / bw) return false; return true; }
 
-template <int WP, int WC, int TP, int TC, int NS, int BK, bool UNI, int NL = 0, bool DIAG = false, int EB = 2, bool HALO = false, bool FREE = false, bool H16 = false, bool SPLIT = false, int BH = HALO_B, int BW = HALO_B, bool HEADT = false, bool PAIRK = false>
+template <int WP, int WC, int TP, int TC, int NS, int BK, bool UNI, int NL = 0, bool DIAG = false, int EB = 2, bool HALO = false, bool FREE = false, bool H16 = false, bool SPLIT = false, int BH = HALO_B, int BW = HALO_B, bool HEADT = false, bool PAIRK = false, bool HEADP = false>
 __global__ __launch_bounds__(64 * (WP * WC + NL)) void conv_igemm(const ConvArgs a)
 {
 #if defined(__HIP_DEVICE_COMPILE__)
@@ -91,6 +91,7 @@
     static_assert(!H16 || EB == 2, "fp16 is a 16-bit storage type");
     static_assert(!SPLIT || (H16 && !DIAG), "split pairs are fp16 pairs");
     static_assert(!PAIRK || (H16 && EB == 2 && BK == 64 && UNI && !DIAG && NL == 0), "pair K loop: fp16, 128-byte rows = one 32-channel group hi | lo, uniform taps");
+    static_assert(!HEADP || (!HALO && !SPLIT && !PAIRK && !HEADT && !DIAG && EB == 2 && NL == 0 && BC >= 128), "pruning head epilogue: symmetric tiled 16-bit form, tiles of at least 128 channels");
     constexpr int RB = BK * 2;
     constexpr int EPC = 16 / EB;
     constexpr int BKE = RB / EB;
@@ -957,6 +958,63 @@
                 }
             }
         }
+    } else if constexpr (HEADP) {
+        constexpr int FP = 16;
+        static_assert(BP * FP <= STAGE_BYTES, "the flags fit the idle stage");
+        char *const flags = smem + (KT % NS) * STAGE_BYTES;
+        const int c0 = ct * BC;
+        const int a_lo = fast_div(c0, a.obj_mul, a.obj_shift);
+        const int sp_an = a_lo * a.obj_attrs + 4 < c0 ? a_lo : -1;
+        if (is_consumer) {
+#pragma unroll
+            for (int i = 0; i < TC; ++i) {
+                const int ch = c0 + (wci * TC + i) * 16 + lq * 4;
+                const float4 bv = *(const float4 *)(a.bias + ch);
+                const float bq[4] = {bv.x, bv.y, bv.z, bv.w};
+#pragma unroll
+                for (int q = 0; q < 4; ++q) {
+                    const int an = fast_div(ch + q, a.obj_mul, a.obj_shift);
+                    const bool real = ch + q < a.Cout && ch + q - an * a.obj_attrs == 4, spare = ch + q == a.Cout && sp_an >= 0;
+                    if (!real && !spare) continue;
+                    const int fa = real ? an : sp_an;
+#pragma unroll
+                    for (int j = 0; j < TP; ++j) {
+                        const int p = (wpi * TP + j) * 16 + l15, m = pt * BP + p;
+                        float v = acc[i][j][q] + bq[q];
+                        if (a.act == ACT_LEAKY) v = fmaxf(v, 0.1f * v);
+                        flags[p * FP + fa] = !(sigmoid_fast(v) < a.prune_below) ? 1 : 0;
+                        if (real && m < M) a.obj_out[(size_t)m * a.obj_na + an] = v;
+                    }
+                }
+            }
+        }
+        asm volatile("s_waitcnt lgkmcnt(0)" ::: "memory");
+        block_barrier();
+        if (is_consumer) {
+#pragma unroll
+            for (int i = 0; i < TC; ++i) {
+                const int ch = c0 + (wci * TC + i) * 16 + lq * 4;
+                if (ch >= a.Cout) continue;
+                const float4 bv = *(const float4 *)(a.bias + ch);
+                const int last = ch + 3 < a.Cout ? ch + 3 : a.Cout - 1;
+                const int f0 = fast_div(ch, a.obj_mul, a.obj_shift), f1 = fast_div(last, a.obj_mul, a.obj_shift);
+#pragma unroll
+                for (int j = 0; j < TP; ++j) {
+                    const int p = (wpi * TP + j) * 16 + l15, m = pt * BP + p;
+                    if (m >= M) continue;
+                    if (!(flags[p * FP + f0] | flags[p * FP + f1])) continue;
+                    float v[4] = {acc[i][j][0] + bv.x, acc[i][j][1] + bv.y, acc[i][j][2] + bv.z, acc[i][j][3] + bv.w};
+                    if (a.act == ACT_LEAKY) {
+#pragma unroll
+                        for (int q = 0; q < 4; ++q) v[q] = fmaxf(v[q], 0.1f * v[q]);
+                    }
+                    float *o = (float *)a.out + (size_t)m * a.out_stride + ch;
+                    if (ch + 3 < a.Cout) *(float4 *)o = float4{v[0], v[1], v[2], v[3]};
+                    else
+                        for (int q = 0; q < 4; ++q) if (ch + q < a.Cout) o[q] = v[q];
+                }
+            }
+        }
     } else if (is_consumer && !HALO) {
 #pragma unroll
         for (int i = 0; i < TC; ++i) {
diff --git a/yolo_tensorflow_amd/csrc/kernels.h b/yolo_tensorflow_amd/csrc/kernels.h
--- a/yolo_tensorflow_amd/csrc/kernels.h
+++ b/yolo_tensorflow_amd/csrc/kernels.h
@@ -64,6 +64,7 @@
     int C2out;
     int tail_f32;
     uint32_t tc_mul, tc_shift, bpi_mul, bpi_shift, bpr_mul, bpr_shift;
+    float prune_below;
 };
 inline int conv_kchunk(int cin_pad, int wdt) { const int row = wdt == DT_FP8 ? 128 : 64; return (wdt != DT_F32 && cin_pad % row == 0) ? row : cin_pad; }
 inline void conv_magic(uint32_t d, uint32_t &mul, uint32_t &shift)
@@ -79,6 +80,10 @@
     conv_magic((uint32_t)(a.Ho * a.Wo), a.howo_mul, a.howo_shift);
     conv_magic((uint32_t)a.Wo, a.wo_mul, a.wo_shift);
 }
+bool head_prunable(int cout, int attrs, int na, int bc, int cout_pad, int *spare_src);
+bool head_pack_spares(void *w, size_t row_bytes, float *bias, int cout, int attrs, int na, int bc, int cout_pad);
+int conv_head_prune_bc(int cfg);
+bool conv_head_prune_ok(const ConvArgs &a, int cfg);
 inline ConvArgs conv_tile_magic(const ConvArgs &a0, int BC, int bh, int bw = 0)
 {
     ConvArgs a = a0;
@@ -239,6 +244,11 @@
     float reject_below;
 };
 #ifdef __HIPCC__
+__device__ __forceinline__ float sigmoid_fast(float x)
+{
+    const float e = __builtin_amdgcn_exp2f(-x * 1.44269504088896340736f);
+    return __builtin_amdgcn_rcpf(1.0f + e);
+}
 __device__ __forceinline__ float region_sigmoid(float x) { return 1.0f / (1.0f + expf(-x)); }
 __device__ __forceinline__ float region_box_attr(int k, const float *p, int cell, int g, const float *anchor_wh)
 {
diff --git a/yolo_tensorflow_amd/csrc/post_ops.hip b/yolo_tensorflow_amd/csrc/post_ops.hip
--- a/yolo_tensorflow_amd/csrc/post_ops.hip
+++ b/yolo_tensorflow_amd/csrc/post_ops.hip
@@ -5,11 +5,6 @@
 struct BoxOut { float x0, y0, x1, y1, score; int cls; };
 
 __device__ __forceinline__ float sigmoidf_(float x) { return 1.0f / (1.0f + expf(-x)); }
-__device__ __forceinline__ float sigmoid_fast(float x)
-{
-    const float e = __builtin_amdgcn_exp2f(-x * 1.44269504088896340736f);
-    return __builtin_amdgcn_rcpf(1.0f + e);
-}
 
 __device__ __forceinline__ float yolo_box_attr(int k, float x, int cx, int cy, const float *anchor, float G, float S, int mode)
 {
diff --git a/yolo_tensorflow_amd/csrc/yolo_api.cpp b/yolo_tensorflow_amd/csrc/yolo_api.cpp
--- a/yolo_tensorflow_amd/csrc/yolo_api.cpp
+++ b/yolo_tensorflow_amd/csrc/yolo_api.cpp
@@ -1,4 +1,11 @@
 #include "yolo_ctx.h"
+
+static int heads_intact(yolo_ctx *c, const char *what)
+{
+    if (c->heads_pruned)
+        return fail(c, YOLO_ERR_STATE, "%s: the last forward ran through yolo_detect* with score threshold %g and its head convs stored only the boxes at or above it; the whole tensor needs yolo_forward", what, c->lean_thr);
+    return YOLO_OK;
+}
 
 extern "C" {
 
@@ -168,6 +175,7 @@
         HIPCK(c, hipSetDevice(c->device));
         return copy_out(c, out, S.out.ptr, (size_t)n * S.C * 4, YOLO_HOST);
     }
+    if (int r = heads_intact(c, "yolo_last_layer_output")) return r;
     const int li = output_layer(c);
     if (li < 1 || (c->layers[li].type != L_YOLO && c->layers[li].type != L_REGION && c->layers[li].type != L_DETECT))
         return fail(c, YOLO_ERR_UNSUPPORTED, "the last layer is not a detection head");
@@ -198,6 +206,7 @@
     if (!c || !out || head < 0) return YOLO_ERR_INVALID;
     if (int r = need_detector(c, "yolo_head_raw")) return r;
     if (c->last_n < 1 || n < 1 || n > c->last_n) return fail(c, YOLO_ERR_STATE, "yolo_head_raw of %d images but the last forward ran %d", n, c->last_n);
+    if (int r = heads_intact(c, "yolo_head_raw")) return r;
     int k = 0;
     for (size_t li = 1; li < c->layers.size(); ++li) {
         const Layer &L = c->layers[li];
@@ -222,6 +231,7 @@
     if (!c) return YOLO_ERR_INVALID;
     if (index < 0 || index >= (int)c->layers.size() || n < 1 || n > c->last_n) return fail(c, YOLO_ERR_INVALID, "bad layer index / n");
     const Layer &L = c->layers[index];
+    if (L.type == L_CONV && L.head) if (int r = heads_intact(c, "yolo_layer_output of a head conv")) return r;
     if (!c->keep_layers) {
         bool kept = L.type == L_CONV && L.storage >= 0 && L.residual_from < -1 && !never_stored(L, index);
         if (kept) for (const Storage &o : c->storages) if (&o != &c->storages[L.storage] && o.phys == c->storages[L.storage].phys && o.def > c->storages[L.storage].def) kept = false;
diff --git a/yolo_tensorflow_amd/csrc/yolo_ctx.h b/yolo_tensorflow_amd/csrc/yolo_ctx.h
--- a/yolo_tensorflow_amd/csrc/yolo_ctx.h
+++ b/yolo_tensorflow_amd/csrc/yolo_ctx.h
@@ -35,6 +35,7 @@
     int residual_from = -2;
     bool head = false;
     float *d_obj = nullptr;
+    int prune_bc = 0;
     int kernel = K_TILED;
     int fused = F_NONE, launcher = -1;
     int fuse_n = 0; bool fuse_ok = false;
@@ -87,6 +88,7 @@
     bool lean_cnt_dirty = false;
     void *d_lean_list = nullptr; unsigned *d_lean_cnt = nullptr;
     float *d_box4 = nullptr; bool lean = false, det_valid = false, lean_ok = false; float lean_thr = 0.f; int lean_heads = 0;
+    bool prune_on = false, heads_pruned = false, graph_pruned = false, graph_img_pruned = false;
     float *d_scores = nullptr; int *d_labels = nullptr; int *d_cand = nullptr; unsigned long long *d_keys = nullptr;
     float4 *d_sbox = nullptr; int *d_slabel = nullptr; float *d_sscore = nullptr; int rows_pow2 = 0;
     void *d_boxes = nullptr; int *d_counts = nullptr; int boxes_cap = 0;
@@ -137,6 +139,7 @@
 inline bool input_never_loaded(const Layer &L, int i) { return L.fused != F_NONE && L.fused != F_PSTEM && i >= L.launcher; }
 inline bool fixed_kernel(const Layer &L) { return L.kernel != K_TILED || L.fused != F_NONE; }
 inline bool window_check_skipped(const Layer &L, int i) { return L.fused != F_NONE && (!fused_may_fall_back(L) || (L.fused == F_RESBLOCK && i < L.launcher)); }
+inline bool lean_multi_head(const yolo_ctx *c, const Layer &Y) { return Y.tree < 0 && c->lean && c->lean_thr > 0.f && c->lean_heads >= 1 && c->lean_heads <= 4; }
 inline bool rides_as_tail(const yolo_ctx *c, const Layer &L) { return L.fused_into >= 0 && c->layers[L.fused_into].tail_on; }
 inline bool issues_launch(const yolo_ctx *c, int i) { const Layer &L = c->layers[i]; return (L.fused == F_NONE || L.launcher == i) && !rides_as_tail(c, L); }
 
@@ -149,6 +152,7 @@
 void resolve_scales(yolo_ctx *c);
 void channel_scales(const yolo_ctx *c, int idx, std::vector<float> &out);
 int tail_fragments(yolo_ctx *c);
+int head_spares(yolo_ctx *c);
 int parse_tree(const std::string &text, Tree &t, std::string &err);
 int load_tree(const std::string &path, Tree &t, std::string &err);
 std::vector<int> pack_tree(const Tree &t, size_t at[7]);
diff --git a/yolo_tensorflow_amd/csrc/yolo_pack.cpp b/yolo_tensorflow_amd/csrc/yolo_pack.cpp
--- a/yolo_tensorflow_amd/csrc/yolo_pack.cpp
+++ b/yolo_tensorflow_amd/csrc/yolo_pack.cpp
@@ -159,6 +159,27 @@
     return YOLO_OK;
 }
 
+int head_spares(yolo_ctx *c)
+{
+    std::vector<uint8_t> w; std::vector<float> b;
+    for (size_t i = 0; i + 1 < c->layers.size(); ++i) {
+        Layer &L = c->layers[i]; const Layer &Y = c->layers[i + 1];
+        L.prune_bc = 0;
+        if (L.type != L_CONV || !L.head || !L.d_obj || Y.type != L_YOLO || !c->half_like() || !c->weights_loaded || rides_as_tail(c, L)) continue;
+        const ConvArgs a = conv_args(c, L, c->max_batch);
+        const int bc = conv_head_prune_bc(conv_resolve_cfg(a, L.tile_cfg));
+        if (!bc || a.split || a.pairk || !head_prunable(L.filters, 5 + Y.classes, Y.na, bc, L.cout_pad, nullptr)) continue;
+        const size_t row = (size_t)L.kpad * dt_size(L.in_dt);
+        HIPCK(c, hipSetDevice(c->device)); HIPCK(c, hipStreamSynchronize(c->stream));
+        w.resize((size_t)L.cout_pad * row); b.resize(L.cout_pad);
+        HIPCK(c, hipMemcpy(w.data(), L.d_w, w.size(), hipMemcpyDeviceToHost)); HIPCK(c, hipMemcpy(b.data(), L.d_b, b.size() * 4, hipMemcpyDeviceToHost));
+        if (!head_pack_spares(w.data(), row, b.data(), L.filters, 5 + Y.classes, Y.na, bc, L.cout_pad)) continue;
+        HIPCK(c, hipMemcpy(L.d_w, w.data(), w.size(), hipMemcpyHostToDevice)); HIPCK(c, hipMemcpy(L.d_b, b.data(), b.size() * 4, hipMemcpyHostToDevice));
+        L.prune_bc = bc;
+    }
+    return YOLO_OK;
+}
+
 }
 
 extern "C" {
@@ -240,7 +261,7 @@
     }
     if (int rc = tail_fragments(c)) return rc;
     c->weights_loaded = true;
-    return YOLO_OK;
+    return head_spares(c);
 }
 
 int yolo_load_darknet_weights(yolo_ctx *c, const char *path, int header_ints)
@@ -368,6 +389,7 @@
     if (tail_fragments(c) != YOLO_OK) return bail(c, c->err);
     c->weights_loaded = true;
     if (hd.num_cfgs == (uint32_t)conv_num_cfgs() && !keep_layers) { if (yolo_set_tile_configs(c, plan.data()) != YOLO_OK) { std::vector<int32_t> none(hd.n_layers, -1); yolo_set_tile_configs(c, none.data()); } }
+    if (head_spares(c) != YOLO_OK) return bail(c, c->err);
     return c;
 }
 
diff --git a/yolo_tensorflow_amd/csrc/yolo_plan.cpp b/yolo_tensorflow_amd/csrc/yolo_plan.cpp
--- a/yolo_tensorflow_amd/csrc/yolo_plan.cpp
+++ b/yolo_tensorflow_amd/csrc/yolo_plan.cpp
@@ -1,4 +1,34 @@
 #include "yolo_ctx.h"
+
+bool head_prunable(int cout, int attrs, int na, int bc, int cout_pad, int *spare_src)
+{
+    if (spare_src) for (int r = 0; r < cout_pad - cout; ++r) spare_src[r] = -1;
+    if (attrs < 5 || na < 1 || na > 16 || cout != na * attrs || bc < 1 || cout_pad < cout) return false;
+    std::vector<int> src(cout_pad - cout > 0 ? cout_pad - cout : 0, -1);
+    for (int c0 = 0; c0 < cout; c0 += bc) {
+        const int c1 = std::min(c0 + bc, cout_pad), real1 = std::min(c1, cout);
+        for (int an = c0 / attrs; an < na && an * attrs < real1; ++an) {
+            const int obj = an * attrs + 4;
+            if (obj >= c0 && obj < real1) continue;
+            if (src.empty() || an != c0 / attrs || obj >= c0 || cout < c0 || cout >= c1 || src[0] >= 0) return false;
+            src[0] = obj;
+        }
+    }
+    if (spare_src) std::copy(src.begin(), src.end(), spare_src);
+    return true;
+}
+
+bool head_pack_spares(void *w, size_t row_bytes, float *bias, int cout, int attrs, int na, int bc, int cout_pad)
+{
+    std::vector<int> src(cout_pad - cout > 0 ? cout_pad - cout : 0, -1);
+    if (!w || !bias || !head_prunable(cout, attrs, na, bc, cout_pad, src.data())) return false;
+    for (size_t r = 0; r < src.size(); ++r) {
+        if (src[r] < 0) continue;
+        memcpy((char *)w + (cout + r) * row_bytes, (const char *)w + (size_t)src[r] * row_bytes, row_bytes);
+        bias[cout + r] = bias[src[r]];
+    }
+    return true;
+}
 
 namespace yolo_impl {
 
@@ -463,6 +493,7 @@
         for (auto &L : c->layers) if (L.type == L_YOLO) { ++c->lean_heads; same = same && (classes < 0 || classes == L.classes) && L.na <= 16 && 5 + L.classes <= 128; classes = L.classes; }
         if (!same || (size_t)c->max_batch * c->rows * 340 >= 0xffffffffull) c->lean_heads = 0;
     }
+    c->prune_on = !getenv("YOLO_NO_HEAD_PRUNE") && !c->keep_layers;
     c->rows_pow2 = 1; while (c->rows_pow2 < c->rows) c->rows_pow2 <<= 1;
     HIPCK(c, hipMalloc((void **)&c->d_scores, nr * 4)); HIPCK(c, hipMalloc((void **)&c->d_labels, nr * 4));
     HIPCK(c, hipMalloc((void **)&c->d_cand, nr * 4)); HIPCK(c, hipMalloc((void **)&c->d_keys, (size_t)c->max_batch * c->rows_pow2 * 8));
@@ -498,3 +529,19 @@
 }
 
 }
+
+extern "C" {
+
+int yolo_head_prune_plan(int cout, int attrs, int anchors, int bc, int cout_pad, int32_t *spare_src)
+{
+    if (cout < 1 || attrs < 1 || anchors < 1 || bc < 1 || cout_pad < cout) return YOLO_ERR_INVALID;
+    return head_prunable(cout, attrs, anchors, bc, cout_pad, (int *)spare_src) ? 1 : 0;
+}
+
+int yolo_head_pack_spares(void *filters, size_t row_bytes, float *bias, int cout, int attrs, int anchors, int bc, int cout_pad)
+{
+    if (!filters || !bias || cout < 1 || attrs < 1 || anchors < 1 || bc < 1 || cout_pad < cout) return YOLO_ERR_INVALID;
+    return head_pack_spares(filters, row_bytes, bias, cout, attrs, anchors, bc, cout_pad) ? 1 : 0;
+}
+
+}
diff --git a/yolo_tensorflow_amd/csrc/yolo_run.cpp b/yolo_tensorflow_amd/csrc/yolo_run.cpp
--- a/yolo_tensorflow_amd/csrc/yolo_run.cpp
+++ b/yolo_tensorflow_amd/csrc/yolo_run.cpp
@@ -146,6 +146,8 @@
     }
     if (c->dtype == YOLO_FP32) { HIPCK(c, launch_conv_f32(a, s)); return YOLO_OK; }
     const int cfg = conv_resolve_cfg(a, L.tile_cfg);
+    if (L.head && L.d_obj && c->prune_on && L.prune_bc && L.prune_bc == conv_head_prune_bc(cfg) && i + 1 < (int)c->layers.size() && c->layers[i + 1].type == L_YOLO &&
+        lean_multi_head(c, c->layers[i + 1]) && conv_head_prune_ok(a, cfg)) { a.prune_below = c->lean_thr; c->heads_pruned = true; }
     if (a.w2 && !a.split && !a.pairk && !conv_cfg_tail_ok(cfg, a.Cout, a.in_dt == DT_FP8, a.tail_f32 != 0)) return fail(c, YOLO_ERR_STATE, "layer %d: tile config %d cannot run the fused 1x1 tail", i, cfg);
     HIPCK(c, a.in_dt == DT_FP8 ? launch_conv_fp8(a, cfg, s) : launch_conv_bf16(a, cfg, s));
     return YOLO_OK;
@@ -155,7 +157,7 @@
 {
     const Layer &L = c->layers[i];
     hipStream_t s = c->stream;
-    if (L.tree < 0 && c->lean && c->lean_thr > 0.f && c->lean_heads >= 1 && c->lean_heads <= 4) {
+    if (lean_multi_head(c, L)) {
         bool later_head = false;
         for (size_t k = i + 1; k < c->layers.size(); ++k) later_head |= c->layers[k].type == L_YOLO;
         if (later_head) return YOLO_OK;
@@ -293,6 +295,7 @@
 static int run_layers(yolo_ctx *c, int n, bool skip_conv = false, std::vector<hipEvent_t> *ev = nullptr)
 {
     const int NL = (int)c->layers.size();
+    c->heads_pruned = false;
     for (int i = 0; i < NL; ++i) {
         if (!(skip_conv && c->layers[i].type == L_CONV)) { int r = run_layer(c, i, n); if (r) return r; }
         if (ev) HIPCK(c, hipEventRecord((*ev)[i + 1], c->stream));
@@ -514,11 +517,11 @@
         e = hipGraphInstantiate(&c->gexec, g, nullptr, nullptr, 0);
         hipGraphDestroy(g);
         if (e != hipSuccess) { (void)hipGetLastError(); c->gexec = nullptr; c->gstate = -1; return eager(); }
-        c->gstate = 2;
+        c->gstate = 2; c->graph_pruned = c->heads_pruned;
     }
     if (c->lean_cnt_dirty) { HIPCK(c, hipMemsetAsync(c->d_lean_cnt, 0, 4, c->stream)); c->lean_cnt_dirty = false; }
     HIPCK(c, hipGraphLaunch(c->gexec, c->stream));
-    c->lean = nms_mode != YOLO_NMS_NUMPY_V3 && c->lean_ok; c->det_valid = !c->lean; c->lean_thr = score_thr;
+    c->lean = nms_mode != YOLO_NMS_NUMPY_V3 && c->lean_ok; c->det_valid = !c->lean; c->lean_thr = score_thr; c->heads_pruned = c->graph_pruned;
     c->last_n = n; c->scores_mode = nms_mode == YOLO_NMS_NUMPY_V3 ? 1 : 0;
     return YOLO_OK;
 }
@@ -641,11 +644,11 @@
         e = hipGraphInstantiate(&c->gexec_img, gr, nullptr, nullptr, 0);
         hipGraphDestroy(gr);
         if (e != hipSuccess) { (void)hipGetLastError(); c->gexec_img = nullptr; c->gstate_img = -1; return eager(); }
-        c->gstate_img = 2;
+        c->gstate_img = 2; c->graph_img_pruned = c->heads_pruned;
     }
     if (c->lean_cnt_dirty) { HIPCK(c, hipMemsetAsync(c->d_lean_cnt, 0, 4, c->stream)); c->lean_cnt_dirty = false; }
     HIPCK(c, hipGraphLaunch(c->gexec_img, c->stream));
-    c->lean = lean && c->lean_ok; c->det_valid = !c->lean; c->lean_thr = score_thr;
+    c->lean = lean && c->lean_ok; c->det_valid = !c->lean; c->lean_thr = score_thr; c->heads_pruned = c->graph_img_pruned;
     c->last_n = n; c->scores_mode = nms_mode == YOLO_NMS_NUMPY_V3 ? 1 : 0; c->stem_u8 = nullptr; c->geom_fit = fit; c->geom_n = n;
     return YOLO_OK;
 }
@@ -741,7 +744,7 @@
     if (n < 1 || n > c->max_batch || iters < 1) return fail(c, YOLO_ERR_INVALID, "bad n/iters");
     HIPCK(c, hipSetDevice(c->device));
     const int NL = (int)c->layers.size();
-    c->lean = false; c->det_valid = true;
+    c->lean = false; c->det_valid = true; c->heads_pruned = false;
     if (c->stem_u8 && n > c->stem_u8_n) c->stem_u8 = nullptr;
     EventSet evs(NL + 1); if (!evs.ok) return fail(c, YOLO_ERR_HIP, "hipEventCreate failed");
     std::vector<hipEvent_t> &ev = evs.e;
diff --git a/yolo_tensorflow_amd/csrc/yolo_tune.cpp b/yolo_tensorflow_amd/csrc/yolo_tune.cpp
--- a/yolo_tensorflow_amd/csrc/yolo_tune.cpp
+++ b/yolo_tensorflow_amd/csrc/yolo_tune.cpp
@@ -129,7 +129,7 @@
         }
     }
     drop_graph(c);
-    return YOLO_OK;
+    return head_spares(c);
 }
 
 int yolo_get_tile_configs(const yolo_ctx *c, int32_t *cfgs)
@@ -158,7 +158,7 @@
         c->layers[i].tile_cfg = v; c->layers[i].tail_on = tail;
     }
     drop_graph(c);
-    return YOLO_OK;
+    return head_spares(c);
 }
 
 }
diff --git a/yolo_tensorflow_amd/hip.py b/yolo_tensorflow_amd/hip.py
--- a/yolo_tensorflow_amd/hip.py
+++ b/yolo_tensorflow_amd/hip.py
@@ -35,7 +35,7 @@
     "yolo_forward_images_u8", "yolo_detect_images_u8", "yolo_detect_images_graph", "yolo_fit_unit_value", "yolo_darknet_boxes_at",
     "yolo_num_classes", "yolo_classify", "yolo_classify_images_u8", "yolo_op_avgpool", "yolo_op_softmax",
     "yolo_set_hier_thresh", "yolo_set_hierarchy_mode", "yolo_darknet_boxes_map", "yolo_tree_geometry", "yolo_tree_read", "yolo_plan_check", "yolo_plan_table",
-    "yolo_op_tree_softmax", "yolo_op_tree_top",
+    "yolo_op_tree_softmax", "yolo_op_tree_top", "yolo_head_prune_plan", "yolo_head_pack_spares",
 ]
 HIER_CONDITIONAL, HIER_ABSOLUTE, HIER_LEAVES = 0, 1, 2
 _HIER_MODES = {None: HIER_CONDITIONAL, "conditional": HIER_CONDITIONAL, "absolute": HIER_ABSOLUTE, "leaves": HIER_LEAVES}
@@ -133,6 +133,9 @@
     l.yolo_plan_table.argtypes = [C.c_char_p, I, I, I, C.c_char_p, SZ, C.c_char_p, SZ]
     l.yolo_op_tree_softmax.argtypes = [P, I, I, C.c_char_p, F, I, P, I]
     l.yolo_op_tree_top.argtypes = [P, I, C.c_char_p, F, P, I]
+    if hasattr(l, "yolo_head_prune_plan"):
+        l.yolo_head_prune_plan.argtypes = [I, I, I, I, I, P]
+        l.yolo_head_pack_spares.argtypes = [P, SZ, P, I, I, I, I, I]
     l.yolo_shard_bounds.argtypes = [I, I, I, C.POINTER(I), C.POINTER(I)]
     l.yolo_dist_flat_words.argtypes = [I, I]; l.yolo_dist_flat_words.restype = C.c_size_t
     l.yolo_dist_split_records.argtypes = [P, I, I, I, P, P]
```

Result: no change. 12660 img/s, median of 5 (+0.2%).
